# sonniki/image-captioning-with-external-knowledge

Hardware: AMD Instinct MI355X
Metric: decode_steps_per_sec (higher is better)
Workload: dtype f32 (3xbf16 split products, fp32 accumulate); 1 GPU; cfg2: geo variant, per-GPU batch 64 x 20 decode positions, 14x14x2048 features, K=20 knowledge rows, vocab 10000; global_batch=64, graph=True, collective_backend=none, split_allreduce=False, parallelism=dp1 (one flat-bucket all-reduce per step)

## Files before the change

image-captioning-with-external-knowledge_amd/csrc/adam.hip:

```cpp
#include "gemm_common.h"
#include "opt_words.h"

namespace ick {
namespace {

struct AdamHyper {
    float gscale, clip, b1, b2, c1, c2, eps, step, bc2_sqrt, coef, w, wd, f;
    bool coupled;
};

struct AdamEma {
    float* e;
    const float* decay;
    int warmup;
};

struct AdamDecay {
    const float* wd;
    const uint8_t* mask;
    int64_t granules;
    int64_t base;
    int coupled;
};

constexpr int kGranuleShift = 6;

__device__ __forceinline__ bool decay_on(const AdamDecay& dec, int64_t at) {
    const int64_t gr = at >> kGranuleShift;
    return gr < dec.granules && dec.mask[gr] != 0;
}

template <bool kOpt, bool kEma, bool kDecay>
__device__ __forceinline__ bool adam_hyper(AdamHyper& h, float gscale, float clip, float lr, float b1, float b2, float eps,
                                           int step0, const uint32_t* step_ptr, const float* __restrict__ gscale_den,
                                           float* words, const ick_lr_schedule& sched, const AdamEma& ema,
                                           const AdamDecay& dec) {
    if (gscale_den) {
        if (!(gscale_den[0] > 0.f)) return false;
        gscale = gscale / gscale_den[0];
    }
    const float t = (float)(step0 + (step_ptr ? (int)*step_ptr : 0));
    const float bc1 = 1.f - powf(b1, t);
    h.bc2_sqrt = sqrtf(1.f - powf(b2, t));
    h.coef = 1.f;
    if (kOpt) {
        lr = lr_schedule(words[kWordBaseLr], sched, t);
        h.coef = words[kWordCoef];
        if (blockIdx.x == 0 && threadIdx.x == 0) words[kWordLrNow] = lr;
    }
    h.step = lr / bc1;
    h.w = 0.f;
    if (kEma) {
        float d = ema.decay[0];
        if (ema.warmup) d = fminf(d, (1.f + t) / (10.f + t));
        h.w = 1.f - d;
    }
    h.wd = 0.f; h.f = 1.f; h.coupled = false;
    if (kDecay) {
        h.wd = dec.wd[0];
        const float shrink = lr * h.wd;
        h.f = 1.f - shrink;
        h.coupled = dec.coupled != 0;
    }
    h.gscale = gscale; h.clip = clip; h.b1 = b1; h.b2 = b2; h.c1 = 1.f - b1; h.c2 = 1.f - b2; h.eps = eps;
    return true;
}

template <bool kOpt, bool kDecay = false>
__device__ __forceinline__ void adam1(const AdamHyper& h, float& p, float& g, float& m, float& v, bool on = false) {
    float x = g * h.gscale;
    if (kOpt) x = x * h.coef;
    if (h.clip > 0.f) x = fminf(fmaxf(x, -h.clip), h.clip);
    g = x;
    if (kDecay && on) {
        if (h.coupled) {
            const float term = h.wd * p;
            x = x + term;
        } else {
            p = p * h.f;
        }
    }
    m = h.b1 * m + h.c1 * x;
    v = h.b2 * v + h.c2 * x * x;
    p -= h.step * m / (sqrtf(v) / h.bc2_sqrt + h.eps);
}

__device__ __forceinline__ void ema1(const AdamHyper& h, float& e, float p) {
    const float d = p - e;
    e = e + h.w * d;
}

__device__ __forceinline__ void ema4(const AdamHyper& h, float4& e, const float4& p) {
    ema1(h, e.x, p.x);
    ema1(h, e.y, p.y);
    ema1(h, e.z, p.z);
    ema1(h, e.w, p.w);
}

template <bool kOpt, bool kDecay = false>
__device__ __forceinline__ void adam4(const AdamHyper& h, float4& p, float4& g, float4& m, float4& v, bool on = false) {
    adam1<kOpt, kDecay>(h, p.x, g.x, m.x, v.x, on);
    adam1<kOpt, kDecay>(h, p.y, g.y, m.y, v.y, on);
    adam1<kOpt, kDecay>(h, p.z, g.z, m.z, v.z, on);
    adam1<kOpt, kDecay>(h, p.w, g.w, m.w, v.w, on);
}

template <bool kOpt, bool kEma, bool kDecay>
__global__ __launch_bounds__(256) void adam_clamp_kernel(float* __restrict__ p, float* __restrict__ g,
                                                         float* __restrict__ m, float* __restrict__ v, int64_t n,
                                                         float gscale, float clip, float lr, float b1, float b2,
                                                         float eps, int step0, const uint32_t* step_ptr,
                                                         const float* __restrict__ gscale_den, float* words,
                                                         ick_lr_schedule sched, AdamEma ema, AdamDecay dec) {
    const int64_t stride = (int64_t)gridDim.x * 256;
    AdamHyper h;
    if (!adam_hyper<kOpt, kEma, kDecay>(h, gscale, clip, lr, b1, b2, eps, step0, step_ptr, gscale_den, words, sched, ema,
                                         dec))
        return;
    for (int64_t i = (int64_t)blockIdx.x * 256 + threadIdx.x; i < n; i += stride) {
        float gi = g[i], mi = m[i], vi = v[i], pi = p[i], ei = 0.f;
        if (kEma) ei = ema.e[i];
        adam1<kOpt, kDecay>(h, pi, gi, mi, vi, kDecay && decay_on(dec, dec.base + i));
        g[i] = gi; m[i] = mi; v[i] = vi; p[i] = pi;
        if (kEma) { ema1(h, ei, pi); ema.e[i] = ei; }
    }
}

template <bool kOpt, bool kEma, bool kDecay>
__global__ __launch_bounds__(256) void adam_clamp_vec4_kernel(float4* __restrict__ p, float4* __restrict__ g,
                                                              float4* __restrict__ m, float4* __restrict__ v, int64_t n4,
                                                              float gscale, float clip, float lr, float b1, float b2,
                                                              float eps, int step0, const uint32_t* step_ptr,
                                                              const float* __restrict__ gscale_den, float* words,
                                                              ick_lr_schedule sched, AdamEma ema, AdamDecay dec) {
    const int64_t stride = (int64_t)gridDim.x * 256;
    AdamHyper h;
    if (!adam_hyper<kOpt, kEma, kDecay>(h, gscale, clip, lr, b1, b2, eps, step0, step_ptr, gscale_den, words, sched, ema,
                                         dec))
        return;
    float4* __restrict__ e = reinterpret_cast<float4*>(ema.e);
    for (int64_t i = (int64_t)blockIdx.x * 256 + threadIdx.x; i < n4; i += stride) {
        float4 gi = g[i], mi = m[i], vi = v[i], pi = p[i], ei;
        if (kEma) ei = e[i];
        adam4<kOpt, kDecay>(h, pi, gi, mi, vi, kDecay && decay_on(dec, dec.base + 4 * i));
        g[i] = gi; m[i] = mi; v[i] = vi; p[i] = pi;
        if (kEma) { ema4(h, ei, pi); e[i] = ei; }
    }
}

constexpr int kT = 64;
constexpr int kLd = 68;

template <bool kOpt, bool kEma, bool kDecay>
__global__ __launch_bounds__(256) void adam_derive_kernel(float* __restrict__ p, float* __restrict__ g,
                                                          float* __restrict__ m, float* __restrict__ v,
                                                          const ick_adam_item* __restrict__ items,
                                                          const ick_adam_block* __restrict__ blocks, float gscale,
                                                          float clip, float lr, float b1, float b2, float eps, int step0,
                                                          const uint32_t* step_ptr, const float* __restrict__ gscale_den,
                                                          float* words, ick_lr_schedule sched, AdamEma ema, AdamDecay dec) {
    __shared__ __attribute__((aligned(16))) float tile[kT * kLd];
    const ick_adam_block blk = blocks[blockIdx.x];
    AdamHyper h;
    if (!adam_hyper<kOpt, kEma, kDecay>(h, gscale, clip, lr, b1, b2, eps, step0, step_ptr, gscale_den, words, sched, ema,
                                         dec))
        return;
    const int tid = threadIdx.x;

    if (blk.item < 0) {
        float4* p4 = reinterpret_cast<float4*>(p) + blk.off4;
        float4* g4 = reinterpret_cast<float4*>(g) + blk.off4;
        float4* m4 = reinterpret_cast<float4*>(m) + blk.off4;
        float4* v4 = reinterpret_cast<float4*>(v) + blk.off4;
        float4* e4 = reinterpret_cast<float4*>(ema.e) + blk.off4;
        float4 pi[4], gi[4], mi[4], vi[4], ei[4];
        bool on[4];
#pragma unroll
        for (int i = 0; i < 4; ++i) {
            const int j = tid + 256 * i;
            on[i] = false;
            if (j < blk.cnt4) {
                gi[i] = g4[j]; mi[i] = m4[j]; vi[i] = v4[j]; pi[i] = p4[j];
                if (kEma) ei[i] = e4[j];
                if (kDecay) on[i] = decay_on(dec, 4 * ((int64_t)blk.off4 + j));
            }
        }
#pragma unroll
        for (int i = 0; i < 4; ++i) {
            const int j = tid + 256 * i;
            if (j < blk.cnt4) {
                adam4<kOpt, kDecay>(h, pi[i], gi[i], mi[i], vi[i], on[i]);
                g4[j] = gi[i]; m4[j] = mi[i]; v4[j] = vi[i]; p4[j] = pi[i];
                if (kEma) { ema4(h, ei[i], pi[i]); e4[j] = ei[i]; }
                if (blk.copy) reinterpret_cast<float4*>(blk.copy)[j] = pi[i];
            }
        }
        return;
    }

    const ick_adam_item it = items[blk.item];
    const int n0 = blk.tn * kT, k0 = blk.tk * kT;
    const int K = it.K;
    {
        float4 pi[4], gi[4], mi[4], vi[4], ei[4];
        int64_t at[4];
        bool on[4];
#pragma unroll
        for (int i = 0; i < 4; ++i) {
            const int idx = tid + 256 * i;
            const int row = idx >> 4, c4 = idx & 15;
            const int r = n0 + row - it.drow0, k = k0 + 4 * c4;
            at[i] = (r >= 0 && r < it.rows && k < K) ? it.off + (int64_t)r * K + k : -1;
            if (at[i] >= 0) {
                gi[i] = *reinterpret_cast<const float4*>(g + at[i]);
                mi[i] = *reinterpret_cast<const float4*>(m + at[i]);
                vi[i] = *reinterpret_cast<const float4*>(v + at[i]);
                pi[i] = *reinterpret_cast<const float4*>(p + at[i]);
                if (kEma) ei[i] = *reinterpret_cast<const float4*>(ema.e + at[i]);
            }
            on[i] = kDecay && at[i] >= 0 && decay_on(dec, at[i]);
        }
#pragma unroll
        for (int i = 0; i < 4; ++i) {
            const int idx = tid + 256 * i;
            const int row = idx >> 4, c4 = idx & 15;
            float4 out = make_float4(0.f, 0.f, 0.f, 0.f);
            if (at[i] >= 0) {
                adam4<kOpt, kDecay>(h, pi[i], gi[i], mi[i], vi[i], on[i]);
                *reinterpret_cast<float4*>(g + at[i]) = gi[i];
                *reinterpret_cast<float4*>(m + at[i]) = mi[i];
                *reinterpret_cast<float4*>(v + at[i]) = vi[i];
                *reinterpret_cast<float4*>(p + at[i]) = pi[i];
                if (kEma) { ema4(h, ei[i], pi[i]); *reinterpret_cast<float4*>(ema.e + at[i]) = ei[i]; }
                out = pi[i];
                if (it.copy) *reinterpret_cast<float4*>(it.copy + (int64_t)(n0 + row) * it.copy_ld + k0 + 4 * c4) = pi[i];
            }
            *reinterpret_cast<float4*>(tile + row * kLd + 4 * c4) = out;
        }
    }
    __syncthreads();
    const int rlo = it.drow0 - n0, rhi = it.drow0 + it.rows - n0;

    if (it.pack) {
        const int K16 = (K + 15) & ~15;
#pragma unroll
        for (int i = 0; i < 4; ++i) {
            const int u = tid + 256 * i;
            const int j = u >> 6, l = u & 63;
            const int k4 = blk.tk * 16 + j;
// ... 17 lines not shown
    }
    if (it.ps) {
        const int64_t np = (int64_t)((it.Nd + 63) / 64) * 64;
        const int K32 = (K + 31) & ~31;
        char* base = reinterpret_cast<char*>(it.ps);
#pragma unroll
        for (int i = 0; i < 2; ++i) {
            const int u = tid + 256 * i;
            const int row = u & 63, c = u >> 6;
            const int k = k0 + 8 * c;
            if (row >= rlo && row < rhi && k < K32) {
                const float4 a = *reinterpret_cast<const float4*>(tile + row * kLd + 8 * c);
                const float4 b = *reinterpret_cast<const float4*>(tile + row * kLd + 8 * c + 4);
                uint32_t hh[4], mm[4], ll[4];
                split3(a.x, a.y, hh[0], mm[0], ll[0]); split3(a.z, a.w, hh[1], mm[1], ll[1]);
                split3(b.x, b.y, hh[2], mm[2], ll[2]); split3(b.z, b.w, hh[3], mm[3], ll[3]);
                char* dst = base + (((int64_t)(k >> 5) * 3) * np + n0 + row) * 64 + (k & 31) * 2;
                *reinterpret_cast<uint4*>(dst) = uint4{hh[0], hh[1], hh[2], hh[3]};
                *reinterpret_cast<uint4*>(dst + np * 64) = uint4{mm[0], mm[1], mm[2], mm[3]};
                *reinterpret_cast<uint4*>(dst + 2 * np * 64) = uint4{ll[0], ll[1], ll[2], ll[3]};
            }
        }
    }
    if (it.ps_t) {
        const int64_t kp = (int64_t)((K + 63) / 64) * 64;
        char* base = reinterpret_cast<char*>(it.ps_t);
#pragma unroll
        for (int i = 0; i < 2; ++i) {
            const int u = tid + 256 * i;
            const int kk = u & 63, c = u >> 6;
            if (8 * c >= rlo && 8 * c < rhi && k0 + kk < K) {
                float x[8];
#pragma unroll
                for (int e = 0; e < 8; ++e) x[e] = tile[(8 * c + e) * kLd + kk];
                uint32_t hh[4], mm[4], ll[4];
#pragma unroll
                for (int e = 0; e < 4; ++e) split3(x[2 * e], x[2 * e + 1], hh[e], mm[e], ll[e]);
                const int n = n0 + 8 * c;
                char* dst = base + (((int64_t)(n >> 5) * 3) * kp + k0 + kk) * 64 + (n & 31) * 2;
                *reinterpret_cast<uint4*>(dst) = uint4{hh[0], hh[1], hh[2], hh[3]};
                *reinterpret_cast<uint4*>(dst + kp * 64) = uint4{mm[0], mm[1], mm[2], mm[3]};
                *reinterpret_cast<uint4*>(dst + 2 * kp * 64) = uint4{ll[0], ll[1], ll[2], ll[3]};
            }
        }
    }
    if (it.tr) {
#pragma unroll
        for (int i = 0; i < 16; ++i) {
            const int u = tid + 256 * i;
            const int nl = u & 63, kl = u >> 6;
            if (nl >= rlo && nl < rhi && k0 + kl < K) it.tr[(int64_t)(k0 + kl) * it.tr_ld + n0 + nl] = tile[nl * kLd + kl];
        }
    }
}

}
}

using namespace ick;

template <bool kEma, bool kDecay>
static int adam_args(const float* p, const float* g, const float* m, const float* v, int64_t count, int32_t step,
                     const uint32_t* step_ptr, const AdamEma& ema, const AdamDecay& dec, bool& al16) {
    ICK_CHECK_ARG(p && g && m && v && count > 0 && (step >= 1 || step_ptr != nullptr));
    if (kEma) ICK_CHECK_ARG(ema.e != nullptr && ema.decay != nullptr);
    if (kDecay)
        ICK_CHECK_ARG(dec.wd != nullptr && dec.mask != nullptr && dec.granules > 0 &&
                      (dec.coupled == ICK_DECAY_DECOUPLED || dec.coupled == ICK_DECAY_COUPLED));
    al16 = ((reinterpret_cast<uintptr_t>(p) | reinterpret_cast<uintptr_t>(g) | reinterpret_cast<uintptr_t>(m) |
             reinterpret_cast<uintptr_t>(v) | (kEma ? reinterpret_cast<uintptr_t>(ema.e) : 0)) & 15) == 0;
    return ICK_OK;
}

template <bool kOpt, bool kEma, bool kDecay = false>
static int launch_adam(float* p, float* g, float* m, float* v, int64_t n, float gscale, float clip, float lr, float* words,
                       ick_lr_schedule sched, float beta1, float beta2, float eps, int32_t step, const uint32_t* step_ptr,
                       const float* gscale_den, AdamEma ema, void* stream, AdamDecay dec = AdamDecay{}) {
    bool al16;
    if (int rc = adam_args<kEma, kDecay>(p, g, m, v, n, step, step_ptr, ema, dec, al16)) return rc;
    if (kDecay) ICK_CHECK_ARG(dec.granules >= ceil_div(n, (int64_t)1 << kGranuleShift));
    if (kEma && (reinterpret_cast<uintptr_t>(ema.e) & 3)) return ICK_EALIGN;
    int64_t done = 0;
    if (n >= 4096 && al16) {
        const int64_t n4 = n / 4;
        hipLaunchKernelGGL((adam_clamp_vec4_kernel<kOpt, kEma, kDecay>), dim3((int)std::min<int64_t>(ceil_div(n4, 256), 4096)),
                           dim3(256), 0, (hipStream_t)stream, reinterpret_cast<float4*>(p), reinterpret_cast<float4*>(g),
                           reinterpret_cast<float4*>(m), reinterpret_cast<float4*>(v), n4, gscale, clip, lr, beta1, beta2,
                           eps, step, step_ptr, gscale_den, words, sched, ema, dec);
        done = 4 * n4;
        if (done == n) ICK_LAUNCH_RET();
    }
    if (kEma) ema.e += done;
    dec.base = done;
    hipLaunchKernelGGL((adam_clamp_kernel<kOpt, kEma, kDecay>), dim3((int)std::min<int64_t>(ceil_div(n - done, 256), 4096)),
                       dim3(256), 0, (hipStream_t)stream, p + done, g + done, m + done, v + done, n - done, gscale, clip, lr,
                       beta1, beta2, eps, step, step_ptr, gscale_den, words, sched, ema, dec);
    ICK_LAUNCH_RET();
}

template <bool kOpt, bool kEma, bool kDecay = false>
static int launch_adam_derive(float* p, float* g, float* m, float* v, const ick_adam_item* items,
                              const ick_adam_block* blocks, int32_t n_blocks, float gscale, float clip, float lr,
                              float* words, ick_lr_schedule sched, float beta1, float beta2, float eps, int32_t step,
                              const uint32_t* step_ptr, const float* gscale_den, AdamEma ema, void* stream,
                              AdamDecay dec = AdamDecay{}) {
    bool al16;
    if (int rc = adam_args<kEma, kDecay>(p, g, m, v, blocks ? n_blocks : 0, step, step_ptr, ema, dec, al16)) return rc;
    if (!al16) return ICK_EALIGN;
    hipLaunchKernelGGL((adam_derive_kernel<kOpt, kEma, kDecay>), dim3(n_blocks), dim3(256), 0, (hipStream_t)stream, p, g, m, v,
                       items, blocks, gscale, clip, lr, beta1, beta2, eps, step, step_ptr, gscale_den, words, sched, ema,
                       dec);
    ICK_LAUNCH_RET();
}

extern "C" int ick_adam_clamp(float* p, float* g, float* m, float* v, int64_t n, float gscale, float clip, float lr,
                              float beta1, float beta2, float eps, int32_t step, const uint32_t* step_ptr,
                              const float* gscale_den, void* stream) {
    return launch_adam<false, false>(p, g, m, v, n, gscale, clip, lr, nullptr, ick_lr_schedule{}, beta1, beta2, eps, step,
                                     step_ptr, gscale_den, AdamEma{}, stream);
}

extern "C" int ick_adam_opt(float* p, float* g, float* m, float* v, int64_t n, float gscale, float clip, float* words,
                            ick_lr_schedule sched, float beta1, float beta2, float eps, int32_t step,
                            const uint32_t* step_ptr, const float* gscale_den, void* stream) {
    ICK_CHECK_ARG(words != nullptr && lr_schedule_ok(sched));
    return launch_adam<true, false>(p, g, m, v, n, gscale, clip, 0.f, words, sched, beta1, beta2, eps, step, step_ptr,
                                    gscale_den, AdamEma{}, stream);
}

extern "C" int ick_adam_clamp_derive(float* p, float* g, float* m, float* v, const ick_adam_item* items,
                                     const ick_adam_block* blocks, int32_t n_blocks, float gscale, float clip, float lr,
                                     float beta1, float beta2, float eps, int32_t step, const uint32_t* step_ptr,
                                     const float* gscale_den, void* stream) {
    return launch_adam_derive<false, false>(p, g, m, v, items, blocks, n_blocks, gscale, clip, lr, nullptr,
                                            ick_lr_schedule{}, beta1, beta2, eps, step, step_ptr, gscale_den, AdamEma{},
                                            stream);
}

extern "C" int ick_adam_opt_derive(float* p, float* g, float* m, float* v, const ick_adam_item* items,
                                   const ick_adam_block* blocks, int32_t n_blocks, float gscale, float clip, float* words,
                                   ick_lr_schedule sched, float beta1, float beta2, float eps, int32_t step,
                                   const uint32_t* step_ptr, const float* gscale_den, void* stream) {
    ICK_CHECK_ARG(words != nullptr && lr_schedule_ok(sched));
    return launch_adam_derive<true, false>(p, g, m, v, items, blocks, n_blocks, gscale, clip, 0.f, words, sched, beta1,
                                           beta2, eps, step, step_ptr, gscale_den, AdamEma{}, stream);
}

extern "C" int ick_adam_ema(float* p, float* g, float* m, float* v, float* e, int64_t n, float gscale, float clip, float lr,
                            float* words, ick_lr_schedule sched, float beta1, float beta2, float eps, int32_t step,
                            const uint32_t* step_ptr, const float* gscale_den, const float* ema_decay, int32_t ema_warmup,
                            void* stream) {
    const AdamEma ema{e, ema_decay, ema_warmup != 0};
    if (!words)
        return launch_adam<false, true>(p, g, m, v, n, gscale, clip, lr, nullptr, ick_lr_schedule{}, beta1, beta2, eps,
                                        step, step_ptr, gscale_den, ema, stream);
    ICK_CHECK_ARG(lr_schedule_ok(sched));
    return launch_adam<true, true>(p, g, m, v, n, gscale, clip, 0.f, words, sched, beta1, beta2, eps, step, step_ptr,
                                   gscale_den, ema, stream);
}

extern "C" int ick_adam_ema_derive(float* p, float* g, float* m, float* v, float* e, const ick_adam_item* items,
                                   const ick_adam_block* blocks, int32_t n_blocks, float gscale, float clip, float lr,
                                   float* words, ick_lr_schedule sched, float beta1, float beta2, float eps, int32_t step,
                                   const uint32_t* step_ptr, const float* gscale_den, const float* ema_decay,
// ... 16 lines not shown
    return opt();
}

extern "C" int ick_adam_decay(float* p, float* g, float* m, float* v, float* e, int64_t n, float gscale, float clip,
                              float lr, float* words, ick_lr_schedule sched, float beta1, float beta2, float eps,
                              int32_t step, const uint32_t* step_ptr, const float* gscale_den, const float* ema_decay,
                              int32_t ema_warmup, const float* decay, const uint8_t* decay_mask, int64_t n_granules,
                              int32_t decay_form, void* stream) {
    const AdamEma ema{e, ema_decay, ema_warmup != 0};
    const AdamDecay dec{decay, decay_mask, n_granules, 0, decay_form};
    const ick_lr_schedule none{};
    if (!e)
        return with_rate(
            words, sched,
            [&] { return launch_adam<false, false, true>(p, g, m, v, n, gscale, clip, lr, nullptr, none, beta1, beta2, eps,
                                                         step, step_ptr, gscale_den, AdamEma{}, stream, dec); },
            [&] { return launch_adam<true, false, true>(p, g, m, v, n, gscale, clip, 0.f, words, sched, beta1, beta2, eps,
                                                        step, step_ptr, gscale_den, AdamEma{}, stream, dec); });
    return with_rate(
        words, sched,
        [&] { return launch_adam<false, true, true>(p, g, m, v, n, gscale, clip, lr, nullptr, none, beta1, beta2, eps, step,
                                                    step_ptr, gscale_den, ema, stream, dec); },
        [&] { return launch_adam<true, true, true>(p, g, m, v, n, gscale, clip, 0.f, words, sched, beta1, beta2, eps, step,
                                                   step_ptr, gscale_den, ema, stream, dec); });
}

extern "C" int ick_adam_decay_derive(float* p, float* g, float* m, float* v, float* e, const ick_adam_item* items,
                                     const ick_adam_block* blocks, int32_t n_blocks, float gscale, float clip, float lr,
                                     float* words, ick_lr_schedule sched, float beta1, float beta2, float eps, int32_t step,
                                     const uint32_t* step_ptr, const float* gscale_den, const float* ema_decay,
                                     int32_t ema_warmup, const float* decay, const uint8_t* decay_mask,
                                     int64_t n_granules, int32_t decay_form, void* stream) {
    const AdamEma ema{e, ema_decay, ema_warmup != 0};
    const AdamDecay dec{decay, decay_mask, n_granules, 0, decay_form};
    const ick_lr_schedule none{};
    if (!e)
        return with_rate(
            words, sched,
            [&] { return launch_adam_derive<false, false, true>(p, g, m, v, items, blocks, n_blocks, gscale, clip, lr,
                                                                nullptr, none, beta1, beta2, eps, step, step_ptr,
                                                                gscale_den, AdamEma{}, stream, dec); },
            [&] { return launch_adam_derive<true, false, true>(p, g, m, v, items, blocks, n_blocks, gscale, clip, 0.f, words,
                                                               sched, beta1, beta2, eps, step, step_ptr, gscale_den,
                                                               AdamEma{}, stream, dec); });
    return with_rate(
        words, sched,
        [&] { return launch_adam_derive<false, true, true>(p, g, m, v, items, blocks, n_blocks, gscale, clip, lr, nullptr,
                                                           none, beta1, beta2, eps, step, step_ptr, gscale_den, ema, stream,
                                                           dec); },
        [&] { return launch_adam_derive<true, true, true>(p, g, m, v, items, blocks, n_blocks, gscale, clip, 0.f, words,
                                                          sched, beta1, beta2, eps, step, step_ptr, gscale_den, ema, stream,
                                                          dec); });
}
```

image-captioning-with-external-knowledge_amd/csrc/backward.hip:

```cpp
#include "common.h"

namespace ick {
namespace {

template <int NJ>
__global__ __launch_bounds__(256) void layernorm_bwd_kernel(const float* __restrict__ dy, const float* __restrict__ x,
                                                            const float* __restrict__ res,
                                                            const float* __restrict__ gamma,
                                                            const float* __restrict__ mean,
                                                            const float* __restrict__ rstd, float* __restrict__ dz,
                                                            float* __restrict__ dgamma, float* __restrict__ dbeta,
                                                            int64_t rows, int d, int rows_per_block,
                                                            float* __restrict__ dx_drop, DropArg darg,
                                                            float* __restrict__ partials) {
    chain_priority();
    extern __shared__ float sm[];
    const Dropout drop = darg.get();
    const int lane = threadIdx.x & 63, wave = threadIdx.x >> 6;
    float ag[NJ], ab[NJ], gm[NJ];
#pragma unroll
    for (int j = 0; j < NJ; ++j) {
        const int c = lane + 64 * j;
        ag[j] = 0.f; ab[j] = 0.f;
        gm[j] = c < d ? gamma[c] : 0.f;
// ... 150 lines not shown
                                                                float* __restrict__ dtype_emb, int ntypes,
                                                                float* __restrict__ dword, int B, int K, int d) {
    if (!SEQ) chain_priority();
    const ScatterWalk<SEQ> w(B * K);
    for (int row = w.row; row < w.row_end; ++row) {
        const EntityIndex ix = entity_index(variant, ent + (int64_t)row * cols, ntypes, vocab);
        bool mine = w.owns(ix.type);
        if (variant == ICK_NEWS && dword != nullptr) {
#pragma unroll
            for (int q = 0; q < 5; ++q) mine = mine || w.owns(ix.name[q]);
        }
        if (!mine) continue;
        for (int c = w.col; c < d; c += w.col_step) {
            float g = dee[(int64_t)row * d + c];
            if (variant == ICK_NEWS) {
                float s = 0.f;
#pragma unroll
                for (int q = 0; q < 5; ++q) s += word_emb[(int64_t)ix.name[q] * d + c];
                const float avg = s / 5.0f;
                const float enc_g = g * avg;
                if (dword) {
                    const float enc = avg != 0.f ? ee[(int64_t)row * d + c] / avg : 0.f;
                    const float gw = g * enc / 5.0f;
#pragma unroll
                    for (int q = 0; q < 5; ++q) w.add(dword + (int64_t)ix.name[q] * d + c, ix.name[q], gw);
                }
                g = enc_g;
            }
            if (c >= ix.type_off)
                w.add(dtype_emb + (int64_t)ix.type * (d - ix.type_off) + (c - ix.type_off), ix.type, g);
        }
    }
}

template <bool SEQ>
__global__ __launch_bounds__(256) void fact_encode_bwd_kernel(const float* __restrict__ dfe,
                                                              const int64_t* __restrict__ facts, float* __restrict__ dee,
                                                              float* __restrict__ dpred, int num_pred, int B, int K,
                                                              int F, int d) {
    if (!SEQ) chain_priority();
    const ScatterWalk<SEQ> w(B * F);
    for (int row = w.row; row < w.row_end; ++row) {
        const FactPair f = fact_pair(facts, row, K, num_pred);
        const int64_t erow = (int64_t)(row / F) * K + f.subj;
        if (!w.owns(erow) && !w.owns(f.pred)) continue;
        for (int c = w.col; c < d; c += w.col_step) {
            const float g = dfe[(int64_t)row * d + c];
            w.add(dee + erow * d + c, erow, g);
            w.add(dpred + (int64_t)f.pred * d + c, f.pred, g);
        }
    }
}

__global__ __launch_bounds__(256) void pointer_bwd_dh_kernel(const float* __restrict__ ds, int64_t ds_ld, int col0,
                                                             const float* __restrict__ ctx, const float* __restrict__ w,
                                                             const float* __restrict__ ind, float* __restrict__ dh,
                                                             int T, int Kc, int d, const int32_t* __restrict__ rowmap,
                                                             const int32_t* __restrict__ count) {
    chain_priority();
    int b = blockIdx.y, t = blockIdx.x;
    int64_t dsrow = (int64_t)b * T + t;
    if (rowmap != nullptr) {
        if (dsrow >= device_bound((int)gridDim.y * T, count)) return;
        const int lr = rowmap[dsrow];
        b = lr / T;
        t = lr - b * T;
    }
    const float* dsr = ds + dsrow * ds_ld + col0;
    for (int c = threadIdx.x; c < d; c += 256) {
        float acc = 0.f;
        const float* cc = ctx + (int64_t)b * Kc * d + c;
        int k = 0;
        for (; k + 8 <= Kc; k += 8) {
            float v[8], g[8];
#pragma unroll
            for (int q = 0; q < 8; ++q) {
                v[q] = cc[(int64_t)(k + q) * d];
                g[q] = dsr[k + q];
                if (ind) g[q] *= ind[((int64_t)b * T + t) * Kc + k + q];
            }
#pragma unroll
            for (int q = 0; q < 8; ++q) acc = fmaf(g[q], v[q], acc);
        }
        for (; k < Kc; ++k) {
            float g = dsr[k];
            if (ind) g *= ind[((int64_t)b * T + t) * Kc + k];
            acc = fmaf(g, cc[(int64_t)k * d], acc);
        }
        dh[((int64_t)b * T + t) * d + c] += acc * w[c];
    }
}

template <bool SEQ>
__global__ __launch_bounds__(256) void pointer_bwd_dctx_kernel(const float* __restrict__ ds, int64_t ds_ld, int col0,
                                                               const float* __restrict__ h, const float* __restrict__ ctx,
                                                               const float* __restrict__ w, const float* __restrict__ ind,
                                                               float* __restrict__ dctx, float* __restrict__ dw,
                                                               float* __restrict__ dbias, int B, int T, int Kc, int d,
                                                               const int32_t* __restrict__ rowstart) {
    chain_priority();
    extern __shared__ float gs[];
    float* red = gs + T * Kc;
    float* dwp = red + 4;
    const int lane = threadIdx.x & 63, wave = threadIdx.x >> 6;
  for (int b = SEQ ? 0 : blockIdx.x; b < (SEQ ? B : (int)blockIdx.x + 1); ++b) {
    float bsum = 0.f;
    const int64_t row0 = rowstart ? rowstart[b] : (int64_t)b * T;
    const int nrow = rowstart ? min(T, rowstart[b + 1] - rowstart[b]) : T;
    for (int idx = threadIdx.x; idx < T * Kc; idx += 256) {
        const int t = idx / Kc, k = idx - t * Kc;
        float g = t < nrow ? ds[(row0 + t) * ds_ld + col0 + k] : 0.f;
        bsum += g;
        if (ind) g *= ind[((int64_t)b * T + t) * Kc + k];
        gs[idx] = g;
    }
    bsum = block_sum<4>(bsum, red);
    if (threadIdx.x == 0 && blockIdx.y == 0) { if (SEQ) dbias[0] += bsum; else atomicAdd(dbias, bsum); }
    const int c = blockIdx.y * 64 + lane;
    const bool ok = c < d;
    const float* hb = h + (int64_t)b * T * d + (ok ? c : 0);
    const float wc = ok ? w[c] : 0.f;
    float dwl = 0.f;
    for (int k = wave; k < Kc; k += 4) {
        float acc = 0.f;
        for (int t = 0; t < T; ++t) acc = fmaf(gs[t * Kc + k], hb[(int64_t)t * d], acc);
        if (ok) {
            const int64_t o = ((int64_t)b * Kc + k) * d + c;
            dctx[o] += acc * wc;
            dwl = fmaf(acc, ctx[o], dwl);
        }
    }
    dwp[wave * 64 + lane] = dwl;
    __syncthreads();
    if (wave == 0 && ok) {
        const float t = (dwp[lane] + dwp[64 + lane]) + (dwp[128 + lane] + dwp[192 + lane]);
        if (SEQ) dw[c] += t; else atomicAdd(dw + c, t);
    }
    if (SEQ) __syncthreads();
  }
}

template <bool SEQ>
__global__ __launch_bounds__(256) void context_gate_bwd_kernel(const int64_t* __restrict__ captions,
                                                               const int64_t* __restrict__ facts,
                                                               const float* __restrict__ dgate, float* __restrict__ dw,
                                                               float* __restrict__ dbias, int B, int L, int T, int K, int F,
                                                               int V, int num_pred, int d, int mode) {
    extern __shared__ int smi[];
    const int tid = threadIdx.x;
  for (int b = SEQ ? 0 : blockIdx.x; b < (SEQ ? B : (int)blockIdx.x + 1); ++b) {
    const GateTables g = build_gate_tables(smi, captions, facts, b, L, K, F, V, num_pred, mode);
    const int *act = g.act, *pred = g.pred, *rep = g.rep;
    float* suf = reinterpret_cast<float*>(g.end);
    const int c = blockIdx.y * 256 + tid;
    if (c < d) {
        float run = 0.f;
        for (int p = T - 1; p >= 0; --p) {
            run += dgate[((int64_t)b * T + p) * d + c];
            suf[p * 256 + tid] = run;
        }
        if (SEQ) dbias[c] += run; else atomicAdd(dbias + c, run);
        for (int j = 0; j < F; ++j) {
            if (!rep[j] || act[j] >= T) continue;
            float* dst = dw + (int64_t)c * num_pred + pred[j];
            if (SEQ) *dst += suf[act[j] * 256 + tid]; else atomicAdd(dst, suf[act[j] * 256 + tid]);
        }
    }
    if (SEQ) __syncthreads();
  }
}

__global__ void counter_add_kernel(uint32_t* c, uint32_t inc, const float* flag) {
    if (flag == nullptr || flag[0] > 0.f) *c += inc;
}

__global__ __launch_bounds__(256) void scale_kernel(float* __restrict__ x, int64_t n, const float* __restrict__ num,
                                                    const float* __restrict__ den) {
    const float s = num[0] / den[0];
    const int64_t stride = (int64_t)gridDim.x * 256;
    for (int64_t i = (int64_t)blockIdx.x * 256 + threadIdx.x; i < n; i += stride) x[i] *= s;
}

}
}

using namespace ick;

extern "C" int ick_layernorm_bwd_rows_per_block(void) { return 8; }

extern "C" int ick_layernorm_bwd(const float* dy, const float* x, const float* res, const float* gamma,
                                 const float* mean, const float* rstd, float* dz, float* dgamma, float* dbeta,
                                 int64_t rows, int32_t d, float* dx_drop, float drop_p, uint32_t drop_seed,
// ... 29 lines not shown

extern "C" int ick_colsum(const float* a, int64_t M, int32_t N, int64_t ld, float* out, void* stream) {
    ICK_CHECK_ARG(a && out && M > 0 && N > 0 && ld >= N);
    const int rpb = deterministic() ? (int)std::min<int64_t>(M, 1 << 30) : 64;
    ICK_CHECK_ARG(ceil_div(M, rpb) <= 65535);
    hipLaunchKernelGGL(colsum_kernel, dim3(ceil_div(N, 64), ceil_div(M, rpb)), dim3(256), 0, (hipStream_t)stream, a, M,
                       N, ld, out, rpb);
    ICK_LAUNCH_RET();
}

extern "C" int ick_caption_embed_bwd(const float* dx, const int64_t* captions, const int64_t* masks, float* dword,
                                     float* dee, float* dfe, int32_t B, int32_t L, int32_t K, int32_t F, int32_t V,
                                     int32_t d, int32_t pad_token, float scale, float drop_p, uint32_t drop_seed,
                                     uint32_t drop_site, const uint32_t* drop_epoch, void* stream) {
    ICK_CHECK_ARG(dx && captions && masks && dee && B > 0 && L > 0 && K > 0 && d > 0);
    if (deterministic())
        hipLaunchKernelGGL(caption_embed_bwd_kernel<true>, dim3(kDetParts, ceil_div(d, 256)), dim3(256), 0,
                           (hipStream_t)stream, dx, captions, masks, dword, dee, dfe, B, L, K, F, V, d, pad_token, scale,
                           DropArg{drop_p, drop_seed, drop_site, drop_epoch});
    else
        hipLaunchKernelGGL(caption_embed_bwd_kernel<false>, dim3(ceil_div((int64_t)B * L, 4)), dim3(256), 0, (hipStream_t)stream,
                           dx, captions, masks, dword, dee, dfe, B, L, K, F, V, d, pad_token, scale,
                           DropArg{drop_p, drop_seed, drop_site, drop_epoch});
    ICK_LAUNCH_RET();
}

extern "C" int ick_pointer_scores_bwd(const float* ds, int64_t ds_ld, int32_t col0, const float* h, const float* ctx,
                                      const float* w, const float* ind, float* dh, float* dctx, float* dw,
                                      float* dbias, int32_t B, int32_t T, int32_t Kc, int32_t d, void* stream) {
    return ick_pointer_scores_bwd_packed(ds, ds_ld, col0, h, ctx, w, ind, dh, dctx, dw, dbias, B, T, Kc, d, nullptr, nullptr,
                                         stream);
}

extern "C" int ick_pointer_scores_bwd_packed(const float* ds, int64_t ds_ld, int32_t col0, const float* h, const float* ctx,
                                             const float* w, const float* ind, float* dh, float* dctx, float* dw,
                                             float* dbias, int32_t B, int32_t T, int32_t Kc, int32_t d,
                                             const int32_t* rowmap, const int32_t* rowstart, void* stream) {
    ICK_CHECK_ARG(ds && h && ctx && w && dh && dctx && dw && dbias && B > 0 && B <= 65535 && T > 0 && Kc > 0 && d > 0);
    ICK_CHECK_ARG((rowmap == nullptr) == (rowstart == nullptr) && (int64_t)B * T <= INT32_MAX);
    const size_t smem = ((size_t)T * Kc + 4 + 256) * sizeof(float);
    ICK_CHECK_ARG(smem <= 64 * 1024);
    hipStream_t s = (hipStream_t)stream;
    hipLaunchKernelGGL(pointer_bwd_dh_kernel, dim3(T, B), dim3(256), 0, s, ds, ds_ld, col0, ctx, w, ind, dh, T, Kc, d, rowmap,
                       rowstart ? rowstart + B : nullptr);
    if (deterministic())
        hipLaunchKernelGGL(pointer_bwd_dctx_kernel<true>, dim3(1, ceil_div(d, 64)), dim3(256), smem, s, ds, ds_ld, col0, h,
                           ctx, w, ind, dctx, dw, dbias, B, T, Kc, d, rowstart);
    else
        hipLaunchKernelGGL(pointer_bwd_dctx_kernel<false>, dim3(B, ceil_div(d, 64)), dim3(256), smem, s, ds, ds_ld, col0, h,
                           ctx, w, ind, dctx, dw, dbias, B, T, Kc, d, rowstart);
    ICK_LAUNCH_RET();
}

extern "C" int ick_entity_encode_bwd(int32_t variant, const float* dee, const float* entities, int32_t ent_cols,
                                     const float* ee, const float* word_emb, int32_t vocab, float* dtype_emb,
                                     int32_t ntypes, float* dword, int32_t B, int32_t K, int32_t d, void* stream) {
    ICK_CHECK_ARG(dee && entities && dtype_emb && B > 0 && K > 0 && d > 6);
    if (variant == ICK_NEWS) ICK_CHECK_ARG(ee && word_emb && vocab > 0);
    if (deterministic())
        hipLaunchKernelGGL(entity_encode_bwd_kernel<true>, dim3(kDetParts, ceil_div(d, 256)), dim3(256), 0,
                           (hipStream_t)stream, variant, dee, entities, ent_cols, ee, word_emb, vocab, dtype_emb, ntypes,
                           dword, B, K, d);
    else
        hipLaunchKernelGGL(entity_encode_bwd_kernel<false>, dim3(ceil_div((int64_t)B * K, 4)), dim3(256), 0, (hipStream_t)stream,
                           variant, dee, entities, ent_cols, ee, word_emb, vocab, dtype_emb, ntypes, dword, B, K, d);
    ICK_LAUNCH_RET();
}

extern "C" int ick_fact_encode_bwd(const float* dfe, const int64_t* facts, float* dee, float* dpred, int32_t num_pred,
                                   int32_t B, int32_t K, int32_t F, int32_t d, void* stream) {
    ICK_CHECK_ARG(dfe && facts && dee && dpred && B > 0 && K > 0 && F > 0 && d > 0);
    if (deterministic())
        hipLaunchKernelGGL(fact_encode_bwd_kernel<true>, dim3(kDetParts, ceil_div(d, 256)), dim3(256), 0, (hipStream_t)stream,
                           dfe, facts, dee, dpred, num_pred, B, K, F, d);
    else
        hipLaunchKernelGGL(fact_encode_bwd_kernel<false>, dim3(ceil_div((int64_t)B * F, 4)), dim3(256), 0, (hipStream_t)stream,
                           dfe, facts, dee, dpred, num_pred, B, K, F, d);
    ICK_LAUNCH_RET();
}

extern "C" int ick_context_gate_bwd(const int64_t* captions, const int64_t* facts, const float* dgate, float* dw,
                                    float* dbias, int32_t B, int32_t L, int32_t T, int32_t K, int32_t F, int32_t V,
                                    int32_t num_pred, int32_t d, int32_t mode, void* stream) {
    ICK_CHECK_ARG(captions && facts && dgate && dw && dbias && B > 0 && L > 0 && K > 0 && F > 0);
    ICK_CHECK_ARG((mode == 0 && T == L) || (mode == 1 && T == 1));
    const size_t smem = gate_table_ints(K, F) * sizeof(int) + (size_t)T * 256 * sizeof(float);
    ICK_CHECK_ARG(smem <= 64 * 1024);
    if (deterministic())
        hipLaunchKernelGGL(context_gate_bwd_kernel<true>, dim3(1, ceil_div(d, 256)), dim3(256), smem, (hipStream_t)stream,
                           captions, facts, dgate, dw, dbias, B, L, T, K, F, V, num_pred, d, mode);
    else
        hipLaunchKernelGGL(context_gate_bwd_kernel<false>, dim3(B, ceil_div(d, 256)), dim3(256), smem, (hipStream_t)stream,
                           captions, facts, dgate, dw, dbias, B, L, T, K, F, V, num_pred, d, mode);
    ICK_LAUNCH_RET();
}

extern "C" int ick_scale_by_ratio(float* x, int64_t n, const float* num, const float* den, void* stream) {
    ICK_CHECK_ARG(x && num && den && n > 0);
    hipLaunchKernelGGL(scale_kernel, dim3((int)std::min<int64_t>(ceil_div(n, 256), 4096)), dim3(256), 0,
                       (hipStream_t)stream, x, n, num, den);
    ICK_LAUNCH_RET();
}

extern "C" int ick_counter_add(uint32_t* counter, uint32_t inc, void* stream) {
    ICK_CHECK_ARG(counter != nullptr);
    hipLaunchKernelGGL(counter_add_kernel, dim3(1), dim3(1), 0, (hipStream_t)stream, counter, inc, (const float*)nullptr);
// ... 9 lines not shown
```

image-captioning-with-external-knowledge_amd/csrc/score_head.hip:

```cpp
#include "decode_select.h"

namespace ick {
namespace {

constexpr int kMaxPerLane = 16;

template <int NJ>
__global__ __launch_bounds__(256) void pointer_scores_kernel(const float* __restrict__ h, const float* __restrict__ ctx,
                                                             const float* __restrict__ w, const float* __restrict__ bias,
                                                             const float* __restrict__ ind, float* __restrict__ out,
                                                             int T, int Kc, int d, int64_t out_ld, int col0,
                                                             const int32_t* __restrict__ out_gmap,
                                                             const int32_t* __restrict__ rowmap,
                                                             const int32_t* __restrict__ count) {
    chain_priority();
    constexpr int KB = 4;
    const int lane = threadIdx.x & 63, wave = threadIdx.x >> 6;
    int b = blockIdx.y, t = blockIdx.x;
    int64_t orow_id = -1;
    if (rowmap != nullptr) {
        const int m = b * T + t;
        if (m >= device_bound((int)gridDim.y * T, count)) return;
        const int lr = rowmap[m];
        b = lr / T;
// ... 294 lines not shown
        if (tid == 0) row_loss[row] = lse - r[target];
    }
    if (dr) {
        const float wr = kWeighted ? weight[b] : 1.f;
        const float inv = wr / s;
        const float wt = kSmooth ? wr * keep : wr, wu = wr * nsub;
        float4* d4 = reinterpret_cast<float4*>(dr);
        const int tq = (int)(target >> 2), tr = (int)(target & 3);
        for (int i0 = 0; i0 < n4; i0 += 256 * 4) {
            float4 x[4];
#pragma unroll
            for (int j = 0; j < 4; ++j) {
                const int i = i0 + tid + 256 * j;
                x[j] = i < n4 ? r4[i] : make_float4(0.f, 0.f, 0.f, 0.f);
            }
#pragma unroll
            for (int j = 0; j < 4; ++j) {
                const int i = i0 + tid + 256 * j;
                if (i < n4) {
                    float4 gq = make_float4(__expf(x[j].x - m) * inv, __expf(x[j].y - m) * inv, __expf(x[j].z - m) * inv,
                                            __expf(x[j].w - m) * inv);
                    if constexpr (kSmooth) { gq.x += wu; gq.y += wu; gq.z += wu; gq.w += wu; }
                    if (i == tq) {
                        if (tr == 0) gq.x -= wt; else if (tr == 1) gq.y -= wt; else if (tr == 2) gq.z -= wt; else gq.w -= wt;
                    }
                    d4[i] = gq;
                }
            }
        }
        for (int i0 = 4 * n4; i0 < Vx; i0 += 256 * 8) {
            float x[8];
#pragma unroll
            for (int j = 0; j < 8; ++j) {
                const int i = i0 + tid + 256 * j;
                x[j] = i < Vx ? r[i] : 0.f;
            }
#pragma unroll
            for (int j = 0; j < 8; ++j) {
                const int i = i0 + tid + 256 * j;
                if (i < Vx) {
                    if constexpr (kSmooth) dr[i] = (__expf(x[j] - m) * inv + wu) - (i == target ? wt : 0.f);
                    else dr[i] = __expf(x[j] - m) * inv - (i == target ? wr : 0.f);
                }
            }
        }
    }
}

template <bool kWeighted>
__global__ __launch_bounds__(256) void packed_ce_reduce_kernel(const float* __restrict__ row_loss, int n, int L,
                                                               const float* __restrict__ weight,
                                                               float* __restrict__ loss_sum, float* __restrict__ count,
                                                               const int32_t* __restrict__ rowmap,
                                                               const int32_t* __restrict__ nrows) {
    __shared__ float red[4];
    float s = 0.f, c = 0.f;
    n = device_bound(n, nrows);
    for (int i = threadIdx.x; i < n; i += 256) {
        const float v = row_loss[i];
        if (v > -0.5f) { s += kWeighted ? weight[(rowmap ? rowmap[i] : i) / L] * v : v; c += 1.f; }
    }
    s = block_sum<4>(s, red);
    c = block_sum<4>(c, red);
    if (threadIdx.x == 0) { loss_sum[0] = s; count[0] = c; }
}

struct RowScan {
    float m, s;
    float cnt;
    int bi;
};
__device__ __forceinline__ void row_scan_push(RowScan& a, float x, int c, float st, int target) {
    a.s += __expf(x - a.m);
    a.cnt += (x > st || (x == st && c < target)) ? 1.f : 0.f;
}
__device__ __forceinline__ void row_scan_best(float& bv, int& bi, float x, int c) {
    if (x > bv) { bv = x; bi = c; }
}

__global__ __launch_bounds__(256) void row_logprob_rank_kernel(const float* __restrict__ scores, int64_t ld,
                                                               const int64_t* __restrict__ caps,
                                                               const int32_t* __restrict__ rowmap,
                                                               const int32_t* __restrict__ count, int L, int Vx, int pad,
                                                               float* __restrict__ tlp, int32_t* __restrict__ rank,
                                                               int32_t* __restrict__ best) {
    __shared__ float4 red[4];
    const int tid = threadIdx.x, lane = tid & 63, wave = tid >> 6;
    const int64_t row = (int64_t)blockIdx.y * L + blockIdx.x;
    if (row >= device_bound((int)gridDim.y * L, count)) return;
    const int lr = rowmap[row];
    const int b = lr / L, t = lr - b * L;
    if (b >= (int)gridDim.y || t >= L - 1) return;
    const int64_t o = (int64_t)b * (L - 1) + t;
    const int64_t target64 = caps[(int64_t)b * L + t + 1];
    if (target64 == pad || target64 < 0 || target64 >= Vx) {
        if (tid == 0) { tlp[o] = 0.f; rank[o] = -1; best[o] = -1; }
        return;
    }
    const int target = (int)target64;
    const float* r = scores + row * ld;
    const float st = r[target];
    const bool vec = (ld & 3) == 0 && (reinterpret_cast<uintptr_t>(scores) & 15) == 0;
    const int n4 = vec ? (Vx >> 2) : 0;
    const float4* r4 = reinterpret_cast<const float4*>(r);
    RowScan a{-INFINITY, 0.f, 0.f, 0x7fffffff};
    for (int i0 = 0; i0 < n4; i0 += 256 * 4) {
        float4 x[4];
#pragma unroll
        for (int j = 0; j < 4; ++j) {
            const int i = i0 + tid + 256 * j;
            x[j] = i < n4 ? r4[i] : make_float4(-INFINITY, -INFINITY, -INFINITY, -INFINITY);
        }
        float bm = a.m;
        int bi = a.bi;
#pragma unroll
        for (int j = 0; j < 4; ++j) {
            const int c = 4 * (i0 + tid + 256 * j);
// ... 183 lines not shown
}

extern "C" int ick_head_rowmap(const int64_t* lengths, int32_t B, int32_t L, int32_t* decode_len, int32_t* rowstart,
                               int32_t* rowmap, void* stream) {
    using namespace ick;
    ICK_CHECK_ARG(lengths && decode_len && rowstart && rowmap && B > 0 && L > 0 && (int64_t)B * L <= INT32_MAX);
    hipLaunchKernelGGL(head_rowmap_kernel, dim3(1), dim3(256), 0, (hipStream_t)stream, lengths, B, L, decode_len, rowstart,
                       rowmap);
    ICK_LAUNCH_RET();
}

extern "C" int ick_gather_rows(const float* src, int64_t src_rs, const int32_t* rowmap, const int32_t* count, float* dst,
                               int64_t dst_rs, int32_t max_rows, int32_t d, void* stream) {
    using namespace ick;
    ICK_CHECK_ARG(src && rowmap && count && dst && max_rows > 0 && d > 0 && src_rs >= d && dst_rs >= d);
    hipLaunchKernelGGL(gather_rows_kernel, dim3(ceil_div(max_rows, 4)), dim3(256), 0, (hipStream_t)stream, src, src_rs,
                       rowmap, count, dst, dst_rs, max_rows, d);
    ICK_LAUNCH_RET();
}

extern "C" int ick_top2(const float* scores, int64_t ld, int32_t B, int32_t Vx, int32_t* best, int32_t* second,
                        void* stream) {
    using namespace ick;
    ICK_CHECK_ARG(scores && best && second && B > 0 && Vx > 0 && ld >= Vx);
    hipLaunchKernelGGL(top2_kernel, dim3(B), dim3(256), 0, (hipStream_t)stream, scores, ld, Vx, best, second);
    ICK_LAUNCH_RET();
}

extern "C" int ick_greedy_update(const int32_t* best, const int32_t* second, int64_t* output, int32_t* top2_hist,
                                 int32_t* finished, int64_t* next_token, int64_t* next_mask, int32_t B, int32_t step,
                                 int32_t max_len, int32_t V, int32_t K, int32_t has_facts, int32_t end_token,
                                 void* stream) {
    using namespace ick;
    ICK_CHECK_ARG(best && second && output && top2_hist && finished && next_token && next_mask);
    ICK_CHECK_ARG(B > 0 && step >= 0 && step < max_len);
    hipLaunchKernelGGL(greedy_update_kernel, dim3(ceil_div(B, 64)), dim3(64), 0, (hipStream_t)stream, best, second,
                       output, top2_hist, finished, next_token, next_mask, B, step, max_len, V, K, has_facts,
                       end_token);
    ICK_LAUNCH_RET();
}

extern "C" int ick_greedy_select(const float* scores, int64_t ld, int32_t B, int32_t Vx, int64_t* output,
                                 int32_t* top2_hist, int32_t* finished, int64_t* next_token, int64_t* next_mask,
                                 int32_t step, int32_t max_len, int32_t V, int32_t K, int32_t has_facts,
                                 int32_t end_token, void* stream) {
    using namespace ick;
    ICK_CHECK_ARG(scores && output && top2_hist && finished && next_token && next_mask);
    ICK_CHECK_ARG(B > 0 && Vx > 0 && ld >= Vx && step >= 0 && step < max_len);
    hipLaunchKernelGGL(greedy_select_kernel, dim3(B), dim3(256), 0, (hipStream_t)stream, scores, ld, Vx, output,
                       top2_hist, finished, next_token, next_mask, step, max_len, V, K, has_facts, end_token);
    ICK_LAUNCH_RET();
}

extern "C" int ick_packed_ce(const float* scores, int64_t ld, const int64_t* captions_sorted,
                             const int32_t* decode_len, int32_t B, int32_t L, int32_t Vx, int32_t pad_token,
                             float* row_loss, float* loss_sum, float* count, float* dscores, void* stream) {
    using namespace ick;
    ICK_CHECK_ARG(scores && captions_sorted && decode_len && row_loss && loss_sum && count);
    ICK_CHECK_ARG(B > 0 && B <= 65535 && L > 0 && Vx > 0 && ld >= Vx);
    hipStream_t s = (hipStream_t)stream;
    hipLaunchKernelGGL(packed_ce_rows_kernel<false>, dim3(L, B), dim3(256), 0, s, scores, ld, captions_sorted, decode_len,
                       L, Vx, pad_token, row_loss, dscores, nullptr, nullptr, CeEps<false>{});
    hipLaunchKernelGGL(packed_ce_reduce_kernel<false>, dim3(1), dim3(256), 0, s, row_loss, B * L, L, nullptr, loss_sum,
                       count, nullptr, nullptr);
    ICK_LAUNCH_RET();
}

extern "C" int ick_packed_ce_packed(const float* scores, int64_t ld, const int64_t* captions, const int32_t* rowmap,
                                    const int32_t* count, const float* weights, int32_t B, int32_t L, int32_t Vx,
                                    int32_t pad_token, float* row_loss, float* loss_sum, float* count_out, float* dscores,
                                    void* stream) {
    using namespace ick;
    ICK_CHECK_ARG(scores && captions && rowmap && count && row_loss && loss_sum && count_out);
    ICK_CHECK_ARG(B > 0 && B <= 65535 && L > 0 && Vx > 0 && ld >= Vx && (int64_t)B * L <= INT32_MAX);
    hipStream_t s = (hipStream_t)stream;
    if (weights != nullptr) {
        hipLaunchKernelGGL((packed_ce_rows_kernel<true, true>), dim3(L, B), dim3(256), 0, s, scores, ld, captions, count, L,
                           Vx, pad_token, row_loss, dscores, weights, rowmap, CeEps<false>{});
        hipLaunchKernelGGL(packed_ce_reduce_kernel<true>, dim3(1), dim3(256), 0, s, row_loss, B * L, L, weights, loss_sum,
                           count_out, rowmap, count);
    } else {
        hipLaunchKernelGGL((packed_ce_rows_kernel<false, true>), dim3(L, B), dim3(256), 0, s, scores, ld, captions, count, L,
                           Vx, pad_token, row_loss, dscores, nullptr, rowmap, CeEps<false>{});
        hipLaunchKernelGGL(packed_ce_reduce_kernel<false>, dim3(1), dim3(256), 0, s, row_loss, B * L, L, nullptr, loss_sum,
                           count_out, rowmap, count);
    }
    ICK_LAUNCH_RET();
}

extern "C" int ick_packed_ce_smooth(const float* scores, int64_t ld, const int64_t* captions, const int32_t* rowmap,
                                    const int32_t* count, const int32_t* decode_len, const float* weights,
                                    const float* eps, int32_t B, int32_t L, int32_t Vx, int32_t pad_token,
                                    float* row_loss, float* loss_sum, float* count_out, float* dscores, void* stream) {
    using namespace ick;
    ICK_CHECK_ARG(scores && captions && eps && row_loss && loss_sum && count_out);
    ICK_CHECK_ARG((rowmap != nullptr) == (count != nullptr) && (rowmap != nullptr || decode_len != nullptr));
    ICK_CHECK_ARG(B > 0 && B <= 65535 && L > 0 && Vx > 0 && ld >= Vx && (int64_t)B * L <= INT32_MAX);
    hipStream_t s = (hipStream_t)stream;
    const dim3 grid(L, B), block(256);
    const int32_t* dl = rowmap ? count : decode_len;
#define ICK_CE_SMOOTH(W, P)                                                                                            \
    hipLaunchKernelGGL((packed_ce_rows_kernel<W, P, true>), grid, block, 0, s, scores, ld, captions, dl, L, Vx,         \
                       pad_token, row_loss, dscores, weights, rowmap, CeEps<true>{eps})
    if (weights != nullptr) {
        if (rowmap) { ICK_CE_SMOOTH(true, true); } else { ICK_CE_SMOOTH(true, false); }
        hipLaunchKernelGGL(packed_ce_reduce_kernel<true>, dim3(1), block, 0, s, row_loss, B * L, L, weights, loss_sum,
                           count_out, rowmap, count);
    } else {
        if (rowmap) { ICK_CE_SMOOTH(false, true); } else { ICK_CE_SMOOTH(false, false); }
        hipLaunchKernelGGL(packed_ce_reduce_kernel<false>, dim3(1), block, 0, s, row_loss, B * L, L, nullptr, loss_sum,
                           count_out, rowmap, count);
    }
#undef ICK_CE_SMOOTH
    ICK_LAUNCH_RET();
}

extern "C" int ick_row_logprob_rank(const float* scores, int64_t ld, const int64_t* captions, const int32_t* rowmap,
                                    const int32_t* count, int32_t R, int32_t L, int32_t Vx, int32_t pad_token,
                                    float* token_log_prob, int32_t* rank, int32_t* best, void* stream) {
    using namespace ick;
    ICK_CHECK_ARG(scores && captions && rowmap && count && token_log_prob && rank && best);
    ICK_CHECK_ARG(R > 0 && R <= 65535 && L > 1 && Vx > 0 && Vx <= (1 << 24) && ld >= Vx && (int64_t)R * L <= INT32_MAX);
    hipLaunchKernelGGL(row_logprob_rank_kernel, dim3(L, R), dim3(256), 0, (hipStream_t)stream, scores, ld, captions,
                       rowmap, count, L, Vx, pad_token, token_log_prob, rank, best);
    ICK_LAUNCH_RET();
}

extern "C" int ick_caption_score_sums(const int32_t* rowstart, int32_t R, int32_t L, int32_t top_k, float* token_log_prob,
                                      int32_t* rank, int32_t* best, float* log_prob, int32_t* tokens, float* loss_sum,
                                      float* count, float* top1_hits, float* topk_hits, void* stream) {
    using namespace ick;
    ICK_CHECK_ARG(rowstart && token_log_prob && rank && best && log_prob && tokens && loss_sum && count && top1_hits &&
                  topk_hits);
    ICK_CHECK_ARG(R > 0 && L > 1 && top_k >= 1 && (int64_t)R * L <= INT32_MAX);
    hipStream_t s = (hipStream_t)stream;
    hipLaunchKernelGGL(caption_sums_kernel, dim3(ceil_div(R, 4)), dim3(256), 0, s, rowstart, R, L, token_log_prob, rank,
                       best, log_prob, tokens);
    hipLaunchKernelGGL(caption_totals_kernel, dim3(1), dim3(256), 0, s, token_log_prob, rank, (int64_t)R * (L - 1), top_k,
                       loss_sum, count, top1_hits, topk_hits);
    ICK_LAUNCH_RET();
}

extern "C" int ick_packed_ce_weighted(const float* scores, int64_t ld, const int64_t* captions_sorted,
                                      const int32_t* decode_len, const float* weights, int32_t B, int32_t L, int32_t Vx,
                                      int32_t pad_token, float* row_loss, float* loss_sum, float* count, float* dscores,
                                      void* stream) {
    using namespace ick;
    ICK_CHECK_ARG(scores && captions_sorted && decode_len && weights && row_loss && loss_sum && count);
    ICK_CHECK_ARG(B > 0 && B <= 65535 && L > 0 && Vx > 0 && ld >= Vx && (int64_t)B * L <= INT32_MAX);
    hipStream_t s = (hipStream_t)stream;
    hipLaunchKernelGGL(packed_ce_rows_kernel<true>, dim3(L, B), dim3(256), 0, s, scores, ld, captions_sorted, decode_len,
                       L, Vx, pad_token, row_loss, dscores, weights, nullptr, CeEps<false>{});
    hipLaunchKernelGGL(packed_ce_reduce_kernel<true>, dim3(1), dim3(256), 0, s, row_loss, B * L, L, weights, loss_sum,
                       count, nullptr, nullptr);
    ICK_LAUNCH_RET();
}
```

image-captioning-with-external-knowledge_amd/lib.py:

```python
import ctypes as C
import os

_PKG = os.path.dirname(os.path.abspath(__file__))
LIB_PATH = os.path.join(_PKG, "libick_amd.so")
if os.environ.get("ICK_LIB_PATH"):
    LIB_PATH = os.environ["ICK_LIB_PATH"]

ICK_GEO, ICK_KNOWLEDGE, ICK_NEWS = 0, 1, 2
VARIANT_ID = {"geo": ICK_GEO, "knowledge": ICK_KNOWLEDGE, "news": ICK_NEWS}
GEMM_RELU, GEMM_ACCUM, GEMM_ATOMIC, GEMM_COLSUM_ONLY = 1, 2, 4, 16

vp = C.c_void_p
i32 = C.c_int32
i64 = C.c_int64
f32 = C.c_float
u32 = C.c_uint32


class GemmArgs(C.Structure):
    _fields_ = [
        ("A", vp), ("B", vp), ("C", vp), ("bias", vp),
        ("M", i32), ("N", i32), ("K", i32),
        ("a_rs", i64), ("a_ks", i64), ("a_grp", i32), ("a_gs", i64), ("a_gmap", vp),
        ("b_rs", i64), ("b_ks", i64),
# ... 173 lines not shown
    "ick_greedy_select": [vp, i64, i32, i32, vp, vp, vp, vp, vp, i32, i32, i32, i32, i32, i32, vp],
    "ick_packed_ce": [vp, i64, vp, vp, i32, i32, i32, i32, vp, vp, vp, vp, vp],
    "ick_packed_ce_weighted": [vp, i64, vp, vp, vp, i32, i32, i32, i32, vp, vp, vp, vp, vp],
    "ick_samples_to_captions": [vp, i32, i32, i32, i32, i32, i32, i32, i32, vp, vp, vp, vp],
    "ick_cider_d": [vp, i32, i32, vp, i32, i32, i32, vp, vp, i32, f32, f32, i32, i32, i32, vp, i32, i32, vp, i32,
                    vp, vp, vp],
    "ick_decode_supported": [i32, i32, i32, i32, i32],
    "ick_decode_plan": [i32, i32, i32, i32, i32, C.POINTER(i32)],
    "ick_decode_layers": [C.POINTER(DecodeCtx), i32, vp],
    "ick_decode_layers_part": [C.POINTER(DecodeCtx), i32, i32, vp],
    "ick_decode_layers_attn": [C.POINTER(DecodeCtx), vp, i32, i32, vp],
    "ick_decode_init": [C.POINTER(DecodeCtx), i32, i32, vp],
    "ick_decode_select_greedy": [C.POINTER(DecodeCtx), i32, vp],
    "ick_decode_select_beam": [C.POINTER(DecodeCtx), C.POINTER(BeamState), i32, vp],
    "ick_decode_beam_supported": [i32, i32],
    "ick_decode_select_sample": [C.POINTER(DecodeCtx), C.POINTER(SampleState), i32, vp],
    "ick_decode_sample_supported": [i32, i32],
    "ick_decode_select_beam_rules": [C.POINTER(DecodeCtx), C.POINTER(BeamState), C.POINTER(DecodeRules), i32, vp],
    "ick_decode_select_sample_rules": [C.POINTER(DecodeCtx), C.POINTER(SampleState), C.POINTER(DecodeRules), i32, vp],
    "ick_decode_select_beam_diverse": [C.POINTER(DecodeCtx), C.POINTER(BeamState), C.POINTER(DecodeRules),
                                       C.POINTER(DecodeDiversity), i32, vp],
    "ick_decode_select_beam_forced": [C.POINTER(DecodeCtx), C.POINTER(BeamState), C.POINTER(DecodeRules),
                                      C.POINTER(DecodeConstraints), i32, vp],
    "ick_decode_select_beam_biased": [C.POINTER(DecodeCtx), C.POINTER(BeamState), C.POINTER(DecodeRules),
                                      C.POINTER(DecodeBias), i32, vp],
    "ick_decode_select_sample_biased": [C.POINTER(DecodeCtx), C.POINTER(SampleState), C.POINTER(DecodeRules),
                                        C.POINTER(DecodeBias), i32, vp],
    "ick_attention_bwd": [C.POINTER(AttnBwdArgs), vp],
    "ick_layernorm_bwd": [vp, vp, vp, vp, vp, vp, vp, vp, vp, i64, i32, vp, f32, u32, u32, vp, vp, vp],
    "ick_layernorm_bwd_rows_per_block": [],
    "ick_gemm_grouped": [vp, i32, vp],
    "ick_attention_bwd_overwrites": [i32, i32, i32],
    "ick_attention_plan": [i32, i32, i32, i32, i32, C.POINTER(i32)],
    "ick_relu_bwd": [vp, vp, vp, i64, f32, vp],
    "ick_colsum": [vp, i64, i32, i64, vp, vp],
    "ick_caption_embed_bwd": [vp, vp, vp, vp, vp, vp, i32, i32, i32, i32, i32, i32, i32, f32, f32, u32, u32, vp, vp],
    "ick_pointer_scores_bwd": [vp, i64, i32, vp, vp, vp, vp, vp, vp, vp, vp, i32, i32, i32, i32, vp],
    "ick_entity_encode_bwd": [i32, vp, vp, i32, vp, vp, i32, vp, i32, vp, i32, i32, i32, vp],
    "ick_fact_encode_bwd": [vp, vp, vp, vp, i32, i32, i32, i32, i32, vp],
    "ick_context_gate_bwd": [vp, vp, vp, vp, vp, i32, i32, i32, i32, i32, i32, i32, i32, i32, vp],
    "ick_adam_clamp": [vp, vp, vp, vp, i64, f32, f32, f32, f32, f32, f32, i32, vp, vp, vp],
    "ick_adam_clamp_derive": [vp, vp, vp, vp, vp, vp, i32, f32, f32, f32, f32, f32, f32, i32, vp, vp, vp],
    "ick_grad_sqnorm_plan": [i64, C.POINTER(i32)],
    "ick_grad_sqnorm": [vp, i64, f32, vp, vp, i64, vp, vp],
    "ick_adam_opt": [vp, vp, vp, vp, i64, f32, f32, vp, LrSchedule, f32, f32, f32, i32, vp, vp, vp],
    "ick_adam_opt_derive": [vp, vp, vp, vp, vp, vp, i32, f32, f32, vp, LrSchedule, f32, f32, f32, i32, vp, vp, vp],
    "ick_adam_ema": [vp, vp, vp, vp, vp, i64, f32, f32, f32, vp, LrSchedule, f32, f32, f32, i32, vp, vp, vp, i32, vp],
    "ick_adam_ema_derive": [vp, vp, vp, vp, vp, vp, vp, i32, f32, f32, f32, vp, LrSchedule, f32, f32, f32, i32, vp, vp, vp,
                            i32, vp],
    "ick_adam_decay": [vp, vp, vp, vp, vp, i64, f32, f32, f32, vp, LrSchedule, f32, f32, f32, i32, vp, vp, vp, i32, vp, vp,
                       i64, i32, vp],
    "ick_adam_decay_derive": [vp, vp, vp, vp, vp, vp, vp, i32, f32, f32, f32, vp, LrSchedule, f32, f32, f32, i32, vp, vp, vp,
                              i32, vp, vp, i64, i32, vp],
    "ick_conv1_wgrad_plan": [i32, i32, i32, i32, C.POINTER(i32), C.POINTER(i64)],
    "ick_conv1_wgrad": [vp, vp, vp, vp, i32, i32, i32, i32, vp, i64, vp],
    "ick_counter_add": [vp, u32, vp],
    "ick_counter_add_if": [vp, u32, vp, vp],
    "ick_timestamp": [vp, vp],
    "ick_copy_batch": [vp, vp, vp, i32, vp],
    "ick_scale_by_ratio": [vp, i64, vp, vp, vp],
    "ick_head_rowmap": [vp, i32, i32, vp, vp, vp, vp],
    "ick_pointer_scores_packed": [vp, vp, vp, vp, vp, vp, i32, i32, i32, i32, i64, i32, vp, vp, vp],
    "ick_packed_ce_packed": [vp, i64, vp, vp, vp, vp, i32, i32, i32, i32, vp, vp, vp, vp, vp],
    "ick_packed_ce_smooth": [vp, i64, vp, vp, vp, vp, vp, vp, i32, i32, i32, i32, vp, vp, vp, vp, vp],
    "ick_pointer_scores_bwd_packed": [vp, i64, i32, vp, vp, vp, vp, vp, vp, vp, vp, i32, i32, i32, i32, vp, vp, vp],
    "ick_gather_rows": [vp, i64, vp, vp, vp, i64, i32, i32, vp],
    "ick_row_logprob_rank": [vp, i64, vp, vp, vp, i32, i32, i32, i32, vp, vp, vp, vp],
    "ick_caption_score_sums": [vp, i32, i32, i32, vp, vp, vp, vp, vp, vp, vp, vp, vp, vp],
    "ick_sched_sample_mix": [vp, i64, vp, vp, vp, vp, i32, i32, i32, i32, i32, i32, i32, vp, vp, vp, vp, i32, vp, vp, vp,
                             vp],
    "ick_caption_metrics": [vp, i32, i32, vp, i32, i32, i32, i32, i32, i32, vp, i32, i32, C.c_double, i32, vp, i32, vp,
                            vp, vp, vp, vp, vp, vp, vp, vp],
    "ick_caption_metric_sums": [vp, vp, vp, i32, vp, vp, vp, vp],
    "ick_geo_reference_counts": [vp, i32, i32, vp, vp, vp, i32, i32, i32, i32, C.POINTER(i32), i32, i32, i32, vp, i32, vp,
                                 i32, i32, i64, i64, i64, vp, vp, vp, vp],
}

_lib = None
PROFILE = None
_proxy = None


class IckError(RuntimeError):
    pass


def load():
    return _proxy if _proxy is not None else load_raw()


def load_raw():
    global _lib
    if _lib is None:
        if not os.path.exists(LIB_PATH):
            raise IckError(
                "libick_amd.so is missing (%s): build it with `python -c 'import __graft_entry__ as g; g.build()'`"
                " -- there is no fallback path" % LIB_PATH)
        import torch
        lib = C.CDLL(LIB_PATH)
        for name, argtypes in SIGNATURES.items():
            fn = getattr(lib, name)
            fn.argtypes = argtypes
            fn.restype = C.c_int
        _lib = lib
    return _lib


_ERRS = {-1: "ICK_EINVAL (bad shape / null pointer / unsupported size)", -2: "ICK_EALIGN", -3: "ICK_EWORKSPACE"}


def check(rc, what):
    if rc != 0:
        raise IckError("%s failed: %s" % (what, _ERRS.get(rc, "hipError_t %d" % rc)))
```

image-captioning-with-external-knowledge_amd/ops.py:

```python
import contextlib
import ctypes as C
import gc
import math
import os

import torch

from . import lib as L


def _p(t):
    return None if t is None else t.data_ptr()


def _stream():
    return torch.cuda.current_stream().cuda_stream


def _f32c(t, name):
    if t.dtype != torch.float32 or not t.is_cuda:
        raise L.IckError("%s must be a float32 device tensor (got %s on %s)" % (name, t.dtype, t.device))
    return t


# ... 577 lines not shown
def decode_select_beam(ctx, beam_state, pos, rules=None, diversity=None, constraints=None, bias=None):
    if bias is not None:
        if diversity is not None or constraints is not None:
            raise L.IckError("decode_select_beam: a column bias does not compose with beam groups or forced columns")
        name, extra = "ick_decode_select_beam_biased", (_ref(rules), C.byref(bias))
    elif constraints is not None:
        name, extra = "ick_decode_select_beam_forced", (_ref(rules), C.byref(constraints))
    elif diversity is not None:
        name, extra = "ick_decode_select_beam_diverse", (_ref(rules), C.byref(diversity))
    else:
        name, extra = ("ick_decode_select_beam", ()) if rules is None else ("ick_decode_select_beam_rules", (_ref(rules),))
    L.check(getattr(L.load(), name)(C.byref(ctx), C.byref(beam_state), *extra, pos, _stream()), name)


def decode_select_beam_forced(ctx, beam_state, rules, constraints, pos):
    decode_select_beam(ctx, beam_state, pos, rules, constraints=constraints)


def decode_select_sample(ctx, sample_state, pos, rules=None, bias=None):
    if bias is not None:
        name, extra = "ick_decode_select_sample_biased", (_ref(rules), C.byref(bias))
    else:
        name, extra = ("ick_decode_select_sample", ()) if rules is None else \
            ("ick_decode_select_sample_rules", (_ref(rules),))
    L.check(getattr(L.load(), name)(C.byref(ctx), C.byref(sample_state), *extra, pos, _stream()), name)


class HeadRows:

    def __init__(self, lengths, B, Lc):
        dev = lengths.device
        lengths = lengths.reshape(-1)
        if lengths.dtype != torch.int64 or not lengths.is_contiguous():
            lengths = lengths.to(torch.int64).contiguous()
        assert lengths.numel() == B
        self.B, self.L = B, Lc
        self.decode_len = torch.empty(B, device=dev, dtype=torch.int32)
        self.rowstart = torch.empty(B + 1, device=dev, dtype=torch.int32)
        self.rowmap = torch.empty(B * Lc, device=dev, dtype=torch.int32)
        self.count = self.rowstart[B:]
        L.check(L.load().ick_head_rowmap(_p(lengths), B, Lc, _p(self.decode_len), _p(self.rowstart), _p(self.rowmap),
                                         _stream()), "ick_head_rowmap")


def gather_rows(x2, pack):
    rows, d = x2.shape
    assert x2.stride(1) == 1 and rows == pack.rowmap.numel()
    out = torch.empty(rows, d, device=x2.device, dtype=torch.float32)
    L.check(L.load().ick_gather_rows(_p(x2), x2.stride(0), _p(pack.rowmap), _p(pack.count), _p(out), d, rows, d,
                                     _stream()), "ick_gather_rows")
    return out


def packed_ce_rows(scores, captions, pack, pad_token, weights=None, want_grad=False, out_sum=None, out_count=None):
    B, Lc, Vx = scores.shape
    dev = scores.device
    if weights is not None and (weights.shape != (B,) or weights.dtype != torch.float32 or not weights.is_cuda or
                                not weights.is_contiguous()):
        raise L.IckError("packed_ce_rows needs contiguous (B,) float32 weights on the device")
    row_loss = torch.empty(B * Lc, device=dev, dtype=torch.float32)
    loss_sum = out_sum if out_sum is not None else torch.empty(1, device=dev, dtype=torch.float32)
    count = out_count if out_count is not None else torch.empty(1, device=dev, dtype=torch.float32)
    dscores = None
    assert scores.stride(0) == Lc * scores.stride(1) and scores.stride(2) == 1
    if want_grad:
        dscores = torch.empty(B, Lc, scores.stride(1), device=dev, dtype=torch.float32)[:, :, :Vx]
    L.check(L.load().ick_packed_ce_packed(_p(scores), scores.stride(1), _p(captions), _p(pack.rowmap), _p(pack.count),
                                          _p(weights), B, Lc, Vx, pad_token, _p(row_loss), _p(loss_sum), _p(count),
                                          _p(dscores), _stream()), "ick_packed_ce_packed")
    return loss_sum, count, dscores


def row_logprob_rank(scores, captions, pack, pad_token, out=None):
    R, Lc, Vx = scores.shape
    dev = scores.device
    if captions.dtype != torch.int64 or not captions.is_contiguous() or tuple(captions.shape) != (R, Lc):
        raise L.IckError("row_logprob_rank needs contiguous int64 captions (%d, %d)" % (R, Lc))
    assert scores.stride(0) == Lc * scores.stride(1) and scores.stride(2) == 1 and pack.rowmap.numel() == R * Lc
    if out is None:
        out = (torch.empty(R, Lc - 1, device=dev, dtype=torch.float32),
               torch.empty(R, Lc - 1, device=dev, dtype=torch.int32),
               torch.empty(R, Lc - 1, device=dev, dtype=torch.int32))
    tlp, rank, best = out
    assert all(t.shape == (R, Lc - 1) and t.is_contiguous() for t in out)
    assert tlp.dtype == torch.float32 and rank.dtype == torch.int32 and best.dtype == torch.int32
    L.check(L.load().ick_row_logprob_rank(_p(scores), scores.stride(1), _p(captions), _p(pack.rowmap), _p(pack.count), R,
                                          Lc, Vx, pad_token, _p(tlp), _p(rank), _p(best), _stream()),
            "ick_row_logprob_rank")
    return tlp, rank, best


def caption_score_sums(pack, tlp, rank, best, top_k=5, out=None):
    R, T = tlp.shape
    dev = tlp.device
    if out is None:
        out = (torch.empty(R, device=dev, dtype=torch.float32), torch.empty(R, device=dev, dtype=torch.int32),
               torch.empty(4, device=dev, dtype=torch.float32))
    log_prob, tokens, totals = out
    assert log_prob.shape == tokens.shape == (R,) and totals.shape == (4,) and totals.is_contiguous()
    assert log_prob.dtype == totals.dtype == torch.float32 and tokens.dtype == torch.int32
    assert pack.rowstart.numel() == R + 1 and tlp.is_contiguous() and rank.is_contiguous() and best.is_contiguous()
    L.check(L.load().ick_caption_score_sums(_p(pack.rowstart), R, T + 1, int(top_k), _p(tlp), _p(rank), _p(best),
                                            _p(log_prob), _p(tokens), _p(totals[0:1]), _p(totals[1:2]), _p(totals[2:3]),
                                            _p(totals[3:4]), _stream()), "ick_caption_score_sums")
    return log_prob, tokens, totals[0:1], totals[1:2], totals[2:3], totals[3:4]


def packed_ce(scores, captions_sorted, decode_len, pad_token, want_grad=False, out_sum=None, out_count=None):
    B, Lc, Vx = scores.shape
    dev = scores.device
    row_loss = torch.empty(B * Lc, device=dev, dtype=torch.float32)
    loss_sum = out_sum if out_sum is not None else torch.empty(1, device=dev, dtype=torch.float32)
    count = out_count if out_count is not None else torch.empty(1, device=dev, dtype=torch.float32)
    dscores = None
    if want_grad:
        dscores = torch.empty(B, Lc, scores.stride(1), device=dev, dtype=torch.float32)[:, :, :Vx]
        assert scores.stride(0) == Lc * scores.stride(1) and scores.stride(2) == 1
    L.check(L.load().ick_packed_ce(_p(scores), scores.stride(1), _p(captions_sorted), _p(decode_len), B, Lc, Vx,
                                   pad_token, _p(row_loss), _p(loss_sum), _p(count), _p(dscores), _stream()),
            "ick_packed_ce")
    return loss_sum, count, dscores


def packed_ce_weighted(scores, captions_sorted, decode_len, weights, pad_token, want_grad=False, out_sum=None,
                       out_count=None):
    B, Lc, Vx = scores.shape
    dev = scores.device
    if weights.shape != (B,) or weights.dtype != torch.float32 or not weights.is_cuda or not weights.is_contiguous():
        raise L.IckError("packed_ce_weighted needs contiguous (B,) float32 weights on the device")
    row_loss = torch.empty(B * Lc, device=dev, dtype=torch.float32)
    loss_sum = out_sum if out_sum is not None else torch.empty(1, device=dev, dtype=torch.float32)
    count = out_count if out_count is not None else torch.empty(1, device=dev, dtype=torch.float32)
    dscores = None
    if want_grad:
        dscores = torch.empty(B, Lc, scores.stride(1), device=dev, dtype=torch.float32)[:, :, :Vx]
        assert scores.stride(0) == Lc * scores.stride(1) and scores.stride(2) == 1
    L.check(L.load().ick_packed_ce_weighted(_p(scores), scores.stride(1), _p(captions_sorted), _p(decode_len),
                                            _p(weights), B, Lc, Vx, pad_token, _p(row_loss), _p(loss_sum), _p(count),
                                            _p(dscores), _stream()),
            "ick_packed_ce_weighted")
    return loss_sum, count, dscores


def packed_ce_smooth(scores, captions, decode_len_or_pack, pad_token, eps, weights=None, want_grad=False, out_sum=None,
                     out_count=None):
    B, Lc, Vx = scores.shape
    dev = scores.device
    if not isinstance(eps, torch.Tensor) or eps.numel() != 1 or eps.dtype != torch.float32 or not eps.is_cuda:
        raise L.IckError("packed_ce_smooth needs eps as a one-element float32 tensor on the device")
    if weights is not None and (weights.shape != (B,) or weights.dtype != torch.float32 or not weights.is_cuda or
                                not weights.is_contiguous()):
        raise L.IckError("packed_ce_smooth needs contiguous (B,) float32 weights on the device")
    pack = decode_len_or_pack if isinstance(decode_len_or_pack, HeadRows) else None
    row_loss = torch.empty(B * Lc, device=dev, dtype=torch.float32)
    loss_sum = out_sum if out_sum is not None else torch.empty(1, device=dev, dtype=torch.float32)
    count = out_count if out_count is not None else torch.empty(1, device=dev, dtype=torch.float32)
    dscores = None
    if pack is not None or want_grad:
        assert scores.stride(0) == Lc * scores.stride(1) and scores.stride(2) == 1
    if want_grad:
        dscores = torch.empty(B, Lc, scores.stride(1), device=dev, dtype=torch.float32)[:, :, :Vx]
    rowmap, rows, dl = (pack.rowmap, pack.count, None) if pack is not None else (None, None, decode_len_or_pack)
    L.check(L.load().ick_packed_ce_smooth(_p(scores), scores.stride(1), _p(captions), _p(rowmap), _p(rows), _p(dl),
                                          _p(weights), _p(eps), B, Lc, Vx, pad_token, _p(row_loss), _p(loss_sum),
                                          _p(count), _p(dscores), _stream()), "ick_packed_ce_smooth")
    return loss_sum, count, dscores


def samples_to_captions(tokens, V, K, has_facts, start, end, pad, out=None):
    R, T = tokens.shape
    if tokens.dtype != torch.int64 or not tokens.is_cuda or not tokens.is_contiguous():
        raise L.IckError("samples_to_captions needs a contiguous int64 (R, T) device tensor")
    if out is None:
        out = (torch.empty(R, T + 1, device=tokens.device, dtype=torch.int64),
               torch.empty(R, T + 1, device=tokens.device, dtype=torch.int64),
               torch.empty(R, device=tokens.device, dtype=torch.int64))
    caps, masks, lengths = out
    assert caps.shape == masks.shape == (R, T + 1) and lengths.shape == (R,)
    assert caps.is_contiguous() and masks.is_contiguous() and lengths.is_contiguous()
    L.check(L.load().ick_samples_to_captions(_p(tokens), R, T, V, K, int(bool(has_facts)), start, end, pad, _p(caps),
                                             _p(masks), _p(lengths), _stream()),
            "ick_samples_to_captions")
    return caps, masks, lengths


SCHED_SAMPLE_MODES = ("sample", "argmax")


def sched_sample_mix(scores, pack, captions, caption_masks, V, K, F, start_token, pad_token, prob, temperature, seed,
                     step, mode="sample", out=None):
    B, Lc, Vx = scores.shape
    dev = scores.device
    if mode not in SCHED_SAMPLE_MODES:
        raise L.IckError("sched_sample_mix: unknown mode %r (one of %s)" % (mode, ", ".join(SCHED_SAMPLE_MODES)))
    if Vx != V + K + F:
        raise L.IckError("sched_sample_mix: scores have %d columns, V + K + F is %d" % (Vx, V + K + F))
    for name, t in (("captions", captions), ("caption_masks", caption_masks)):
        if t.dtype != torch.int64 or not t.is_cuda or not t.is_contiguous() or tuple(t.shape) != (B, Lc):
            raise L.IckError("sched_sample_mix needs contiguous int64 %s (%d, %d) on the device" % (name, B, Lc))
    for name, t, dt in (("prob", prob, torch.float32), ("temperature", temperature, torch.float32),
                        ("seed", seed, torch.int64), ("step", step, torch.int32)):
        if not isinstance(t, torch.Tensor) or t.numel() != 1 or t.dtype != dt or not t.is_cuda:
            raise L.IckError("sched_sample_mix needs %s as a one-element %s tensor on the device" % (name, dt))
    assert scores.stride(0) == Lc * scores.stride(1) and scores.stride(2) == 1
    assert pack.B == B and pack.L == Lc
    if out is None:
        out = (torch.empty(B, Lc, device=dev, dtype=torch.int64), torch.empty(B, Lc, device=dev, dtype=torch.int64),
               torch.empty(B, Lc, device=dev, dtype=torch.int32))
    caps_in, masks_in, replaced = out
    assert all(tuple(t.shape) == (B, Lc) and t.is_contiguous() for t in out)
    assert caps_in.dtype == masks_in.dtype == torch.int64 and replaced.dtype == torch.int32
    L.check(L.load().ick_sched_sample_mix(_p(scores), scores.stride(1), _p(pack.rowstart), _p(pack.decode_len),
                                          _p(captions), _p(caption_masks), B, Lc, V, K, F, start_token, pad_token,
                                          _p(prob), _p(temperature), _p(seed), _p(step), int(mode == "argmax"),
                                          _p(caps_in), _p(masks_in), _p(replaced), _stream()), "ick_sched_sample_mix")
    return caps_in, masks_in, replaced


# ... 405 lines not shown
        elif db is not None:
            if pack is not None:
                gemm_grouped([colsum_problem(dy, db, k_bound=kb)])
            else:
                colsum(dy, db)

    overlap = SIDE is not None and (dw is not None or db is not None)
    if overlap:
        if wg is not None:
            SIDE.add_problem(wg, dy, x, xt_ps)
            for e in extra:
                SIDE.add_problem(e, dy)
            if group_now:
                SIDE.flush_group()
        else:
            SIDE.submit(param_grads, dy, x)
    if need_dx:
        scatter = {} if pack is None else dict(m_bound=kb, c_grp=1, c_gs=dx.stride(0), c_gmap=pack.rowmap)
        split = max(1, min(16, N // 1024)) if (M * K) <= 1280 * 512 else 1
        if is_deterministic():
            split = 1
        elif accumulate_dx and split == 1 and N >= 512 and (M * K) <= 1280 * 512:
            split = max(1, min(8, (N + 150) // 300))
        if wt_ps is not None and split > 1 and gemm_split_mode() >= 1 and K <= 320:
            split = max(1, min(16, N // 512, 256 // ((M + 63) // 64)))
        if split > 1:
            if dx is None:
                dx = torch.zeros(M, K, device=dy.device, dtype=torch.float32)
            elif not accumulate_dx:
                dx.zero_()
            gemm_raw(dy, w, dx, M, K, N, dy.stride(0), 1, 1, w.stride(0), dx.stride(0), atomic=True, split_k=split,
                     b_ps=wt_ps, **scatter)
        else:
            if dx is None:
                dx = torch.empty(M, K, device=dy.device, dtype=torch.float32)
            gemm_raw(dy, w, dx, M, K, N, dy.stride(0), 1, 1, w.stride(0), dx.stride(0), accumulate=accumulate_dx,
                     gate=gate, gate_scale=gate_scale, **scatter)
            gate = None
    if not overlap:
        param_grads()
    if gate is not None:
        relu_bwd(dx, gate, out=dx, scale=gate_scale)
    return dx


def caption_embed_bwd(dx, captions, masks, dword, dee, dfe, V, pad_token, scale, drop=None):
    B, Lc = captions.shape
    K, d = dee.shape[1], dee.shape[2]
    F = 0 if dfe is None else dfe.shape[1]
    L.check(L.load().ick_caption_embed_bwd(_p(dx), _p(captions), _p(masks), _p(dword), _p(dee), _p(dfe), B, Lc, K, F,
                                           V, d, pad_token, scale, *_dargs(drop), _stream()), "ick_caption_embed_bwd")


def pointer_scores_bwd(dscores, col0, h, ctx, w, ind, dh, dctx, dw, dbias, pack=None):
    B, T, d = h.shape
    Kc = ctx.shape[1]
    if pack is not None:
        L.check(L.load().ick_pointer_scores_bwd_packed(_p(dscores), dscores.stride(-2), col0, _p(h), _p(ctx), _p(w), _p(ind),
                                                       _p(dh), _p(dctx), _p(dw), _p(dbias), B, T, Kc, d, _p(pack.rowmap),
                                                       _p(pack.rowstart), _stream()), "ick_pointer_scores_bwd_packed")
        return
    L.check(L.load().ick_pointer_scores_bwd(_p(dscores), dscores.stride(-2), col0, _p(h), _p(ctx), _p(w), _p(ind),
                                            _p(dh), _p(dctx), _p(dw), _p(dbias), B, T, Kc, d, _stream()),
            "ick_pointer_scores_bwd")


def entity_encode_bwd(variant, dee, entities, ee, dtype_emb, word_emb=None, dword=None):
    B, K, cols = entities.shape
    d = dee.shape[2]
    L.check(L.load().ick_entity_encode_bwd(L.VARIANT_ID[variant], _p(dee), _p(entities), cols, _p(ee), _p(word_emb),
                                           0 if word_emb is None else word_emb.shape[0], _p(dtype_emb),
                                           dtype_emb.shape[0], _p(dword), B, K, d, _stream()),
            "ick_entity_encode_bwd")


def fact_encode_bwd(dfe, facts, dee, dpred):
    B, F, d = dfe.shape
    K = dee.shape[1]
    L.check(L.load().ick_fact_encode_bwd(_p(dfe), _p(facts), _p(dee), _p(dpred), dpred.shape[0], B, K, F, d,
                                         _stream()), "ick_fact_encode_bwd")


def context_gate_bwd(captions, facts, dgate, dw, dbias, K, V, mode=0):
    B, Lc = captions.shape
    F = facts.shape[1]
    T, d = dgate.shape[1], dgate.shape[2]
    L.check(L.load().ick_context_gate_bwd(_p(captions), _p(facts), _p(dgate), _p(dw), _p(dbias), B, Lc, T, K, F, V,
                                          dw.shape[1], d, mode, _stream()), "ick_context_gate_bwd")


def _opt_words(words, who):
    if not isinstance(words, torch.Tensor) or words.dtype != torch.float32 or not words.is_cuda or \
            words.numel() < L.OPT_WORDS or not words.is_contiguous() or words.data_ptr() % 16:
        raise L.IckError("%s needs the optimizer words as a contiguous, 16-byte aligned float32 device tensor of %d "
                         "elements (base lr, max_norm, norm, coef, lr used, sum of squares)" % (who, L.OPT_WORDS))
    return words


def lr_schedule_struct(schedule):
    if isinstance(schedule, L.LrSchedule):
        return schedule
    sch = schedule or {}
    kind = sch.get("kind", "constant")
    if kind not in L.LR_KINDS:
        raise L.IckError("unknown lr schedule kind %r (one of %s)" % (kind, ", ".join(sorted(L.LR_KINDS))))
    return L.LrSchedule(L.LR_KINDS[kind], int(sch.get("warmup_steps", 0)), int(sch.get("total_steps", 0)),
                        float(sch.get("min_lr_ratio", 0.0)))


def grad_sqnorm_plan(n):
    plan = (L.i32 * 3)()
    L.check(L.load().ick_grad_sqnorm_plan(n, plan), "ick_grad_sqnorm_plan")
    return tuple(plan)


def grad_sqnorm(g, words, scratch=None, gscale=1.0, gscale_den=None):
    _opt_words(words, "grad_sqnorm")
    if g.dtype != torch.float32 or not g.is_cuda or not g.is_contiguous():
        raise L.IckError("grad_sqnorm needs a contiguous float32 device bucket")
    if scratch is None:
        scratch = torch.empty(grad_sqnorm_plan(g.numel())[2], device=g.device, dtype=torch.float32)
    L.check(L.load().ick_grad_sqnorm(_p(g), g.numel(), gscale, _p(gscale_den), _p(scratch), scratch.numel(), _p(words),
                                     _stream()), "ick_grad_sqnorm")
    return words


def conv1_wgrad_plan(B, Cc, P, d):
    plan, floats = (L.i32 * 4)(), L.i64()
    L.check(L.load().ick_conv1_wgrad_plan(B, Cc, P, d, plan, C.byref(floats)), "ick_conv1_wgrad_plan")
    return tuple(plan), floats.value


def conv1_wgrad(d_img, feats, dw, db, scratch=None):
    for name, t in (("d_img", d_img), ("feats", feats), ("dw", dw), ("db", db)):
        if not isinstance(t, torch.Tensor) or t.dtype != torch.float32 or not t.is_cuda or not t.is_contiguous():
            raise L.IckError("conv1_wgrad needs %s as a contiguous float32 device tensor" % name)
    if d_img.dim() != 3 or feats.dim() not in (3, 4):
        raise L.IckError("conv1_wgrad takes d_img (B, P, d) and feats (B, C, P) or (B, C, H, W)")
    B, P, d = d_img.shape
    Cc = feats.shape[1]
    if feats.shape[0] != B or feats.numel() != B * Cc * P or dw.numel() != d * Cc or db.numel() != d:
        raise L.IckError("conv1_wgrad: d_img %s, feats %s, dw %s, db %s do not fit together"
                         % (tuple(d_img.shape), tuple(feats.shape), tuple(dw.shape), tuple(db.shape)))
    need = conv1_wgrad_plan(B, Cc, P, d)[1]
    if scratch is None:
        scratch = torch.empty(need, device=d_img.device, dtype=torch.float32)
    elif scratch.dtype != torch.float32 or not scratch.is_cuda or not scratch.is_contiguous() or scratch.numel() < need:
        raise L.IckError("conv1_wgrad needs %d contiguous float32 device floats of scratch" % need)
    L.check(L.load().ick_conv1_wgrad(_p(d_img), _p(feats), _p(dw), _p(db), B, Cc, P, d, _p(scratch), scratch.numel(),
                                     _stream()), "ick_conv1_wgrad")
    return dw, db


_ADAM_ENTRIES = ("ick_adam_clamp", "ick_adam_opt", "ick_adam_clamp_derive", "ick_adam_opt_derive")
_ADAM_EMA_ENTRIES = ("ick_adam_ema", "ick_adam_ema_derive")
_ADAM_DECAY_ENTRIES = ("ick_adam_decay", "ick_adam_decay_derive")
DECAY_DECOUPLED, DECAY_COUPLED = 0, 1


def adam_update(p, g, m, v, step, lr=None, *, words=None, schedule=None, cover=None, clip=5.0, gscale=1.0, beta1=0.9,
                beta2=0.999, eps=1e-8, step_tensor=None, gscale_den=None, ema=None, ema_decay_word=None, ema_warmup=False,
                decay_word=None, decay_mask=None, decoupled=True):
    if (lr is None) == (words is None):
        raise L.IckError("adam_update needs exactly one of lr (a host float) and words (the optimizer words)")
    if words is None and schedule is not None:
        raise L.IckError("adam_update: a schedule shapes the rate in the optimizer words; give words, not lr")
    if ema is None and (ema_decay_word is not None or ema_warmup):
        raise L.IckError("adam_update: ema_decay_word / ema_warmup shape a moving average; give ema= as well")
    if (decay_word is None) != (decay_mask is None):
        raise L.IckError("adam_update: weight decay needs both decay_word (wd) and decay_mask (which granules decay)")
    decay = ()
    if decay_word is not None:
        granules = (p.numel() + 63) // 64
        for what, t, dtype, least in (("decay_word", decay_word, torch.float32, 1),
                                      ("decay_mask", decay_mask, torch.uint8, granules)):
            if not isinstance(t, torch.Tensor) or t.dtype != dtype or not t.is_cuda or not t.is_contiguous() or \
                    t.numel() < least:
                raise L.IckError("adam_update needs %s as a contiguous %s device tensor of at least %d element(s)"
                                 % (what, str(dtype).replace("torch.", ""), least))
        decay = (_p(decay_word), _p(decay_mask), decay_mask.numel(), DECAY_DECOUPLED if decoupled else DECAY_COUPLED)
    if ema is None and not decay:
        name = _ADAM_ENTRIES[(words is not None) + 2 * (cover is not None)]
        rate = (lr,) if words is None else (_p(_opt_words(words, "adam_update")), lr_schedule_struct(schedule))
        avg, tail = (), ()
    else:
        avg, tail = (None,), (None, 0)
        if ema is not None:
            for what, t, least in (("ema", ema, p.numel()), ("ema_decay_word", ema_decay_word, 1)):
                if not isinstance(t, torch.Tensor) or t.dtype != torch.float32 or not t.is_cuda or not t.is_contiguous() or \
                        t.numel() < least:
                    raise L.IckError("adam_update needs %s as a contiguous float32 device tensor of at least %d element(s)"
                                     % (what, least))
            if ema.data_ptr() % (4 if cover is None else 16):
                raise L.IckError("adam_update: ema must lie on %d bytes" % (4 if cover is None else 16))
            avg, tail = (_p(ema),), (_p(ema_decay_word), int(bool(ema_warmup)))
        name = (_ADAM_DECAY_ENTRIES if decay else _ADAM_EMA_ENTRIES)[cover is not None]
        rate = (0.0, _p(_opt_words(words, "adam_update")), lr_schedule_struct(schedule)) if words is not None else \
            (lr, None, L.LrSchedule())
        tail += decay
    if cover is None:
        over = (p.numel(),)
    else:
        L.ADAM_DERIVE_BYTES, L.ADAM_DERIVE_FLOATS = cover.nbytes, p.numel()
        over = (_p(cover.items_dev), _p(cover.blocks_dev), cover.n_blocks)
    L.check(getattr(L.load(), name)(_p(p), _p(g), _p(m), _p(v), *avg, *over, gscale, clip, *rate, beta1, beta2, eps, step,
                                    _p(step_tensor), _p(gscale_den), *tail, _stream()), name)


def counter_add(counter, inc=1):
    L.check(L.load().ick_counter_add(_p(counter), inc, _stream()), "ick_counter_add")


def counter_add_if(counter, inc, flag):
    L.check(L.load().ick_counter_add_if(_p(counter), inc, _p(flag), _stream()), "ick_counter_add_if")


def scale_by_ratio(x, num, den):
    L.check(L.load().ick_scale_by_ratio(_p(x), x.numel(), _p(num), _p(den), _stream()), "ick_scale_by_ratio")
```

image-captioning-with-external-knowledge_amd/profiling.py:

```python
import ctypes as C

import torch

from . import lib as L

PEAK_FP32_MFMA_TFLOPS = 157.3
PEAK_HBM_GBS = 8000.0
PEAK_BF16_MFMA_TFLOPS = 2500.0
PEAK_SPLIT_FP32_EQ_TFLOPS = PEAK_BF16_MFMA_TFLOPS / 6.0
PER_CU_L2_STREAM_GBS = 134.0


def _struct(arg):
    return arg._obj if hasattr(arg, "_obj") else arg


def _gemm_label(a):
    lay = ("A k-major" if (a.a_rs == 1 and a.a_ks != 1) else "A row-major") + ", " + \
          ("B k-major" if (a.b_rs == 1 and a.b_ks != 1) else "B row-major")
    return "%dx%dx%d (%s%s)" % (a.M, a.N, a.K, lay, ", split-K %d" % a.split_k if a.split_k > 1 else "")


TRACE_KEYS = {}

# ... 18 lines not shown
            label = "GEMM " + _gemm_label(a) + tag
            _split_plan(a, label)
            return label, fl, "flop_split" if spl else "flop"
        _split_plan(a, "chain GEMMs (< 2 GFLOP each: projections, FFN, their data gradients)")
        return "chain GEMMs (< 2 GFLOP each: projections, FFN, their data gradients)", fl, "flop"
    if name == "ick_gemm_grouped":
        arr, n = args[0], args[1]
        fl = fl_split = 0.0
        for i in range(n):
            a = arr[i]
            if not (a.flags & L.GEMM_COLSUM_ONLY):
                f = 2.0 * a.M * a.N * a.K
                fl += f
                spl, ps = _split_plan(a)
                if ps:
                    _split_plan(a, "grouped weight-gradient GEMMs")
                if spl:
                    fl_split += f
        return "grouped weight-gradient GEMMs", fl, "flop_mixed", fl_split
    if name == "ick_attention":
        a = _struct(args[0])
        return "attention forward (T=%d)" % a.T if a.T > 1 else "attention decode step", 4.0 * a.B * a.H * a.T * a.S * a.dh, "flop"
    if name == "ick_attention_bwd":
        a = _struct(args[0])
        return "attention backward", 10.0 * a.B * a.H * a.T * a.S * a.dh, "flop"
    if name == "ick_rowchain_fwd":
        a = _struct(args[0])
        fl = 2.0 * a.M * (a.K1 * a.d + (a.d * a.N2 if a.w2p else 0))
        return ("row chain forward (out-projection + add & norm + next Linear)", fl, "flop", 0.0,
                4.0 * (a.K1 * a.d + (a.d * a.N2 if a.w2p else 0)))
    if name == "ick_rowchain_bwd":
        a = _struct(args[0])
        fl = 2.0 * a.M * ((a.K0 * a.d if a.g0 else 0) + (2 * a.d * a.N1 if a.w1p else 0) + a.d * a.d)
        return ("row chain backward (Linear' + norm' [+ FFN' + norm'] + out-projection')", fl, "flop", 0.0,
                4.0 * ((a.K0 * a.d if a.g0 else 0) + (2 * a.d * a.N1 if a.w1p else 0) + a.d * a.d))
    if name == "ick_pack_weights":
        arr, n = args[0], args[1]
        return "packed weight copies", 8.0 * sum(arr[i].N * arr[i].K for i in range(n)), "byte"
    if name == "ick_presplit_weights":
        arr, n = args[0], args[1]
        return "presplit weights", 10.0 * sum(arr[i].N * arr[i].K for i in range(n)), "byte"
    if name == "ick_add_layernorm":
        rows, d = args[5], args[6]
        return "residual + LayerNorm", 4.0 * rows * d * 3, "byte"
    if name == "ick_layernorm_bwd":
        rows, d = args[9], args[10]
        return "LayerNorm backward", 4.0 * rows * d * 5, "byte"
    if name == "ick_packed_ce":
        B, Lc, Vx = args[4], args[5], args[6]
        return "packed cross entropy (+ gradient)", 4.0 * B * Lc * Vx * (2 if args[11] else 1), "byte"
    if name == "ick_packed_ce_weighted":
        B, Lc, Vx = args[5], args[6], args[7]
        return "weighted packed cross entropy (+ gradient)", 4.0 * B * Lc * Vx * (2 if args[12] else 1), "byte"
    if name == "ick_packed_ce_packed":
        B, Lc, Vx = args[6], args[7], args[8]
        return (("weighted " if args[5] else "") + "packed cross entropy (+ gradient)",
                4.0 * B * Lc * Vx * (2 if args[13] else 1), "byte")
    if name == "ick_packed_ce_smooth":
        B, Lc, Vx = args[8], args[9], args[10]
        return (("weighted " if args[6] else "") + "packed cross entropy, label smoothing (+ gradient)",
                4.0 * B * Lc * Vx * (2 if args[15] else 1), "byte")
    if name in ("ick_adam_clamp", "ick_adam_opt"):
        return "clamp + Adam", 4.0 * args[4] * 7, "byte"
    if name in ("ick_adam_clamp_derive", "ick_adam_opt_derive"):
        return "clamp + Adam + re-laid-out weight copies", float(getattr(L, "ADAM_DERIVE_BYTES", 0)), "byte"
    if name == "ick_adam_ema":
        return "clamp + Adam + EMA", 4.0 * args[5] * 9, "byte"
    if name == "ick_adam_ema_derive":
        return ("clamp + Adam + EMA + re-laid-out weight copies",
                float(getattr(L, "ADAM_DERIVE_BYTES", 0)) + 8.0 * getattr(L, "ADAM_DERIVE_FLOATS", 0), "byte")
    if name == "ick_adam_decay":
        streams = 9 if args[4] else 7
        return ("clamp + Adam + weight decay" + (" + EMA" if args[4] else ""),
                4.0 * args[5] * streams + args[5] / 64.0, "byte")
    if name == "ick_adam_decay_derive":
        floats = getattr(L, "ADAM_DERIVE_FLOATS", 0)
        return ("clamp + Adam + weight decay" + (" + EMA" if args[4] else "") + " + re-laid-out weight copies",
                float(getattr(L, "ADAM_DERIVE_BYTES", 0)) + (8.0 * floats if args[4] else 0.0) + floats / 64.0, "byte")
    if name == "ick_grad_sqnorm":
        return "gradient norm (global-norm clip)", 4.0 * args[1], "byte"
    if name == "ick_decode_layers":
        c = _struct(args[0])
        kv = 4.0 * c.R * c.layers * 2 * c.H * c.S * 32
        w = 4.0 * (c.layers * (4 * c.d * c.d + 2 * c.d * c.d + 2 * c.d * c.FF) + c.V * c.d)
        return "fused decode step (3 kernels / layer + head + vocabulary)", kv + w, "byte"
    if name == "ick_decode_layers_part":
        c = _struct(args[0])
        kv = 4.0 * c.R * c.layers * 2 * c.H * c.S * 32
        w = 4.0 * (c.layers * (4 * c.d * c.d + 2 * c.d * c.d + 2 * c.d * c.FF) + c.V * c.d)
        first = 4.0 * 4 * c.d * c.d
        return ("fused decode step (3 kernels / layer + head + vocabulary)", first if args[2] == 1 else kv + w - first, "byte")
    if name == "ick_decode_select_greedy":
        return "greedy selection + next-token embedding", None, None
    return name[4:].replace("_", " "), None, None


class _Profiled:
    def __init__(self, lib):
        self._lib = lib

    def __getattr__(self, name):
        fn = getattr(self._lib, name)
        argtypes = L.SIGNATURES.get(name)
        if L.PROFILE is None or not argtypes or argtypes[-1] is not L.vp:
            return fn

        def timed(*args):
            label, work, unit, *rest = classify(name, args)
            e0, e1 = torch.cuda.Event(enable_timing=True), torch.cuda.Event(enable_timing=True)
            e0.record()
            rc = fn(*args)
            e1.record()
            L.PROFILE.append((label, work, unit, e0, e1, rest[0] if rest else 0.0, rest[1] if len(rest) > 1 else 0.0))
            return rc
        return timed


def start():
    L.PROFILE = []
    L._proxy = _Profiled(L.load_raw())


def stop():
    rec, L.PROFILE = L.PROFILE, None
    L._proxy = None
    return rec


def summarise(records, steps):
    torch.cuda.synchronize()
    rows = {}
    for label, work, unit, e0, e1, work_split, cu_bytes in records:
        r = rows.setdefault(label, {"name": label, "launches": 0, "us": 0.0, "work": 0.0, "unit": unit, "work_split": 0.0,
                                    "cu_bytes": 0.0})
        r["launches"] += 1
        r["cu_bytes"] += cu_bytes
        r["us"] += e0.elapsed_time(e1) * 1e3
        if work is not None:
            r["work"] += work
            r["work_split"] += work_split
    out = []
    for r in rows.values():
        n = r["launches"]
        row = {"name": r["name"], "launches_per_step": n / steps, "avg_us": r["us"] / n, "us_per_step": r["us"] / steps}
        if r["unit"] in ("flop", "flop_split", "flop_mixed") and r["us"] > 0 and r["work"] > 0:
            ach = r["work"] / (r["us"] * 1e-6) / 1e12
# ... 25 lines not shown
```

image-captioning-with-external-knowledge_amd/training.py:

```python
import collections
import contextlib
import functools
import math
import os
import weakref

import torch

from . import dp, ops
from .bucket import ParamBucket
from .decoder import DropSites
from .lib import IckError
from .weights import DerivedWeights, first_stage, vocab_planes_wanted


class Tape:

    def __init__(self):
        self.enc_layers = {}
        self.dec_layers = []
        self.misc = {}


def _p(x):
# ... 445 lines not shown

    def late(self):
        if self.side is not None and getattr(self, "joined", False):
            self.retired = self.side
            self.side = ops.SideStream()
        self._run(True)


def _backward_phases(dec, tape, dscores, grads, want_image_grad=False, image_grad_sink=None):
    m = tape.misc
    V = dec.vocab_size
    h, ee, fe = m["h"], m["ee"], m["fe"]
    dims = _dims(dec, h)
    B, L, M, d, H, _, dev = dims
    grads = dict(grads)
    for prm in unique_parameters(dec):
        if id(prm) not in grads and prm is not dec.word_embedding.weight:
            grads[id(prm)] = torch.zeros_like(prm)
    P, K, Fn, S = m["P"], m["K"], m["Fn"], m["S"]
    Vx = dscores.shape[2]
    dsc2 = dscores.view(M, Vx)
    pre = m.get("prezero") or {}

    def zeroed(name, like):
        t = pre.get(name)
        return t if t is not None and t.shape == like.shape else torch.zeros_like(like)

    dee = zeroed("dee", ee)
    dfe = zeroed("dfe", fe) if fe is not None else None
    hv = m["hv"] if dec.has_facts else h
    dhv0 = pre.get("dhv")
    pack = m.get("pack")
    valid = pack if os.environ.get("ICK_NO_VALID_ROW_WGRAD", "0") in ("", "0") and not ops.is_deterministic() else None
    hv_t_ps = _rows_t_presplit(hv.view(M, d), pack) if _g(grads, dec.fc_vocab.weight) is not None else None
    if dhv0 is not None and (dhv0.shape != (M, d) or (pack is None and ops.is_deterministic())):
        dhv0 = None
    if dhv0 is None and pack is not None:
        dhv0 = torch.zeros(M, d, device=dev, dtype=torch.float32)
    dhv = _lin_bwd(grads, dsc2[:, :V], hv.view(M, d), dec.fc_vocab.weight, dec.fc_vocab.bias, dx=dhv0,
                   acc=dhv0 is not None, group_now=True, wt_ps=m.get("vocab_t_ps"), xt_ps=hv_t_ps, pack=pack).view(B, L, d)
    if dec.has_facts:
        dh = ops.mul(dhv, m["gate"])
        dgate = ops.mul(dhv, h)
        gw, gb = _g(grads, dec.fc_predicate.weight), _g(grads, dec.fc_predicate.bias)
        if gw is not None:
            ops.context_gate_bwd(m["captions"], m["facts"], dgate, gw, gb, K, V, mode=0)
    else:
        dh = dhv

    def gbuf(param):
        return _g(grads, param)

    ops.pointer_scores_bwd(dscores, V, h, ee, _p(dec.fc_entity.weight), None, dh, dee, gbuf(dec.fc_entity.weight),
                           gbuf(dec.fc_entity.bias), pack=pack)
    if dec.has_facts:
        ops.pointer_scores_bwd(dscores, V + K, h, fe, _p(dec.fc_fact.weight), m["eib"], dh, dfe,
                               gbuf(dec.fc_fact.weight), gbuf(dec.fc_fact.bias), pack=pack)
    layers = list(dec.transformer_decoder.layers)
    nseg = 2 * len(layers)
    dkv_rows = ops.attention_bwd_buffer((B, S, nseg * d), L, S, d // H, dev)
    ops.stamp("bwd: head done")
    pkb = m.get("pkb")
    mem_t_ps = _memory_t_presplit(m, B, S, d)
    mem2 = m["mem"].view(B * S, d)
    dx, state = dh, (dh.view(M, d), None, None)
    for li in reversed(range(len(layers))):
        if pkb is not None:
            state = _decoder_layer_bwd_chain(li, layers[li], tape.dec_layers[li], state, dkv_rows, m["kv"], S, grads,
                                             pkb, mem2, mem_t_ps, valid, dims)
            dx = state[0]
        else:
            dx = _decoder_layer_bwd(li, layers[li], tape.dec_layers[li], dx, dkv_rows, m["kv"], S, grads, mem2,
                                    mem_t_ps, valid, dims)
        ops.stamp("bwd: decoder layer %d done" % li)
    yield
    nctx = K + Fn
    dkv_ctx = dkv_rows[:, P:]
    if pkb is None:
        ksplit = max(1, min(8, (nseg * d) // 450)) if B * nctx * d <= 1280 * 512 else 1
        if ops.is_deterministic():
            ksplit = 1
        dctx = (torch.zeros if ksplit > 1 else torch.empty)(B, nctx, d, device=dev, dtype=torch.float32)
        ops.gemm_raw(dkv_ctx, m["wkv"], dctx, B * nctx, d, nseg * d, nseg * d, 1, 1, d, d, a_grp=nctx,
                     a_gs=S * nseg * d, atomic=ksplit > 1, split_k=ksplit)
    if want_image_grad:
        d_img = torch.empty(B, P, d, device=dev, dtype=torch.float32)

        def image_grad():
            ops.gemm_raw(dkv_rows, m["wkv"], d_img, B * P, d, nseg * d, nseg * d, 1, 1, d, d, a_grp=P, a_gs=S * nseg * d)
            if image_grad_sink is not None:
                image_grad_sink(d_img)

        if image_grad_sink is not None and ops.SIDE is not None and not os.environ.get("ICK_CONV1_BWD_MAIN"):
            ops.SIDE.submit(image_grad, dkv_rows, m["wkv"], d_img)
        else:
            image_grad()
        m["d_img"] = d_img
    ops.stamp("bwd: context gradient ready")

    def context_encoder_bwd(stack, name, tag, rows):
        if pkb is not None:
            return _context_encoder_bwd_chain(dec, stack, tape.enc_layers[name], grads, pkb, tag, dkv_ctx[:, rows],
                                              pkb[("kv", "T")])
        return _context_encoder_bwd(dec, stack, tape.enc_layers[name], dctx[:, rows].contiguous(), grads)

    dee_enc = context_encoder_bwd(dec.transformer_encoder_entities, "entities", "e", slice(0, K))
    ops.stamp("bwd: entity context encoder done")
    dee += dee_enc
    if dec.has_facts:
        dfe += context_encoder_bwd(dec.transformer_encoder_facts, "facts", "f", slice(K, None))
# ... 182 lines not shown
        self.flat_e = self.enc_e = self._ema_word = None
        self._ema_swapped = False
        self.train_conv1 = bool(train_conv1)
        self.encoder_lr = float(encoder_lr)
        if self.train_conv1 and encoder is None:
            raise IckError("train_conv1=True needs encoder=: the step cannot reach Encoder.conv1 without it")
        self.max_grad_norm = check_max_grad_norm(max_grad_norm)
        self.lr_schedule = check_lr_schedule(lr_schedule)
        self._words = self._norm_scratch = None
        self.label_smoothing = self._check_smoothing(label_smoothing)
        self._eps_word = None
        self.lazy = bool(lazy_update)
        self.packed_head = os.environ.get("ICK_NO_PACKED_HEAD", "0") in ("", "0")
        self._pending = False
        self._gb = None
        if deterministic is None:
            deterministic = ops.is_deterministic()
        else:
            ops.set_deterministic(bool(deterministic))
        self.deterministic = bool(deterministic)
        self.enc = encoder
        self.seed = seed
        self.lr, self.clip, self.betas, self.eps = lr, (0.0 if grad_clip is None else grad_clip), betas, eps
        self.pg = process_group
        self.use_graph = use_graph
        self.step_count = 0
        params = [p for p in unique_parameters(decoder) if p.requires_grad]
        early_ids = {id(p) for p in early_parameters(decoder)}
        params = [p for p in params if id(p) in early_ids] + [p for p in params if id(p) not in early_ids]
        dev = params[0].device
        if self.train_conv1 and encoder.conv1.weight.device != dev:
            raise IckError("train_conv1=True: the encoder must be on the decoder's device (%s)" % dev)
        self._dec_bucket = db = ParamBucket(params, IckError)
        self._buckets = [db]
        self.params, self.n = params, db.n
        self.n_early = db.offsets[sum(id(p) in early_ids for p in params)]
        self.flat_p, self.flat_m, self.flat_v = db.p, db.m, db.v
        self.ne = 0
        if self.train_conv1:
            c1 = encoder.conv1
            self._enc_bucket = eb = ParamBucket([c1.weight, c1.bias], IckError)
            self._buckets.append(eb)
            self.enc_params, self.ne = eb.params, eb.n
            self.enc_p, self.enc_m, self.enc_v = eb.p, eb.m, eb.v
            encoder.invalidate_caches()
        self._t = self.n + self.ne
        self.flat_g = torch.zeros(self._t + 2, device=dev, dtype=torch.float32)
        self.grads = db.grad_views(self.flat_g[:self.n])
        if self.train_conv1:
            self.enc_g = self.flat_g[self.n:self._t]
            eg = eb.grad_views(self.enc_g)
            self._c1_gw, self._c1_gb = eg[id(c1.weight)].view(c1.weight.shape[0], -1), eg[id(c1.bias)]
        self.counter = torch.zeros(1, device=dev, dtype=torch.int32)
        self.one = torch.ones(1, device=dev, dtype=torch.float32)
        if self.max_grad_norm is not None or self.lr_schedule is not None:
            self._make_words()
        if self.label_smoothing != 0.0:
            self._eps_word = torch.full((1,), self.label_smoothing, device=dev, dtype=torch.float32)
        if self.ema_decay is not None:
            self._ema_word = torch.full((1,), self.ema_decay, device=dev, dtype=torch.float32)
        if self.ss is not None:
            sd = (self.seed if self.ss["seed"] is None else self.ss["seed"]) & (2 ** 64 - 1)
            self._ss_words = (torch.full((1,), self.ss["prob"], device=dev, dtype=torch.float32),
                              torch.full((1,), self.ss["temperature"], device=dev, dtype=torch.float32),
                              torch.tensor([sd - 2 ** 64 if sd >= 2 ** 63 else sd], device=dev, dtype=torch.int64))
        if self.weight_decay is not None:
            names = {}
            for name, p in decoder.named_parameters():
                names.setdefault(id(p), name)
            self._decayed = [(names[id(p)], p) for p in params if self._decay_filter(names[id(p)], p)]
            self._wd_word = torch.full((1,), self.weight_decay, device=dev, dtype=torch.float32)
            self._wd_mask = db.decay_mask(p for _, p in self._decayed)
        if self.encoder_weight_decay is not None:
            self._enc_wd_word = torch.full((1,), self.encoder_weight_decay, device=dev, dtype=torch.float32)
            self._enc_wd_mask = eb.decay_mask([encoder.conv1.weight])
        self._graphs = {}
        self.derived = None
        self._derived_tried = False
        for b in self._buckets:
            dp.broadcast_bucket(b.p, self.pg)
            if self.ema_decay is not None:
                b.start_average()
        self.flat_e = self._dec_bucket.e
        if self.train_conv1:
            self.enc_e = self._enc_bucket.e
        env = os.environ.get("ICK_SPLIT_ALLREDUCE", "0")
        self.allreduce_probe_ms = None
        if dp.world_size(self.pg) > 1 and (env == "auto" or os.environ.get("ICK_ALLREDUCE_PROBE") == "1"):
            self.allreduce_probe_ms = dp.time_all_reduce(self.flat_g, self.pg)
        if env == "auto":
            self.split = self.allreduce_probe_ms is not None and self.allreduce_probe_ms > 0.26
        else:
            self.split = env not in ("", "0")

    def _overlap(self, off_switch):
        if self.deterministic:
            return False
        return bool((self.use_graph or os.environ.get("ICK_GROUP_SAME_STREAM")) and not os.environ.get(off_switch))

    def _enc_kwargs(self, enc_in):
        if enc_in.dim() == 4:
            c1 = self.enc.conv1
            return dict(enc_tok=None, feats=enc_in, conv1=(c1.weight.detach(), c1.bias.detach(), self.enc.conv1_presplit()))
        return dict(enc_tok=enc_in)

    @staticmethod
# ... 2 lines not shown
        if not 0.0 <= eps < 1.0:
            raise IckError("label_smoothing must lie in [0, 1), got %r" % (eps,))
        return eps

    def set_label_smoothing(self, eps):
        eps = self._check_smoothing(eps)
        if eps != 0.0:
            if self._eps_word is None:
                self._eps_word = torch.empty(1, device=self.flat_p.device, dtype=torch.float32)
            self._eps_word.fill_(eps)
        self.label_smoothing = eps

    def _make_words(self):
        dev = self.flat_p.device
        if self._words is None:
            w = [0.0] * 8
            w[0], w[1], w[3] = float(self.lr), self.max_grad_norm or 0.0, 1.0
            self._words = torch.tensor(w, device=dev, dtype=torch.float32)
            self._sched = ops.lr_schedule_struct(self.lr_schedule)
        if self.max_grad_norm is not None and self._norm_scratch is None:
            self._norm_scratch = torch.empty(ops.grad_sqnorm_plan(self.n)[2], device=dev, dtype=torch.float32)

    def _word(self, i, what):
        if self._words is None:
            raise IckError("%s needs a TrainStep built with max_grad_norm= or lr_schedule=" % what)
        return self._words[i:i + 1]

    @property
    def grad_norm(self):
        return self._word(2, "grad_norm")

    @property
    def clip_coef(self):
        return self._word(3, "clip_coef")

    @property
    def lr_now(self):
        return self._word(4, "lr_now")

    def set_max_grad_norm(self, m):
        m = check_max_grad_norm(m)
        self.flush()
        if (m is None) != (self.max_grad_norm is None):
            self._graphs.clear()
        self.max_grad_norm = m
        if m is None and self._words is None:
            return
        self._make_words()
        self._words[1:2].fill_(m or 0.0)
        if m is None:
            self._words[3:4].fill_(1.0)

    def _loss(self, scores, captions, decode_len, weights, pack=None):
        tail = dict(want_grad=True, out_sum=self.flat_g[self._t:self._t + 1], out_count=self.flat_g[self._t + 1:])
        pad = self.dec.word_map["<pad>"]
        if self.label_smoothing != 0.0:
            return ops.packed_ce_smooth(scores, captions, pack if pack is not None else decode_len, pad, self._eps_word,
                                        weights=weights, **tail)
        if pack is not None:
            return ops.packed_ce_rows(scores, captions, pack, pad, weights=weights, **tail)
        if weights is None:
            return ops.packed_ce(scores, captions, decode_len, pad, **tail)
        return ops.packed_ce_weighted(scores, captions, decode_len, weights, pad, **tail)

    def _side_tail(self, box, captions, entities, facts, lengths):
        def tail():
            self.flat_g.zero_()
            if self.packed_head:
                box["pack"] = ops.HeadRows(lengths, captions.shape[0], captions.shape[1])
                box["decode_len"] = box["pack"].decode_len
            else:
                box["decode_len"] = (lengths.reshape(-1) - 1).to(torch.int32)
            box["prezero"] = _prezeroed(self.dec, captions, entities, facts)

        return tail

    def _forward_and_loss(self, captions, caption_masks, entities, facts, enc_in, gmap, lengths, weights=None):
        box = {}
        lazy = self._lazy_active(enc_in)
        fed, fed_masks = captions, caption_masks
        if self.ss is not None:
            if self._ss_inline:
                self._first_pass(captions, caption_masks, entities, facts, enc_in, gmap, lengths)
            fed, fed_masks = self._ss_bufs[tuple(captions.shape)][:2]
        scores, tape = forward_with_tape(self.dec, fed, fed_masks, entities, facts, gmap=gmap,
                                         seed=self.seed * 2654435761 & 0xFFFFFFFF, epoch=self.counter, fresh_pack=True,
                                         overlap=self._overlap("ICK_NO_FWD_OVERLAP"),
                                         side_tail=self._side_tail(box, captions, entities, facts, lengths),
                                         derived=self.derived, pre_side=self._deferred_update if lazy else None,
                                         pre_main=self._adam_conv1 if self.train_conv1 and lazy else None,
                                         head_rows=lambda: box.get("pack"), **self._enc_kwargs(enc_in))
        tape.misc["prezero"] = box.get("prezero")
        ops.stamp("fwd: scores done")
        ce = self._loss(scores, captions, box["decode_len"], weights, box.get("pack"))
        ops.stamp("CE done")
        return (self.dec, tape, ce[2], self.grads), dict(self._conv1_bwd_kwargs(enc_in),
                                                         overlap=self._overlap("ICK_NO_BWD_OVERLAP"))

    def _first_pass(self, captions, caption_masks, entities, facts, enc_in, gmap, lengths, weights=None):
        dec = self.dec
        B, Lc = captions.shape
        V, K = dec.vocab_size, entities.shape[1]
        Fn = facts.shape[1] if dec.has_facts else 0
        wm = dec.word_map
        wi = dec.weight_images()
        groups = ["kv"] + (["chain"] if dec.chain_supported() else []) + (["pred_wt"] if dec.has_facts else [])
        if ops.gemm_split_mode() != 0:
# ... 36 lines not shown

    def sampled_inputs(self):
        self._need_sampling("sampled_inputs")
        if self._ss_out is None:
            raise IckError("sampled_inputs: no step has run yet")
        return self._ss_out

    def _part_a(self, *inputs):
        ops.stamp("A: start")
        args, kwargs = self._forward_and_loss(*inputs)
        backward_from_tape(*args, **kwargs)
        ops.stamp("A: end (after join)")

    def _lazy_active(self, enc_in):
        return bool(self.lazy and self.ss is None and self.use_graph and self.derived is not None and not self.split
                    and not self.deterministic
                    and enc_in is not None and enc_in.dim() == 4 and self._overlap("ICK_NO_FWD_OVERLAP"))

    def _conv1_bwd_kwargs(self, enc_in):
        if not self.train_conv1:
            return {}

        def sink(d_img):
            ops.stamp("conv1 weight gradient starts")
            ops.conv1_wgrad(d_img, enc_in, self._c1_gw, self._c1_gb)
            ops.stamp("conv1 weight gradient done")

        return dict(want_image_grad=True, image_grad_sink=sink)

    def _ema_kwargs(self, e):
        if self.ema_decay is None:
            return {}
        return dict(ema=e, ema_decay_word=self._ema_word, ema_warmup=self.ema_warmup)

    def _decay_kwargs(self, word, mask):
        if word is None:
            return {}
        return dict(decay_word=word, decay_mask=mask, decoupled=self.decoupled_weight_decay)

    def _adam_conv1(self):
        ops.adam_update(self.enc_p, self.enc_g, self.enc_m, self.enc_v, 1, lr=self.encoder_lr, clip=self.clip, gscale=1.0,
                        beta1=self.betas[0], beta2=self.betas[1], eps=self.eps, step_tensor=self.counter,
                        gscale_den=self.flat_g[self._t + 1:], **self._ema_kwargs(self.enc_e),
                        **self._decay_kwargs(self._enc_wd_word, self._enc_wd_mask))
        self._conv1_resplit()

    def _conv1_resplit(self):
        ps = self.enc.conv1_presplit()
        if ps is not None:
            w = self.enc.conv1.weight.detach()
            ops.presplit_weights([(w.view(w.shape[0], -1), ps)])

    def _deferred_update(self):
        self._adam()
        ops.counter_add_if(self.counter, 1, self.flat_g[self._t + 1:])

    def flush(self):
        if not self._pending:
            return
        if self._gb is not None:
            self._gb.replay()
        else:
            self._part_b()
        self.flat_g[self._t + 1:].zero_()
        self._pending = False
        self.dec.invalidate_caches()
        if self.derived is not None:
            self.derived.mark_current()

    def _adam(self):
        den = self.flat_g[self._t + 1:]
        if self._words is not None and self.max_grad_norm is not None:
            ops.grad_sqnorm(self.flat_g[:self.n], self._words, self._norm_scratch, gscale=1.0, gscale_den=den)
        rate = dict(lr=self.lr) if self._words is None else dict(words=self._words, schedule=self._sched)
        ops.adam_update(self.flat_p, self.flat_g, self.flat_m, self.flat_v, 1, cover=self.derived,
                        clip=self.clip, gscale=1.0, beta1=self.betas[0], beta2=self.betas[1], eps=self.eps,
                        step_tensor=self.counter, gscale_den=den, **rate, **self._ema_kwargs(self.flat_e),
                        **self._decay_kwargs(self._wd_word, self._wd_mask))

    def _part_a1(self, *inputs):
        args, kwargs = self._forward_and_loss(*inputs)
        self._bp = BackwardPass(*args, **kwargs)
        self._bp.early(join=True)

    def _part_a2(self):
        self._bp.late()

    def _part_b(self):
        ops.stamp("B: start")
        self._adam()
        if self.train_conv1:
            self._adam_conv1()
        ops.counter_add(self.counter, 1)
        ops.stamp("B: end")

    @staticmethod
    def _warm_static(fn, inputs):
        static = [None if t is None else t.contiguous().clone() for t in inputs]
        side = torch.cuda.Stream()
        side.wait_stream(torch.cuda.current_stream())
        with torch.cuda.stream(side):
            fn(*static)
        torch.cuda.current_stream().wait_stream(side)
        return static

    @staticmethod
    def _after(first, fn):
        return fn if first is None else lambda *s: (first(*s), fn(*s))

    def _capture(self, fn, inputs, first=None):
        static = self._warm_static(self._after(first, fn), inputs)
        g = torch.cuda.CUDAGraph()
        with ops.capture(g):
            fn(*static)
        return g, static

    def _capture_split(self, inputs, first=None):
        static = self._warm_static(self._after(first, lambda *s: (self._part_a1(*s), self._part_a2())), inputs)
        g1, g2 = torch.cuda.CUDAGraph(), torch.cuda.CUDAGraph()
        with ops.capture(g1):
            self._part_a1(*static)
        with ops.capture(g2):
            self._part_a2()
        return g1, static, g2

    def _adam_order(self):
        mine = {id(p) for p in self.params}
        return [p for p in unique_parameters(self.dec) if id(p) in mine]

    def _slot(self, flat, p):
        return self._dec_bucket.slot(flat, p)
# ... 307 lines not shown
                        first(*static)
                    if not self._graphs:
                        self._ss_first.clear()
                    self._ss_first[key] = g0
                gb, _ = self._capture(self._part_b, [])
                self._gb = gb
                self._graphs[key] = (ga, static, gb, ga2)
                self._last_static = static
            except RuntimeError as e:
                import warnings
                warnings.warn("ick_amd TrainStep: hipGraph capture failed (%s); continuing without graphs" % e)
                torch.cuda.synchronize()
                self.use_graph = False
            for t, sv in zip(state, snap):
                t.copy_(sv)
            if self.derived is not None:
                self.derived.stale = True
                self.derived.ensure_current()
            if self.train_conv1:
                self._conv1_resplit()
            self.flat_g[self._t + 1:].zero_()
        if self.use_graph:
            ga, static, gb, ga2 = self._graphs[key]
            if self._lazy_active(enc_in) and not self._pending:
                self.flat_g[self._t + 1:].zero_()
            from .decoder import copy_inputs
            copy_inputs(static, inputs)
            part_a, part_a2, part_b = ga.replay, None if ga2 is None else ga2.replay, gb.replay
            first = self._ss_first[key].replay if self.ss is not None and not self._ss_inline else None
        else:
            part_a = functools.partial(self._part_a1 if self.split else self._part_a, *inputs)
            part_a2, part_b = self._part_a2 if self.split else None, self._part_b
            first = functools.partial(self._first_pass, *inputs) if self.ss is not None and not self._ss_inline else None
        if first is not None:
            first()
        part_a()
        if part_a2 is None:
            dp.allreduce_bucket(self.flat_g, self.pg)
        else:
            w1 = dp.allreduce_bucket(self.flat_g[:self.n_early], self.pg, async_op=True)
            part_a2()
            w2 = dp.allreduce_bucket(self.flat_g[self.n_early:], self.pg, async_op=True)
            for w in (w1, w2):
                if w is not None:
                    w.wait()
        if self._lazy_active(enc_in):
            self._pending = True
        else:
            part_b()
        self.step_count += 1
        dec.invalidate_caches()
        if self.derived is not None:
            self.derived.mark_current()
        return self.flat_g[self._t:self._t + 1] / self.flat_g[self._t + 1:]
```

include/ick_amd.h:

```cpp
#ifndef ICK_AMD_H
#define ICK_AMD_H

#include <stdint.h>

#ifdef __cplusplus
extern "C" {
#endif

#define ICK_OK 0
#define ICK_EINVAL (-1)
#define ICK_EALIGN (-2)
#define ICK_EWORKSPACE (-3)

#define ICK_MAX_LAYERS 8

int ick_version(void);
int ick_set_deterministic(int on);
int ick_get_deterministic(void);
int ick_device_info(int* num_cu, int* wave_size, char* arch_name, int arch_name_len);

typedef struct {
    const float* A; const float* B; float* C; const float* bias;
    int32_t M, N, K;
    int64_t a_rs, a_ks; int32_t a_grp; int64_t a_gs; const int32_t* a_gmap;
// ... 323 lines not shown
    float* pack_t;
    float* copy;
    void* ps;
    void* ps_t;
    float* tr;
    int64_t copy_ld, tr_ld;
} ick_adam_item;
typedef struct ick_adam_block {
    int32_t item, tn, tk, cnt4;
    int64_t off4;
    float* copy;
} ick_adam_block;
int ick_adam_clamp_derive(float* p, float* g, float* m, float* v, const ick_adam_item* items,
                          const ick_adam_block* blocks, int32_t n_blocks, float gscale, float clip, float lr,
                          float beta1, float beta2, float eps, int32_t step, const uint32_t* step_ptr,
                          const float* gscale_den, void* stream);

#define ICK_OPT_WORDS 8
enum { ICK_LR_CONSTANT = 0, ICK_LR_INVERSE_SQRT = 1, ICK_LR_COSINE = 2, ICK_LR_LINEAR = 3 };
typedef struct ick_lr_schedule {
    int32_t kind, warmup, total;
    float min_ratio;
} ick_lr_schedule;
int ick_grad_sqnorm_plan(int64_t n, int32_t* plan);
int ick_grad_sqnorm(const float* g, int64_t n, float gscale, const float* gscale_den, float* scratch,
                    int64_t scratch_floats, float* words, void* stream);
int ick_adam_opt(float* p, float* g, float* m, float* v, int64_t n, float gscale, float clip, float* words,
                 ick_lr_schedule sched, float beta1, float beta2, float eps, int32_t step, const uint32_t* step_ptr,
                 const float* gscale_den, void* stream);
int ick_adam_opt_derive(float* p, float* g, float* m, float* v, const ick_adam_item* items, const ick_adam_block* blocks,
                        int32_t n_blocks, float gscale, float clip, float* words, ick_lr_schedule sched, float beta1,
                        float beta2, float eps, int32_t step, const uint32_t* step_ptr, const float* gscale_den,
                        void* stream);
int ick_adam_ema(float* p, float* g, float* m, float* v, float* e, int64_t n, float gscale, float clip, float lr,
                 float* words, ick_lr_schedule sched, float beta1, float beta2, float eps, int32_t step,
                 const uint32_t* step_ptr, const float* gscale_den, const float* ema_decay, int32_t ema_warmup,
                 void* stream);
int ick_adam_ema_derive(float* p, float* g, float* m, float* v, float* e, const ick_adam_item* items,
                        const ick_adam_block* blocks, int32_t n_blocks, float gscale, float clip, float lr, float* words,
                        ick_lr_schedule sched, float beta1, float beta2, float eps, int32_t step, const uint32_t* step_ptr,
                        const float* gscale_den, const float* ema_decay, int32_t ema_warmup, void* stream);
#define ICK_DECAY_DECOUPLED 0
#define ICK_DECAY_COUPLED 1
int ick_adam_decay(float* p, float* g, float* m, float* v, float* e, int64_t n, float gscale, float clip, float lr,
                   float* words, ick_lr_schedule sched, float beta1, float beta2, float eps, int32_t step,
                   const uint32_t* step_ptr, const float* gscale_den, const float* ema_decay, int32_t ema_warmup,
                   const float* decay, const uint8_t* decay_mask, int64_t n_granules, int32_t decay_form, void* stream);
int ick_adam_decay_derive(float* p, float* g, float* m, float* v, float* e, const ick_adam_item* items,
                          const ick_adam_block* blocks, int32_t n_blocks, float gscale, float clip, float lr, float* words,
                          ick_lr_schedule sched, float beta1, float beta2, float eps, int32_t step,
                          const uint32_t* step_ptr, const float* gscale_den, const float* ema_decay, int32_t ema_warmup,
                          const float* decay, const uint8_t* decay_mask, int64_t n_granules, int32_t decay_form,
                          void* stream);
int ick_conv1_wgrad_plan(int32_t B, int32_t C, int32_t P, int32_t d, int32_t* plan, int64_t* scratch_floats);
int ick_conv1_wgrad(const float* d_img, const float* feats, float* dw, float* db, int32_t B, int32_t C, int32_t P,
                    int32_t d, float* scratch, int64_t scratch_floats, void* stream);
int ick_counter_add(uint32_t* counter, uint32_t inc, void* stream);
int ick_counter_add_if(uint32_t* counter, uint32_t inc, const float* flag, void* stream);
int ick_copy_batch(const void* const* src, void* const* dst, const long long* bytes, int n, void* stream);
int ick_timestamp(unsigned long long* out, void* stream);
int ick_scale_by_ratio(float* x, int64_t n, const float* num, const float* den, void* stream);

int ick_head_rowmap(const int64_t* lengths, int32_t B, int32_t L, int32_t* decode_len, int32_t* rowstart,
                    int32_t* rowmap, void* stream);
int ick_pointer_scores_packed(const float* h, const float* ctx, const float* w, const float* bias, const float* ind,
                              float* out, int32_t B, int32_t T, int32_t Kc, int32_t d, int64_t out_ld, int32_t col0,
                              const int32_t* rowmap, const int32_t* count, void* stream);
int ick_packed_ce_packed(const float* scores, int64_t ld, const int64_t* captions, const int32_t* rowmap,
                         const int32_t* count, const float* weights, int32_t B, int32_t L, int32_t Vx, int32_t pad_token,
                         float* row_loss, float* loss_sum, float* count_out, float* dscores, void* stream);
int ick_packed_ce_smooth(const float* scores, int64_t ld, const int64_t* captions, const int32_t* rowmap,
                         const int32_t* count, const int32_t* decode_len, const float* weights, const float* eps,
                         int32_t B, int32_t L, int32_t Vx, int32_t pad_token, float* row_loss, float* loss_sum,
                         float* count_out, float* dscores, void* stream);
int ick_pointer_scores_bwd_packed(const float* ds, int64_t ds_ld, int32_t col0, const float* h, const float* ctx,
                                  const float* w, const float* ind, float* dh, float* dctx, float* dw, float* dbias,
                                  int32_t B, int32_t T, int32_t Kc, int32_t d, const int32_t* rowmap,
                                  const int32_t* rowstart, void* stream);
int ick_gather_rows(const float* src, int64_t src_rs, const int32_t* rowmap, const int32_t* count, float* dst,
                    int64_t dst_rs, int32_t max_rows, int32_t d, void* stream);

int ick_row_logprob_rank(const float* scores, int64_t ld, const int64_t* captions, const int32_t* rowmap,
                         const int32_t* count, int32_t R, int32_t L, int32_t Vx, int32_t pad_token, float* token_log_prob,
                         int32_t* rank, int32_t* best, void* stream);
int ick_caption_score_sums(const int32_t* rowstart, int32_t R, int32_t L, int32_t top_k, float* token_log_prob,
                           int32_t* rank, int32_t* best, float* log_prob, int32_t* tokens, float* loss_sum, float* count,
                           float* top1_hits, float* topk_hits, void* stream);

int ick_sched_sample_mix(const float* scores, int64_t ld, const int32_t* rowstart, const int32_t* decode_len,
                         const int64_t* captions, const int64_t* caption_masks, int32_t B, int32_t L, int32_t V,
                         int32_t K, int32_t F, int32_t start_token, int32_t pad_token, const float* prob,
                         const float* temperature, const int64_t* seed, const uint32_t* step, int32_t argmax,
                         int64_t* captions_in, int64_t* masks_in, int32_t* replaced, void* stream);

#define ICK_GEO_TERMS 8
#define ICK_GEO_NAME_CHARS 50
#define ICK_GEO_MAX_T 128
#define ICK_GEO_MAX_K 4095
#define ICK_GEO_MAX_BINS 64
#define ICK_GEO_MAX_TYPES 4096
int ick_geo_reference_counts(const int64_t* tokens, int32_t N, int32_t T, const int32_t* image_index,
                             const float* entities, const int64_t* entity_names, int32_t B, int32_t K, int32_t C,
                             int32_t V, const int32_t* trigger_ids, int32_t of_id, int32_t the_id, int32_t a_id,
                             const double* bins_distance, int32_t n_distance, const double* bins_azimuth,
                             int32_t n_azimuth, int32_t n_types, int64_t hist_ld, int64_t seed, int64_t row_offset,
                             int32_t* marks, int32_t* generated, int32_t* random, void* stream);

#ifdef __cplusplus
}
#endif
#endif
```

Before: 822,700 decode-steps/s.

## Fold step-counter bump into Adam, fuse pointer bwd kernels, compute loss mean on device

```diff
diff --git a/image-captioning-with-external-knowledge_amd/csrc/adam.hip b/image-captioning-with-external-knowledge_amd/csrc/adam.hip
--- a/image-captioning-with-external-knowledge_amd/csrc/adam.hip
+++ b/image-captioning-with-external-knowledge_amd/csrc/adam.hip
@@ -22,6 +22,21 @@
     int64_t base;
     int coupled;
 };
+
+struct AdamBump {
+    uint32_t* counter;
+    uint32_t inc;
+    uint32_t* ticket;
+};
+__device__ __forceinline__ void adam_bump(const AdamBump& b) {
+    if (b.ticket == nullptr) return;
+    __syncthreads();
+    if (threadIdx.x == 0 &&
+        __hip_atomic_fetch_add(b.ticket, 1u, __ATOMIC_RELAXED, __HIP_MEMORY_SCOPE_AGENT) == gridDim.x - 1u) {
+        *b.counter += b.inc;
+        __hip_atomic_store(b.ticket, 0u, __ATOMIC_RELAXED, __HIP_MEMORY_SCOPE_AGENT);
+    }
+}
 
 constexpr int kGranuleShift = 6;
 
@@ -111,7 +126,7 @@
                                                          float gscale, float clip, float lr, float b1, float b2,
                                                          float eps, int step0, const uint32_t* step_ptr,
                                                          const float* __restrict__ gscale_den, float* words,
-                                                         ick_lr_schedule sched, AdamEma ema, AdamDecay dec) {
+                                                         ick_lr_schedule sched, AdamEma ema, AdamDecay dec, AdamBump bump) {
     const int64_t stride = (int64_t)gridDim.x * 256;
     AdamHyper h;
     if (!adam_hyper<kOpt, kEma, kDecay>(h, gscale, clip, lr, b1, b2, eps, step0, step_ptr, gscale_den, words, sched, ema,
@@ -124,6 +139,7 @@
         g[i] = gi; m[i] = mi; v[i] = vi; p[i] = pi;
         if (kEma) { ema1(h, ei, pi); ema.e[i] = ei; }
     }
+    adam_bump(bump);
 }
 
 template <bool kOpt, bool kEma, bool kDecay>
@@ -132,7 +148,7 @@
                                                               float gscale, float clip, float lr, float b1, float b2,
                                                               float eps, int step0, const uint32_t* step_ptr,
                                                               const float* __restrict__ gscale_den, float* words,
-                                                              ick_lr_schedule sched, AdamEma ema, AdamDecay dec) {
+                                                              ick_lr_schedule sched, AdamEma ema, AdamDecay dec, AdamBump bump) {
     const int64_t stride = (int64_t)gridDim.x * 256;
     AdamHyper h;
     if (!adam_hyper<kOpt, kEma, kDecay>(h, gscale, clip, lr, b1, b2, eps, step0, step_ptr, gscale_den, words, sched, ema,
@@ -146,6 +162,7 @@
         g[i] = gi; m[i] = mi; v[i] = vi; p[i] = pi;
         if (kEma) { ema4(h, ei, pi); e[i] = ei; }
     }
+    adam_bump(bump);
 }
 
 constexpr int kT = 64;
@@ -158,7 +175,8 @@
                                                           const ick_adam_block* __restrict__ blocks, float gscale,
                                                           float clip, float lr, float b1, float b2, float eps, int step0,
                                                           const uint32_t* step_ptr, const float* __restrict__ gscale_den,
-                                                          float* words, ick_lr_schedule sched, AdamEma ema, AdamDecay dec) {
+                                                          float* words, ick_lr_schedule sched, AdamEma ema, AdamDecay dec,
+                                                          AdamBump bump) {
     __shared__ __attribute__((aligned(16))) float tile[kT * kLd];
     const ick_adam_block blk = blocks[blockIdx.x];
     AdamHyper h;
@@ -195,6 +213,7 @@
                 if (blk.copy) reinterpret_cast<float4*>(blk.copy)[j] = pi[i];
             }
         }
+        adam_bump(bump);
         return;
     }
 
@@ -318,6 +337,7 @@
             if (nl >= rlo && nl < rhi && k0 + kl < K) it.tr[(int64_t)(k0 + kl) * it.tr_ld + n0 + nl] = tile[nl * kLd + kl];
         }
     }
+    adam_bump(bump);
 }
 
 }
@@ -341,18 +361,22 @@
 template <bool kOpt, bool kEma, bool kDecay = false>
 static int launch_adam(float* p, float* g, float* m, float* v, int64_t n, float gscale, float clip, float lr, float* words,
                        ick_lr_schedule sched, float beta1, float beta2, float eps, int32_t step, const uint32_t* step_ptr,
-                       const float* gscale_den, AdamEma ema, void* stream, AdamDecay dec = AdamDecay{}) {
+                       const float* gscale_den, AdamEma ema, void* stream, AdamDecay dec = AdamDecay{},
+                       AdamBump bump = AdamBump{}) {
     bool al16;
     if (int rc = adam_args<kEma, kDecay>(p, g, m, v, n, step, step_ptr, ema, dec, al16)) return rc;
+    if (bump.ticket) ICK_CHECK_ARG(step_ptr != nullptr);
+    bump.counter = const_cast<uint32_t*>(step_ptr);
     if (kDecay) ICK_CHECK_ARG(dec.granules >= ceil_div(n, (int64_t)1 << kGranuleShift));
     if (kEma && (reinterpret_cast<uintptr_t>(ema.e) & 3)) return ICK_EALIGN;
     int64_t done = 0;
     if (n >= 4096 && al16) {
         const int64_t n4 = n / 4;
+        const AdamBump here = n % 4 == 0 ? bump : AdamBump{};
         hipLaunchKernelGGL((adam_clamp_vec4_kernel<kOpt, kEma, kDecay>), dim3((int)std::min<int64_t>(ceil_div(n4, 256), 4096)),
                            dim3(256), 0, (hipStream_t)stream, reinterpret_cast<float4*>(p), reinterpret_cast<float4*>(g),
                            reinterpret_cast<float4*>(m), reinterpret_cast<float4*>(v), n4, gscale, clip, lr, beta1, beta2,
-                           eps, step, step_ptr, gscale_den, words, sched, ema, dec);
+                           eps, step, step_ptr, gscale_den, words, sched, ema, dec, here);
         done = 4 * n4;
         if (done == n) ICK_LAUNCH_RET();
     }
@@ -360,7 +384,7 @@
     dec.base = done;
     hipLaunchKernelGGL((adam_clamp_kernel<kOpt, kEma, kDecay>), dim3((int)std::min<int64_t>(ceil_div(n - done, 256), 4096)),
                        dim3(256), 0, (hipStream_t)stream, p + done, g + done, m + done, v + done, n - done, gscale, clip, lr,
-                       beta1, beta2, eps, step, step_ptr, gscale_den, words, sched, ema, dec);
+                       beta1, beta2, eps, step, step_ptr, gscale_den, words, sched, ema, dec, bump);
     ICK_LAUNCH_RET();
 }
 
@@ -369,13 +393,15 @@
                               const ick_adam_block* blocks, int32_t n_blocks, float gscale, float clip, float lr,
                               float* words, ick_lr_schedule sched, float beta1, float beta2, float eps, int32_t step,
                               const uint32_t* step_ptr, const float* gscale_den, AdamEma ema, void* stream,
-                              AdamDecay dec = AdamDecay{}) {
+                              AdamDecay dec = AdamDecay{}, AdamBump bump = AdamBump{}) {
     bool al16;
     if (int rc = adam_args<kEma, kDecay>(p, g, m, v, blocks ? n_blocks : 0, step, step_ptr, ema, dec, al16)) return rc;
     if (!al16) return ICK_EALIGN;
+    if (bump.ticket) ICK_CHECK_ARG(step_ptr != nullptr);
+    bump.counter = const_cast<uint32_t*>(step_ptr);
     hipLaunchKernelGGL((adam_derive_kernel<kOpt, kEma, kDecay>), dim3(n_blocks), dim3(256), 0, (hipStream_t)stream, p, g, m, v,
                        items, blocks, gscale, clip, lr, beta1, beta2, eps, step, step_ptr, gscale_den, words, sched, ema,
-                       dec);
+                       dec, bump);
     ICK_LAUNCH_RET();
 }
 
@@ -498,3 +524,61 @@
                                                           sched, beta1, beta2, eps, step, step_ptr, gscale_den, ema, stream,
                                                           dec); });
 }
+
+template <bool kDerive, typename... Over>
+static int adam_step(float* p, float* g, float* m, float* v, float* e, float gscale, float clip, float lr, float* words,
+                     ick_lr_schedule sched, float beta1, float beta2, float eps, int32_t step, uint32_t* step_ptr,
+                     const float* gscale_den, const float* ema_decay, int32_t ema_warmup, const float* decay,
+                     const uint8_t* decay_mask, int64_t n_granules, int32_t decay_form, uint32_t bump_inc,
+                     uint32_t* ticket, void* stream, Over... over) {
+    const AdamEma ema = e ? AdamEma{e, ema_decay, ema_warmup != 0} : AdamEma{};
+    const AdamDecay dec{decay, decay_mask, n_granules, 0, decay_form};
+    const AdamBump bump{nullptr, bump_inc, ticket};
+    if (words) ICK_CHECK_ARG(lr_schedule_ok(sched));
+    if (!words) sched = ick_lr_schedule{};
+    auto go = [&](auto opt, auto avg, auto wd) {
+        constexpr bool kOpt = decltype(opt)::value, kEma = decltype(avg)::value, kDecay = decltype(wd)::value;
+        const float rate = kOpt ? 0.f : lr;
+        if constexpr (kDerive)
+            return launch_adam_derive<kOpt, kEma, kDecay>(p, g, m, v, over..., gscale, clip, rate, words, sched, beta1, beta2,
+                                                          eps, step, step_ptr, gscale_den, ema, stream,
+                                                          kDecay ? dec : AdamDecay{}, bump);
+        else
+            return launch_adam<kOpt, kEma, kDecay>(p, g, m, v, over..., gscale, clip, rate, words, sched, beta1, beta2, eps,
+                                                   step, step_ptr, gscale_den, ema, stream, kDecay ? dec : AdamDecay{},
+                                                   bump);
+    };
+    using T = std::true_type;
+    using F = std::false_type;
+    const int which = (words ? 1 : 0) | (e ? 2 : 0) | (decay ? 4 : 0);
+    switch (which) {
+        case 0: return go(F{}, F{}, F{});
+        case 1: return go(T{}, F{}, F{});
+        case 2: return go(F{}, T{}, F{});
+        case 3: return go(T{}, T{}, F{});
+        case 4: return go(F{}, F{}, T{});
+        case 5: return go(T{}, F{}, T{});
+        case 6: return go(F{}, T{}, T{});
+        default: return go(T{}, T{}, T{});
+    }
+}
+
+extern "C" int ick_adam_step(float* p, float* g, float* m, float* v, float* e, int64_t n, float gscale, float clip, float lr,
+                             float* words, ick_lr_schedule sched, float beta1, float beta2, float eps, int32_t step,
+                             uint32_t* step_ptr, const float* gscale_den, const float* ema_decay, int32_t ema_warmup,
+                             const float* decay, const uint8_t* decay_mask, int64_t n_granules, int32_t decay_form,
+                             uint32_t bump_inc, uint32_t* ticket, void* stream) {
+    return adam_step<false>(p, g, m, v, e, gscale, clip, lr, words, sched, beta1, beta2, eps, step, step_ptr, gscale_den,
+                            ema_decay, ema_warmup, decay, decay_mask, n_granules, decay_form, bump_inc, ticket, stream, n);
+}
+
+extern "C" int ick_adam_step_derive(float* p, float* g, float* m, float* v, float* e, const ick_adam_item* items,
+                                    const ick_adam_block* blocks, int32_t n_blocks, float gscale, float clip, float lr,
+                                    float* words, ick_lr_schedule sched, float beta1, float beta2, float eps, int32_t step,
+                                    uint32_t* step_ptr, const float* gscale_den, const float* ema_decay,
+                                    int32_t ema_warmup, const float* decay, const uint8_t* decay_mask, int64_t n_granules,
+                                    int32_t decay_form, uint32_t bump_inc, uint32_t* ticket, void* stream) {
+    return adam_step<true>(p, g, m, v, e, gscale, clip, lr, words, sched, beta1, beta2, eps, step, step_ptr, gscale_den,
+                           ema_decay, ema_warmup, decay, decay_mask, n_granules, decay_form, bump_inc, ticket, stream,
+                           items, blocks, n_blocks);
+}
diff --git a/image-captioning-with-external-knowledge_amd/csrc/backward.hip b/image-captioning-with-external-knowledge_amd/csrc/backward.hip
--- a/image-captioning-with-external-knowledge_amd/csrc/backward.hip
+++ b/image-captioning-with-external-knowledge_amd/csrc/backward.hip
@@ -226,16 +226,15 @@
     }
 }
 
-__global__ __launch_bounds__(256) void pointer_bwd_dh_kernel(const float* __restrict__ ds, int64_t ds_ld, int col0,
-                                                             const float* __restrict__ ctx, const float* __restrict__ w,
-                                                             const float* __restrict__ ind, float* __restrict__ dh,
-                                                             int T, int Kc, int d, const int32_t* __restrict__ rowmap,
-                                                             const int32_t* __restrict__ count) {
-    chain_priority();
-    int b = blockIdx.y, t = blockIdx.x;
+__device__ __forceinline__ void pointer_bwd_dh_role(int bx, int by, int B, const float* __restrict__ ds, int64_t ds_ld,
+                                                    int col0, const float* __restrict__ ctx, const float* __restrict__ w,
+                                                    const float* __restrict__ ind, float* __restrict__ dh, int T, int Kc,
+                                                    int d, const int32_t* __restrict__ rowmap,
+                                                    const int32_t* __restrict__ count) {
+    int b = by, t = bx;
     int64_t dsrow = (int64_t)b * T + t;
     if (rowmap != nullptr) {
-        if (dsrow >= device_bound((int)gridDim.y * T, count)) return;
+        if (dsrow >= device_bound(B * T, count)) return;
         const int lr = rowmap[dsrow];
         b = lr / T;
         t = lr - b * T;
@@ -265,19 +264,26 @@
     }
 }
 
-template <bool SEQ>
-__global__ __launch_bounds__(256) void pointer_bwd_dctx_kernel(const float* __restrict__ ds, int64_t ds_ld, int col0,
-                                                               const float* __restrict__ h, const float* __restrict__ ctx,
-                                                               const float* __restrict__ w, const float* __restrict__ ind,
-                                                               float* __restrict__ dctx, float* __restrict__ dw,
-                                                               float* __restrict__ dbias, int B, int T, int Kc, int d,
-                                                               const int32_t* __restrict__ rowstart) {
+__global__ __launch_bounds__(256) void pointer_bwd_dh_kernel(const float* __restrict__ ds, int64_t ds_ld, int col0,
+                                                             const float* __restrict__ ctx, const float* __restrict__ w,
+                                                             const float* __restrict__ ind, float* __restrict__ dh,
+                                                             int T, int Kc, int d, const int32_t* __restrict__ rowmap,
+                                                             const int32_t* __restrict__ count) {
     chain_priority();
-    extern __shared__ float gs[];
+    pointer_bwd_dh_role(blockIdx.x, blockIdx.y, gridDim.y, ds, ds_ld, col0, ctx, w, ind, dh, T, Kc, d, rowmap, count);
+}
+
+template <bool SEQ, bool kBatch>
+__device__ __forceinline__ void pointer_bwd_dctx_role(int bx, int by, float* gs, const float* __restrict__ ds,
+                                                      int64_t ds_ld, int col0, const float* __restrict__ h,
+                                                      const float* __restrict__ ctx, const float* __restrict__ w,
+                                                      const float* __restrict__ ind, float* __restrict__ dctx,
+                                                      float* __restrict__ dw, float* __restrict__ dbias, int B, int T,
+                                                      int Kc, int d, const int32_t* __restrict__ rowstart) {
     float* red = gs + T * Kc;
     float* dwp = red + 4;
     const int lane = threadIdx.x & 63, wave = threadIdx.x >> 6;
-  for (int b = SEQ ? 0 : blockIdx.x; b < (SEQ ? B : (int)blockIdx.x + 1); ++b) {
+  for (int b = SEQ ? 0 : bx; b < (SEQ ? B : bx + 1); ++b) {
     float bsum = 0.f;
     const int64_t row0 = rowstart ? rowstart[b] : (int64_t)b * T;
     const int nrow = rowstart ? min(T, rowstart[b + 1] - rowstart[b]) : T;
@@ -289,15 +295,27 @@
         gs[idx] = g;
     }
     bsum = block_sum<4>(bsum, red);
-    if (threadIdx.x == 0 && blockIdx.y == 0) { if (SEQ) dbias[0] += bsum; else atomicAdd(dbias, bsum); }
-    const int c = blockIdx.y * 64 + lane;
+    if (threadIdx.x == 0 && by == 0) { if (SEQ) dbias[0] += bsum; else atomicAdd(dbias, bsum); }
+    const int c = by * 64 + lane;
     const bool ok = c < d;
     const float* hb = h + (int64_t)b * T * d + (ok ? c : 0);
     const float wc = ok ? w[c] : 0.f;
     float dwl = 0.f;
     for (int k = wave; k < Kc; k += 4) {
         float acc = 0.f;
-        for (int t = 0; t < T; ++t) acc = fmaf(gs[t * Kc + k], hb[(int64_t)t * d], acc);
+        if (kBatch) {
+            int t = 0;
+            for (; t + 8 <= T; t += 8) {
+                float hv[8];
+#pragma unroll
+                for (int q = 0; q < 8; ++q) hv[q] = hb[(int64_t)(t + q) * d];
+#pragma unroll
+                for (int q = 0; q < 8; ++q) acc = fmaf(gs[(t + q) * Kc + k], hv[q], acc);
+            }
+            for (; t < T; ++t) acc = fmaf(gs[t * Kc + k], hb[(int64_t)t * d], acc);
+        } else {
+            for (int t = 0; t < T; ++t) acc = fmaf(gs[t * Kc + k], hb[(int64_t)t * d], acc);
+        }
         if (ok) {
             const int64_t o = ((int64_t)b * Kc + k) * d + c;
             dctx[o] += acc * wc;
@@ -312,6 +330,41 @@
     }
     if (SEQ) __syncthreads();
   }
+}
+
+template <bool SEQ>
+__global__ __launch_bounds__(256) void pointer_bwd_dctx_kernel(const float* __restrict__ ds, int64_t ds_ld, int col0,
+                                                               const float* __restrict__ h, const float* __restrict__ ctx,
+                                                               const float* __restrict__ w, const float* __restrict__ ind,
+                                                               float* __restrict__ dctx, float* __restrict__ dw,
+                                                               float* __restrict__ dbias, int B, int T, int Kc, int d,
+                                                               const int32_t* __restrict__ rowstart) {
+    chain_priority();
+    extern __shared__ float gs[];
+    pointer_bwd_dctx_role<SEQ, false>(blockIdx.x, blockIdx.y, gs, ds, ds_ld, col0, h, ctx, w, ind, dctx, dw, dbias, B, T, Kc,
+                                      d, rowstart);
+}
+
+template <bool SEQ>
+__global__ __launch_bounds__(256) void pointer_bwd_fused_kernel(const float* __restrict__ ds, int64_t ds_ld, int col0,
+                                                                const float* __restrict__ h, const float* __restrict__ ctx,
+                                                                const float* __restrict__ w, const float* __restrict__ ind,
+                                                                float* __restrict__ dh, float* __restrict__ dctx,
+                                                                float* __restrict__ dw, float* __restrict__ dbias, int B,
+                                                                int T, int Kc, int d, const int32_t* __restrict__ rowmap,
+                                                                const int32_t* __restrict__ rowstart, int ctx_x,
+                                                                int n_ctx) {
+    chain_priority();
+    extern __shared__ float gs[];
+    const int id = blockIdx.x;
+    if (id < n_ctx) {
+        pointer_bwd_dctx_role<SEQ, true>(id % ctx_x, id / ctx_x, gs, ds, ds_ld, col0, h, ctx, w, ind, dctx, dw, dbias, B, T,
+                                         Kc, d, rowstart);
+    } else {
+        const int r = id - n_ctx;
+        pointer_bwd_dh_role(r % T, r / T, B, ds, ds_ld, col0, ctx, w, ind, dh, T, Kc, d, rowmap,
+                            rowstart ? rowstart + B : nullptr);
+    }
 }
 
 template <bool SEQ>
@@ -447,6 +500,36 @@
     ICK_LAUNCH_RET();
 }
 
+extern "C" int ick_pointer_scores_bwd_fused_packed(const float* ds, int64_t ds_ld, int32_t col0, const float* h,
+                                                   const float* ctx, const float* w, const float* ind, float* dh,
+                                                   float* dctx, float* dw, float* dbias, int32_t B, int32_t T, int32_t Kc,
+                                                   int32_t d, const int32_t* rowmap, const int32_t* rowstart,
+                                                   void* stream) {
+    ICK_CHECK_ARG(ds && h && ctx && w && dh && dctx && dw && dbias && B > 0 && B <= 65535 && T > 0 && Kc > 0 && d > 0);
+    ICK_CHECK_ARG((rowmap == nullptr) == (rowstart == nullptr) && (int64_t)B * T <= INT32_MAX);
+    const size_t smem = ((size_t)T * Kc + 4 + 256) * sizeof(float);
+    ICK_CHECK_ARG(smem <= 64 * 1024);
+    const int ctx_x = deterministic() ? 1 : B;
+    const int64_t n_ctx = (int64_t)ctx_x * ceil_div(d, 64);
+    ICK_CHECK_ARG(n_ctx + (int64_t)B * T <= INT32_MAX);
+    const dim3 grid((unsigned)(n_ctx + (int64_t)B * T));
+    hipStream_t s = (hipStream_t)stream;
+    if (deterministic())
+        hipLaunchKernelGGL(pointer_bwd_fused_kernel<true>, grid, dim3(256), smem, s, ds, ds_ld, col0, h, ctx, w, ind, dh,
+                           dctx, dw, dbias, B, T, Kc, d, rowmap, rowstart, ctx_x, (int)n_ctx);
+    else
+        hipLaunchKernelGGL(pointer_bwd_fused_kernel<false>, grid, dim3(256), smem, s, ds, ds_ld, col0, h, ctx, w, ind, dh,
+                           dctx, dw, dbias, B, T, Kc, d, rowmap, rowstart, ctx_x, (int)n_ctx);
+    ICK_LAUNCH_RET();
+}
+
+extern "C" int ick_pointer_scores_bwd_fused(const float* ds, int64_t ds_ld, int32_t col0, const float* h, const float* ctx,
+                                            const float* w, const float* ind, float* dh, float* dctx, float* dw,
+                                            float* dbias, int32_t B, int32_t T, int32_t Kc, int32_t d, void* stream) {
+    return ick_pointer_scores_bwd_fused_packed(ds, ds_ld, col0, h, ctx, w, ind, dh, dctx, dw, dbias, B, T, Kc, d, nullptr,
+                                               nullptr, stream);
+}
+
 extern "C" int ick_entity_encode_bwd(int32_t variant, const float* dee, const float* entities, int32_t ent_cols,
                                      const float* ee, const float* word_emb, int32_t vocab, float* dtype_emb,
                                      int32_t ntypes, float* dword, int32_t B, int32_t K, int32_t d, void* stream) {
diff --git a/image-captioning-with-external-knowledge_amd/csrc/score_head.hip b/image-captioning-with-external-knowledge_amd/csrc/score_head.hip
--- a/image-captioning-with-external-knowledge_amd/csrc/score_head.hip
+++ b/image-captioning-with-external-knowledge_amd/csrc/score_head.hip
@@ -370,7 +370,8 @@
                                                                const float* __restrict__ weight,
                                                                float* __restrict__ loss_sum, float* __restrict__ count,
                                                                const int32_t* __restrict__ rowmap,
-                                                               const int32_t* __restrict__ nrows) {
+                                                               const int32_t* __restrict__ nrows,
+                                                               float* __restrict__ mean) {
     __shared__ float red[4];
     float s = 0.f, c = 0.f;
     n = device_bound(n, nrows);
@@ -380,7 +381,11 @@
     }
     s = block_sum<4>(s, red);
     c = block_sum<4>(c, red);
-    if (threadIdx.x == 0) { loss_sum[0] = s; count[0] = c; }
+    if (threadIdx.x == 0) {
+        loss_sum[0] = s;
+        count[0] = c;
+        if (mean) mean[0] = c > 0.f ? s / c : 0.f;
+    }
 }
 
 struct RowScan {
@@ -670,9 +675,9 @@
     ICK_LAUNCH_RET();
 }
 
-extern "C" int ick_packed_ce(const float* scores, int64_t ld, const int64_t* captions_sorted,
+static int packed_ce_impl(const float* scores, int64_t ld, const int64_t* captions_sorted,
                              const int32_t* decode_len, int32_t B, int32_t L, int32_t Vx, int32_t pad_token,
-                             float* row_loss, float* loss_sum, float* count, float* dscores, void* stream) {
+                             float* row_loss, float* loss_sum, float* count, float* dscores, float* mean, void* stream) {
     using namespace ick;
     ICK_CHECK_ARG(scores && captions_sorted && decode_len && row_loss && loss_sum && count);
     ICK_CHECK_ARG(B > 0 && B <= 65535 && L > 0 && Vx > 0 && ld >= Vx);
@@ -680,14 +685,14 @@
     hipLaunchKernelGGL(packed_ce_rows_kernel<false>, dim3(L, B), dim3(256), 0, s, scores, ld, captions_sorted, decode_len,
                        L, Vx, pad_token, row_loss, dscores, nullptr, nullptr, CeEps<false>{});
     hipLaunchKernelGGL(packed_ce_reduce_kernel<false>, dim3(1), dim3(256), 0, s, row_loss, B * L, L, nullptr, loss_sum,
-                       count, nullptr, nullptr);
-    ICK_LAUNCH_RET();
-}
-
-extern "C" int ick_packed_ce_packed(const float* scores, int64_t ld, const int64_t* captions, const int32_t* rowmap,
+                       count, nullptr, nullptr, mean);
+    ICK_LAUNCH_RET();
+}
+
+static int packed_ce_packed_impl(const float* scores, int64_t ld, const int64_t* captions, const int32_t* rowmap,
                                     const int32_t* count, const float* weights, int32_t B, int32_t L, int32_t Vx,
                                     int32_t pad_token, float* row_loss, float* loss_sum, float* count_out, float* dscores,
-                                    void* stream) {
+                                    float* mean, void* stream) {
     using namespace ick;
     ICK_CHECK_ARG(scores && captions && rowmap && count && row_loss && loss_sum && count_out);
     ICK_CHECK_ARG(B > 0 && B <= 65535 && L > 0 && Vx > 0 && ld >= Vx && (int64_t)B * L <= INT32_MAX);
@@ -696,20 +701,21 @@
         hipLaunchKernelGGL((packed_ce_rows_kernel<true, true>), dim3(L, B), dim3(256), 0, s, scores, ld, captions, count, L,
                            Vx, pad_token, row_loss, dscores, weights, rowmap, CeEps<false>{});
         hipLaunchKernelGGL(packed_ce_reduce_kernel<true>, dim3(1), dim3(256), 0, s, row_loss, B * L, L, weights, loss_sum,
-                           count_out, rowmap, count);
+                           count_out, rowmap, count, mean);
     } else {
         hipLaunchKernelGGL((packed_ce_rows_kernel<false, true>), dim3(L, B), dim3(256), 0, s, scores, ld, captions, count, L,
                            Vx, pad_token, row_loss, dscores, nullptr, rowmap, CeEps<false>{});
         hipLaunchKernelGGL(packed_ce_reduce_kernel<false>, dim3(1), dim3(256), 0, s, row_loss, B * L, L, nullptr, loss_sum,
-                           count_out, rowmap, count);
-    }
-    ICK_LAUNCH_RET();
-}
-
-extern "C" int ick_packed_ce_smooth(const float* scores, int64_t ld, const int64_t* captions, const int32_t* rowmap,
+                           count_out, rowmap, count, mean);
+    }
+    ICK_LAUNCH_RET();
+}
+
+static int packed_ce_smooth_impl(const float* scores, int64_t ld, const int64_t* captions, const int32_t* rowmap,
                                     const int32_t* count, const int32_t* decode_len, const float* weights,
                                     const float* eps, int32_t B, int32_t L, int32_t Vx, int32_t pad_token,
-                                    float* row_loss, float* loss_sum, float* count_out, float* dscores, void* stream) {
+                                    float* row_loss, float* loss_sum, float* count_out, float* dscores, float* mean,
+                                    void* stream) {
     using namespace ick;
     ICK_CHECK_ARG(scores && captions && eps && row_loss && loss_sum && count_out);
     ICK_CHECK_ARG((rowmap != nullptr) == (count != nullptr) && (rowmap != nullptr || decode_len != nullptr));
@@ -723,11 +729,11 @@
     if (weights != nullptr) {
         if (rowmap) { ICK_CE_SMOOTH(true, true); } else { ICK_CE_SMOOTH(true, false); }
         hipLaunchKernelGGL(packed_ce_reduce_kernel<true>, dim3(1), block, 0, s, row_loss, B * L, L, weights, loss_sum,
-                           count_out, rowmap, count);
+                           count_out, rowmap, count, mean);
     } else {
         if (rowmap) { ICK_CE_SMOOTH(false, true); } else { ICK_CE_SMOOTH(false, false); }
         hipLaunchKernelGGL(packed_ce_reduce_kernel<false>, dim3(1), block, 0, s, row_loss, B * L, L, nullptr, loss_sum,
-                           count_out, rowmap, count);
+                           count_out, rowmap, count, mean);
     }
 #undef ICK_CE_SMOOTH
     ICK_LAUNCH_RET();
@@ -759,10 +765,10 @@
     ICK_LAUNCH_RET();
 }
 
-extern "C" int ick_packed_ce_weighted(const float* scores, int64_t ld, const int64_t* captions_sorted,
+static int packed_ce_weighted_impl(const float* scores, int64_t ld, const int64_t* captions_sorted,
                                       const int32_t* decode_len, const float* weights, int32_t B, int32_t L, int32_t Vx,
                                       int32_t pad_token, float* row_loss, float* loss_sum, float* count, float* dscores,
-                                      void* stream) {
+                                      float* mean, void* stream) {
     using namespace ick;
     ICK_CHECK_ARG(scores && captions_sorted && decode_len && weights && row_loss && loss_sum && count);
     ICK_CHECK_ARG(B > 0 && B <= 65535 && L > 0 && Vx > 0 && ld >= Vx && (int64_t)B * L <= INT32_MAX);
@@ -770,6 +776,68 @@
     hipLaunchKernelGGL(packed_ce_rows_kernel<true>, dim3(L, B), dim3(256), 0, s, scores, ld, captions_sorted, decode_len,
                        L, Vx, pad_token, row_loss, dscores, weights, nullptr, CeEps<false>{});
     hipLaunchKernelGGL(packed_ce_reduce_kernel<true>, dim3(1), dim3(256), 0, s, row_loss, B * L, L, weights, loss_sum,
-                       count, nullptr, nullptr);
-    ICK_LAUNCH_RET();
-}
+                       count, nullptr, nullptr, mean);
+    ICK_LAUNCH_RET();
+}
+
+extern "C" int ick_packed_ce(const float* scores, int64_t ld, const int64_t* captions_sorted, const int32_t* decode_len,
+                             int32_t B, int32_t L, int32_t Vx, int32_t pad_token, float* row_loss, float* loss_sum,
+                             float* count, float* dscores, void* stream) {
+    return packed_ce_impl(scores, ld, captions_sorted, decode_len, B, L, Vx, pad_token, row_loss, loss_sum, count, dscores,
+                          nullptr, stream);
+}
+
+extern "C" int ick_packed_ce_weighted(const float* scores, int64_t ld, const int64_t* captions_sorted,
+                                      const int32_t* decode_len, const float* weights, int32_t B, int32_t L, int32_t Vx,
+                                      int32_t pad_token, float* row_loss, float* loss_sum, float* count, float* dscores,
+                                      void* stream) {
+    return packed_ce_weighted_impl(scores, ld, captions_sorted, decode_len, weights, B, L, Vx, pad_token, row_loss, loss_sum,
+                                   count, dscores, nullptr, stream);
+}
+
+extern "C" int ick_packed_ce_packed(const float* scores, int64_t ld, const int64_t* captions, const int32_t* rowmap,
+                                    const int32_t* count, const float* weights, int32_t B, int32_t L, int32_t Vx,
+                                    int32_t pad_token, float* row_loss, float* loss_sum, float* count_out, float* dscores,
+                                    void* stream) {
+    return packed_ce_packed_impl(scores, ld, captions, rowmap, count, weights, B, L, Vx, pad_token, row_loss, loss_sum,
+                                 count_out, dscores, nullptr, stream);
+}
+
+extern "C" int ick_packed_ce_smooth(const float* scores, int64_t ld, const int64_t* captions, const int32_t* rowmap,
+                                    const int32_t* count, const int32_t* decode_len, const float* weights,
+                                    const float* eps, int32_t B, int32_t L, int32_t Vx, int32_t pad_token,
+                                    float* row_loss, float* loss_sum, float* count_out, float* dscores, void* stream) {
+    return packed_ce_smooth_impl(scores, ld, captions, rowmap, count, decode_len, weights, eps, B, L, Vx, pad_token, row_loss,
+                                 loss_sum, count_out, dscores, nullptr, stream);
+}
+
+extern "C" int ick_packed_ce_weighted_mean(const float* scores, int64_t ld, const int64_t* captions_sorted,
+                                           const int32_t* decode_len, const float* weights, int32_t B, int32_t L,
+                                           int32_t Vx, int32_t pad_token, float* row_loss, float* loss_sum, float* count,
+                                           float* dscores, float* mean, void* stream) {
+    ICK_CHECK_ARG(mean != nullptr);
+    if (weights == nullptr)
+        return packed_ce_impl(scores, ld, captions_sorted, decode_len, B, L, Vx, pad_token, row_loss, loss_sum, count,
+                              dscores, mean, stream);
+    return packed_ce_weighted_impl(scores, ld, captions_sorted, decode_len, weights, B, L, Vx, pad_token, row_loss, loss_sum,
+                                   count, dscores, mean, stream);
+}
+
+extern "C" int ick_packed_ce_packed_mean(const float* scores, int64_t ld, const int64_t* captions, const int32_t* rowmap,
+                                         const int32_t* count, const float* weights, int32_t B, int32_t L, int32_t Vx,
+                                         int32_t pad_token, float* row_loss, float* loss_sum, float* count_out,
+                                         float* dscores, float* mean, void* stream) {
+    ICK_CHECK_ARG(mean != nullptr);
+    return packed_ce_packed_impl(scores, ld, captions, rowmap, count, weights, B, L, Vx, pad_token, row_loss, loss_sum,
+                                 count_out, dscores, mean, stream);
+}
+
+extern "C" int ick_packed_ce_smooth_mean(const float* scores, int64_t ld, const int64_t* captions, const int32_t* rowmap,
+                                         const int32_t* count, const int32_t* decode_len, const float* weights,
+                                         const float* eps, int32_t B, int32_t L, int32_t Vx, int32_t pad_token,
+                                         float* row_loss, float* loss_sum, float* count_out, float* dscores, float* mean,
+                                         void* stream) {
+    ICK_CHECK_ARG(mean != nullptr);
+    return packed_ce_smooth_impl(scores, ld, captions, rowmap, count, decode_len, weights, eps, B, L, Vx, pad_token, row_loss,
+                                 loss_sum, count_out, dscores, mean, stream);
+}
diff --git a/image-captioning-with-external-knowledge_amd/lib.py b/image-captioning-with-external-knowledge_amd/lib.py
--- a/image-captioning-with-external-knowledge_amd/lib.py
+++ b/image-captioning-with-external-knowledge_amd/lib.py
@@ -249,6 +249,10 @@
                        i64, i32, vp],
     "ick_adam_decay_derive": [vp, vp, vp, vp, vp, vp, vp, i32, f32, f32, f32, vp, LrSchedule, f32, f32, f32, i32, vp, vp, vp,
                               i32, vp, vp, i64, i32, vp],
+    "ick_adam_step": [vp, vp, vp, vp, vp, i64, f32, f32, f32, vp, LrSchedule, f32, f32, f32, i32, vp, vp, vp, i32, vp, vp,
+                      i64, i32, u32, vp, vp],
+    "ick_adam_step_derive": [vp, vp, vp, vp, vp, vp, vp, i32, f32, f32, f32, vp, LrSchedule, f32, f32, f32, i32, vp, vp, vp,
+                             i32, vp, vp, i64, i32, u32, vp, vp],
     "ick_conv1_wgrad_plan": [i32, i32, i32, i32, C.POINTER(i32), C.POINTER(i64)],
     "ick_conv1_wgrad": [vp, vp, vp, vp, i32, i32, i32, i32, vp, i64, vp],
     "ick_counter_add": [vp, u32, vp],
@@ -262,6 +266,11 @@
     "ick_packed_ce_smooth": [vp, i64, vp, vp, vp, vp, vp, vp, i32, i32, i32, i32, vp, vp, vp, vp, vp],
     "ick_pointer_scores_bwd_packed": [vp, i64, i32, vp, vp, vp, vp, vp, vp, vp, vp, i32, i32, i32, i32, vp, vp, vp],
     "ick_gather_rows": [vp, i64, vp, vp, vp, i64, i32, i32, vp],
+    "ick_packed_ce_weighted_mean": [vp, i64, vp, vp, vp, i32, i32, i32, i32, vp, vp, vp, vp, vp, vp],
+    "ick_packed_ce_packed_mean": [vp, i64, vp, vp, vp, vp, i32, i32, i32, i32, vp, vp, vp, vp, vp, vp],
+    "ick_packed_ce_smooth_mean": [vp, i64, vp, vp, vp, vp, vp, vp, i32, i32, i32, i32, vp, vp, vp, vp, vp, vp],
+    "ick_pointer_scores_bwd_fused": [vp, i64, i32, vp, vp, vp, vp, vp, vp, vp, vp, i32, i32, i32, i32, vp],
+    "ick_pointer_scores_bwd_fused_packed": [vp, i64, i32, vp, vp, vp, vp, vp, vp, vp, vp, i32, i32, i32, i32, vp, vp, vp],
     "ick_row_logprob_rank": [vp, i64, vp, vp, vp, i32, i32, i32, i32, vp, vp, vp, vp],
     "ick_caption_score_sums": [vp, i32, i32, i32, vp, vp, vp, vp, vp, vp, vp, vp, vp, vp],
     "ick_sched_sample_mix": [vp, i64, vp, vp, vp, vp, i32, i32, i32, i32, i32, i32, i32, vp, vp, vp, vp, i32, vp, vp, vp,
diff --git a/image-captioning-with-external-knowledge_amd/ops.py b/image-captioning-with-external-knowledge_amd/ops.py
--- a/image-captioning-with-external-knowledge_amd/ops.py
+++ b/image-captioning-with-external-knowledge_amd/ops.py
@@ -653,7 +653,8 @@
     return out
 
 
-def packed_ce_rows(scores, captions, pack, pad_token, weights=None, want_grad=False, out_sum=None, out_count=None):
+def packed_ce_rows(scores, captions, pack, pad_token, weights=None, want_grad=False, out_sum=None, out_count=None,
+                   mean=None):
     B, Lc, Vx = scores.shape
     dev = scores.device
     if weights is not None and (weights.shape != (B,) or weights.dtype != torch.float32 or not weights.is_cuda or
@@ -666,10 +667,19 @@
     assert scores.stride(0) == Lc * scores.stride(1) and scores.stride(2) == 1
     if want_grad:
         dscores = torch.empty(B, Lc, scores.stride(1), device=dev, dtype=torch.float32)[:, :, :Vx]
-    L.check(L.load().ick_packed_ce_packed(_p(scores), scores.stride(1), _p(captions), _p(pack.rowmap), _p(pack.count),
-                                          _p(weights), B, Lc, Vx, pad_token, _p(row_loss), _p(loss_sum), _p(count),
-                                          _p(dscores), _stream()), "ick_packed_ce_packed")
+    name, tail = _ce_mean("ick_packed_ce_packed", mean)
+    L.check(getattr(L.load(), name)(_p(scores), scores.stride(1), _p(captions), _p(pack.rowmap), _p(pack.count),
+                                    _p(weights), B, Lc, Vx, pad_token, _p(row_loss), _p(loss_sum), _p(count), _p(dscores),
+                                    *tail, _stream()), name)
     return loss_sum, count, dscores
+
+
+def _ce_mean(name, mean):
+    if mean is None:
+        return name, ()
+    if mean.numel() != 1 or mean.dtype != torch.float32 or not mean.is_cuda:
+        raise L.IckError("the loss's mean must be one float32 on the device")
+    return name + "_mean", (_p(mean),)
 
 
 def row_logprob_rank(scores, captions, pack, pad_token, out=None):
@@ -707,7 +717,7 @@
     return log_prob, tokens, totals[0:1], totals[1:2], totals[2:3], totals[3:4]
 
 
-def packed_ce(scores, captions_sorted, decode_len, pad_token, want_grad=False, out_sum=None, out_count=None):
+def packed_ce(scores, captions_sorted, decode_len, pad_token, want_grad=False, out_sum=None, out_count=None, mean=None):
     B, Lc, Vx = scores.shape
     dev = scores.device
     row_loss = torch.empty(B * Lc, device=dev, dtype=torch.float32)
@@ -717,6 +727,12 @@
     if want_grad:
         dscores = torch.empty(B, Lc, scores.stride(1), device=dev, dtype=torch.float32)[:, :, :Vx]
         assert scores.stride(0) == Lc * scores.stride(1) and scores.stride(2) == 1
+    if mean is not None:
+        name, tail = _ce_mean("ick_packed_ce_weighted", mean)
+        L.check(getattr(L.load(), name)(_p(scores), scores.stride(1), _p(captions_sorted), _p(decode_len), None, B, Lc, Vx,
+                                        pad_token, _p(row_loss), _p(loss_sum), _p(count), _p(dscores), *tail, _stream()),
+                name)
+        return loss_sum, count, dscores
     L.check(L.load().ick_packed_ce(_p(scores), scores.stride(1), _p(captions_sorted), _p(decode_len), B, Lc, Vx,
                                    pad_token, _p(row_loss), _p(loss_sum), _p(count), _p(dscores), _stream()),
             "ick_packed_ce")
@@ -724,7 +740,7 @@
 
 
 def packed_ce_weighted(scores, captions_sorted, decode_len, weights, pad_token, want_grad=False, out_sum=None,
-                       out_count=None):
+                       out_count=None, mean=None):
     B, Lc, Vx = scores.shape
     dev = scores.device
     if weights.shape != (B,) or weights.dtype != torch.float32 or not weights.is_cuda or not weights.is_contiguous():
@@ -736,15 +752,15 @@
     if want_grad:
         dscores = torch.empty(B, Lc, scores.stride(1), device=dev, dtype=torch.float32)[:, :, :Vx]
         assert scores.stride(0) == Lc * scores.stride(1) and scores.stride(2) == 1
-    L.check(L.load().ick_packed_ce_weighted(_p(scores), scores.stride(1), _p(captions_sorted), _p(decode_len),
-                                            _p(weights), B, Lc, Vx, pad_token, _p(row_loss), _p(loss_sum), _p(count),
-                                            _p(dscores), _stream()),
-            "ick_packed_ce_weighted")
+    name, tail = _ce_mean("ick_packed_ce_weighted", mean)
+    L.check(getattr(L.load(), name)(_p(scores), scores.stride(1), _p(captions_sorted), _p(decode_len), _p(weights), B, Lc,
+                                    Vx, pad_token, _p(row_loss), _p(loss_sum), _p(count), _p(dscores), *tail, _stream()),
+            name)
     return loss_sum, count, dscores
 
 
 def packed_ce_smooth(scores, captions, decode_len_or_pack, pad_token, eps, weights=None, want_grad=False, out_sum=None,
-                     out_count=None):
+                     out_count=None, mean=None):
     B, Lc, Vx = scores.shape
     dev = scores.device
     if not isinstance(eps, torch.Tensor) or eps.numel() != 1 or eps.dtype != torch.float32 or not eps.is_cuda:
@@ -762,9 +778,10 @@
     if want_grad:
         dscores = torch.empty(B, Lc, scores.stride(1), device=dev, dtype=torch.float32)[:, :, :Vx]
     rowmap, rows, dl = (pack.rowmap, pack.count, None) if pack is not None else (None, None, decode_len_or_pack)
-    L.check(L.load().ick_packed_ce_smooth(_p(scores), scores.stride(1), _p(captions), _p(rowmap), _p(rows), _p(dl),
-                                          _p(weights), _p(eps), B, Lc, Vx, pad_token, _p(row_loss), _p(loss_sum),
-                                          _p(count), _p(dscores), _stream()), "ick_packed_ce_smooth")
+    name, tail = _ce_mean("ick_packed_ce_smooth", mean)
+    L.check(getattr(L.load(), name)(_p(scores), scores.stride(1), _p(captions), _p(rowmap), _p(rows), _p(dl), _p(weights),
+                                    _p(eps), B, Lc, Vx, pad_token, _p(row_loss), _p(loss_sum), _p(count), _p(dscores),
+                                    *tail, _stream()), name)
     return loss_sum, count, dscores
 
 
@@ -1276,17 +1293,15 @@
                                            V, d, pad_token, scale, *_dargs(drop), _stream()), "ick_caption_embed_bwd")
 
 
-def pointer_scores_bwd(dscores, col0, h, ctx, w, ind, dh, dctx, dw, dbias, pack=None):
+def pointer_scores_bwd(dscores, col0, h, ctx, w, ind, dh, dctx, dw, dbias, pack=None, fused=False):
     B, T, d = h.shape
     Kc = ctx.shape[1]
+    name = "ick_pointer_scores_bwd_fused" if fused else "ick_pointer_scores_bwd"
+    tail = ()
     if pack is not None:
-        L.check(L.load().ick_pointer_scores_bwd_packed(_p(dscores), dscores.stride(-2), col0, _p(h), _p(ctx), _p(w), _p(ind),
-                                                       _p(dh), _p(dctx), _p(dw), _p(dbias), B, T, Kc, d, _p(pack.rowmap),
-                                                       _p(pack.rowstart), _stream()), "ick_pointer_scores_bwd_packed")
-        return
-    L.check(L.load().ick_pointer_scores_bwd(_p(dscores), dscores.stride(-2), col0, _p(h), _p(ctx), _p(w), _p(ind),
-                                            _p(dh), _p(dctx), _p(dw), _p(dbias), B, T, Kc, d, _stream()),
-            "ick_pointer_scores_bwd")
+        name, tail = name + "_packed", (_p(pack.rowmap), _p(pack.rowstart))
+    L.check(getattr(L.load(), name)(_p(dscores), dscores.stride(-2), col0, _p(h), _p(ctx), _p(w), _p(ind), _p(dh),
+                                    _p(dctx), _p(dw), _p(dbias), B, T, Kc, d, *tail, _stream()), name)
 
 
 def entity_encode_bwd(variant, dee, entities, ee, dtype_emb, word_emb=None, dword=None):
@@ -1384,7 +1399,7 @@
 
 def adam_update(p, g, m, v, step, lr=None, *, words=None, schedule=None, cover=None, clip=5.0, gscale=1.0, beta1=0.9,
                 beta2=0.999, eps=1e-8, step_tensor=None, gscale_den=None, ema=None, ema_decay_word=None, ema_warmup=False,
-                decay_word=None, decay_mask=None, decoupled=True):
+                decay_word=None, decay_mask=None, decoupled=True, bump=None):
     if (lr is None) == (words is None):
         raise L.IckError("adam_update needs exactly one of lr (a host float) and words (the optimizer words)")
     if words is None and schedule is not None:
@@ -1403,6 +1418,27 @@
                 raise L.IckError("adam_update needs %s as a contiguous %s device tensor of at least %d element(s)"
                                  % (what, str(dtype).replace("torch.", ""), least))
         decay = (_p(decay_word), _p(decay_mask), decay_mask.numel(), DECAY_DECOUPLED if decoupled else DECAY_COUPLED)
+    if bump is not None:
+        inc, ticket = bump
+        if step_tensor is None or ticket.numel() != 1 or ticket.dtype != torch.int32 or not ticket.is_cuda:
+            raise L.IckError("adam_update: bump needs step_tensor and a one-element int32 device ticket")
+        if ema is not None:
+            for what, t, least in (("ema", ema, p.numel()), ("ema_decay_word", ema_decay_word, 1)):
+                if not isinstance(t, torch.Tensor) or t.dtype != torch.float32 or not t.is_cuda or not t.is_contiguous() or \
+                        t.numel() < least:
+                    raise L.IckError("adam_update needs %s as a contiguous float32 device tensor of at least %d element(s)"
+                                     % (what, least))
+        if cover is None:
+            name, over = "ick_adam_step", (p.numel(),)
+        else:
+            L.ADAM_DERIVE_BYTES, L.ADAM_DERIVE_FLOATS = cover.nbytes, p.numel()
+            name, over = "ick_adam_step_derive", (_p(cover.items_dev), _p(cover.blocks_dev), cover.n_blocks)
+        rate = (0.0, _p(_opt_words(words, "adam_update")), lr_schedule_struct(schedule)) if words is not None else \
+            (lr, None, L.LrSchedule())
+        L.check(getattr(L.load(), name)(_p(p), _p(g), _p(m), _p(v), _p(ema), *over, gscale, clip, *rate, beta1, beta2, eps,
+                                        step, _p(step_tensor), _p(gscale_den), _p(ema_decay_word), int(bool(ema_warmup)),
+                                        *(decay or (None, None, 0, 0)), int(inc), _p(ticket), _stream()), name)
+        return
     if ema is None and not decay:
         name = _ADAM_ENTRIES[(words is not None) + 2 * (cover is not None)]
         rate = (lr,) if words is None else (_p(_opt_words(words, "adam_update")), lr_schedule_struct(schedule))
@@ -1431,6 +1467,10 @@
                                     _p(step_tensor), _p(gscale_den), *tail, _stream()), name)
 
 
+def adam_ticket(device):
+    return torch.zeros(1, device=device, dtype=torch.int32)
+
+
 def counter_add(counter, inc=1):
     L.check(L.load().ick_counter_add(_p(counter), inc, _stream()), "ick_counter_add")
 
diff --git a/image-captioning-with-external-knowledge_amd/profiling.py b/image-captioning-with-external-knowledge_amd/profiling.py
--- a/image-captioning-with-external-knowledge_amd/profiling.py
+++ b/image-captioning-with-external-knowledge_amd/profiling.py
@@ -94,11 +94,15 @@
     if name == "ick_packed_ce_weighted":
         B, Lc, Vx = args[5], args[6], args[7]
         return "weighted packed cross entropy (+ gradient)", 4.0 * B * Lc * Vx * (2 if args[12] else 1), "byte"
-    if name == "ick_packed_ce_packed":
+    if name == "ick_packed_ce_weighted_mean":
+        B, Lc, Vx = args[5], args[6], args[7]
+        return (("weighted " if args[4] else "") + "packed cross entropy (+ gradient)",
+                4.0 * B * Lc * Vx * (2 if args[12] else 1), "byte")
+    if name in ("ick_packed_ce_packed", "ick_packed_ce_packed_mean"):
         B, Lc, Vx = args[6], args[7], args[8]
         return (("weighted " if args[5] else "") + "packed cross entropy (+ gradient)",
                 4.0 * B * Lc * Vx * (2 if args[13] else 1), "byte")
-    if name == "ick_packed_ce_smooth":
+    if name in ("ick_packed_ce_smooth", "ick_packed_ce_smooth_mean"):
         B, Lc, Vx = args[8], args[9], args[10]
         return (("weighted " if args[6] else "") + "packed cross entropy, label smoothing (+ gradient)",
                 4.0 * B * Lc * Vx * (2 if args[15] else 1), "byte")
@@ -119,6 +123,15 @@
         floats = getattr(L, "ADAM_DERIVE_FLOATS", 0)
         return ("clamp + Adam + weight decay" + (" + EMA" if args[4] else "") + " + re-laid-out weight copies",
                 float(getattr(L, "ADAM_DERIVE_BYTES", 0)) + (8.0 * floats if args[4] else 0.0) + floats / 64.0, "byte")
+    if name in ("ick_adam_step", "ick_adam_step_derive"):
+        e, decay = args[4], args[19 if name == "ick_adam_step" else 21]
+        label = "clamp + Adam" + (" + weight decay" if decay else "") + (" + EMA" if e else "")
+        if name == "ick_adam_step":
+            return label, 4.0 * args[5] * (9 if e else 7) + (args[5] / 64.0 if decay else 0.0), "byte"
+        floats = getattr(L, "ADAM_DERIVE_FLOATS", 0)
+        return (label + " + re-laid-out weight copies",
+                float(getattr(L, "ADAM_DERIVE_BYTES", 0)) + (8.0 * floats if e else 0.0) + (floats / 64.0 if decay else 0.0),
+                "byte")
     if name == "ick_grad_sqnorm":
         return "gradient norm (global-norm clip)", 4.0 * args[1], "byte"
     if name == "ick_decode_layers":
@@ -134,6 +147,8 @@
         return ("fused decode step (3 kernels / layer + head + vocabulary)", first if args[2] == 1 else kv + w - first, "byte")
     if name == "ick_decode_select_greedy":
         return "greedy selection + next-token embedding", None, None
+    if name in ("ick_pointer_scores_bwd_fused", "ick_pointer_scores_bwd_fused_packed"):
+        return "pointer scores bwd" + (" packed" if name.endswith("_packed") else ""), None, None
     return name[4:].replace("_", " "), None, None
 
 
diff --git a/image-captioning-with-external-knowledge_amd/training.py b/image-captioning-with-external-knowledge_amd/training.py
--- a/image-captioning-with-external-knowledge_amd/training.py
+++ b/image-captioning-with-external-knowledge_amd/training.py
@@ -521,10 +521,10 @@
         return _g(grads, param)
 
     ops.pointer_scores_bwd(dscores, V, h, ee, _p(dec.fc_entity.weight), None, dh, dee, gbuf(dec.fc_entity.weight),
-                           gbuf(dec.fc_entity.bias), pack=pack)
+                           gbuf(dec.fc_entity.bias), pack=pack, fused=True)
     if dec.has_facts:
         ops.pointer_scores_bwd(dscores, V + K, h, fe, _p(dec.fc_fact.weight), m["eib"], dh, dfe,
-                               gbuf(dec.fc_fact.weight), gbuf(dec.fc_fact.bias), pack=pack)
+                               gbuf(dec.fc_fact.weight), gbuf(dec.fc_fact.bias), pack=pack, fused=True)
     layers = list(dec.transformer_decoder.layers)
     nseg = 2 * len(layers)
     dkv_rows = ops.attention_bwd_buffer((B, S, nseg * d), L, S, d // H, dev)
@@ -813,6 +813,8 @@
             eg = eb.grad_views(self.enc_g)
             self._c1_gw, self._c1_gb = eg[id(c1.weight)].view(c1.weight.shape[0], -1), eg[id(c1.bias)]
         self.counter = torch.zeros(1, device=dev, dtype=torch.int32)
+        self._mean = torch.zeros(1, device=dev, dtype=torch.float32)
+        self._adam_ticket = ops.adam_ticket(dev)
         self.one = torch.ones(1, device=dev, dtype=torch.float32)
         if self.max_grad_norm is not None or self.lr_schedule is not None:
             self._make_words()
@@ -921,7 +923,8 @@
             self._words[3:4].fill_(1.0)
 
     def _loss(self, scores, captions, decode_len, weights, pack=None):
-        tail = dict(want_grad=True, out_sum=self.flat_g[self._t:self._t + 1], out_count=self.flat_g[self._t + 1:])
+        tail = dict(want_grad=True, out_sum=self.flat_g[self._t:self._t + 1], out_count=self.flat_g[self._t + 1:],
+                    mean=self._mean)
         pad = self.dec.word_map["<pad>"]
         if self.label_smoothing != 0.0:
             return ops.packed_ce_smooth(scores, captions, pack if pack is not None else decode_len, pad, self._eps_word,
@@ -1064,8 +1067,7 @@
             ops.presplit_weights([(w.view(w.shape[0], -1), ps)])
 
     def _deferred_update(self):
-        self._adam()
-        ops.counter_add_if(self.counter, 1, self.flat_g[self._t + 1:])
+        self._adam(bump=(1, self._adam_ticket))
 
     def flush(self):
         if not self._pending:
@@ -1080,7 +1082,7 @@
         if self.derived is not None:
             self.derived.mark_current()
 
-    def _adam(self):
+    def _adam(self, bump=None):
         den = self.flat_g[self._t + 1:]
         if self._words is not None and self.max_grad_norm is not None:
             ops.grad_sqnorm(self.flat_g[:self.n], self._words, self._norm_scratch, gscale=1.0, gscale_den=den)
@@ -1088,7 +1090,7 @@
         ops.adam_update(self.flat_p, self.flat_g, self.flat_m, self.flat_v, 1, cover=self.derived,
                         clip=self.clip, gscale=1.0, beta1=self.betas[0], beta2=self.betas[1], eps=self.eps,
                         step_tensor=self.counter, gscale_den=den, **rate, **self._ema_kwargs(self.flat_e),
-                        **self._decay_kwargs(self._wd_word, self._wd_mask))
+                        **self._decay_kwargs(self._wd_word, self._wd_mask), bump=bump)
 
     def _part_a1(self, *inputs):
         args, kwargs = self._forward_and_loss(*inputs)
@@ -1502,4 +1504,6 @@
         dec.invalidate_caches()
         if self.derived is not None:
             self.derived.mark_current()
+        if dp.world_size(self.pg) == 1:
+            return self._mean
         return self.flat_g[self._t:self._t + 1] / self.flat_g[self._t + 1:]
diff --git a/include/ick_amd.h b/include/ick_amd.h
--- a/include/ick_amd.h
+++ b/include/ick_amd.h
@@ -399,6 +399,17 @@
                           const uint32_t* step_ptr, const float* gscale_den, const float* ema_decay, int32_t ema_warmup,
                           const float* decay, const uint8_t* decay_mask, int64_t n_granules, int32_t decay_form,
                           void* stream);
+int ick_adam_step(float* p, float* g, float* m, float* v, float* e, int64_t n, float gscale, float clip, float lr,
+                  float* words, ick_lr_schedule sched, float beta1, float beta2, float eps, int32_t step,
+                  uint32_t* step_ptr, const float* gscale_den, const float* ema_decay, int32_t ema_warmup,
+                  const float* decay, const uint8_t* decay_mask, int64_t n_granules, int32_t decay_form,
+                  uint32_t bump_inc, uint32_t* ticket, void* stream);
+int ick_adam_step_derive(float* p, float* g, float* m, float* v, float* e, const ick_adam_item* items,
+                         const ick_adam_block* blocks, int32_t n_blocks, float gscale, float clip, float lr, float* words,
+                         ick_lr_schedule sched, float beta1, float beta2, float eps, int32_t step, uint32_t* step_ptr,
+                         const float* gscale_den, const float* ema_decay, int32_t ema_warmup, const float* decay,
+                         const uint8_t* decay_mask, int64_t n_granules, int32_t decay_form, uint32_t bump_inc,
+                         uint32_t* ticket, void* stream);
 int ick_conv1_wgrad_plan(int32_t B, int32_t C, int32_t P, int32_t d, int32_t* plan, int64_t* scratch_floats);
 int ick_conv1_wgrad(const float* d_img, const float* feats, float* dw, float* db, int32_t B, int32_t C, int32_t P,
                     int32_t d, float* scratch, int64_t scratch_floats, void* stream);
@@ -427,6 +438,26 @@
 int ick_gather_rows(const float* src, int64_t src_rs, const int32_t* rowmap, const int32_t* count, float* dst,
                     int64_t dst_rs, int32_t max_rows, int32_t d, void* stream);
 
+int ick_packed_ce_weighted_mean(const float* scores, int64_t ld, const int64_t* captions, const int32_t* decode_len,
+                                const float* weights, int32_t B, int32_t L, int32_t Vx, int32_t pad_token,
+                                float* row_loss, float* loss_sum, float* count_out, float* dscores, float* mean,
+                                void* stream);
+int ick_packed_ce_packed_mean(const float* scores, int64_t ld, const int64_t* captions, const int32_t* rowmap,
+                              const int32_t* count, const float* weights, int32_t B, int32_t L, int32_t Vx,
+                              int32_t pad_token, float* row_loss, float* loss_sum, float* count_out, float* dscores,
+                              float* mean, void* stream);
+int ick_packed_ce_smooth_mean(const float* scores, int64_t ld, const int64_t* captions, const int32_t* rowmap,
+                              const int32_t* count, const int32_t* decode_len, const float* weights, const float* eps,
+                              int32_t B, int32_t L, int32_t Vx, int32_t pad_token, float* row_loss, float* loss_sum,
+                              float* count_out, float* dscores, float* mean, void* stream);
+int ick_pointer_scores_bwd_fused(const float* ds, int64_t ds_ld, int32_t col0, const float* h, const float* ctx,
+                                 const float* w, const float* ind, float* dh, float* dctx, float* dw, float* dbias,
+                                 int32_t B, int32_t T, int32_t Kc, int32_t d, void* stream);
+int ick_pointer_scores_bwd_fused_packed(const float* ds, int64_t ds_ld, int32_t col0, const float* h, const float* ctx,
+                                        const float* w, const float* ind, float* dh, float* dctx, float* dw,
+                                        float* dbias, int32_t B, int32_t T, int32_t Kc, int32_t d, const int32_t* rowmap,
+                                        const int32_t* rowstart, void* stream);
+
 int ick_row_logprob_rank(const float* scores, int64_t ld, const int64_t* captions, const int32_t* rowmap,
                          const int32_t* count, int32_t R, int32_t L, int32_t Vx, int32_t pad_token, float* token_log_prob,
                          int32_t* rank, int32_t* best, void* stream);
```

Measured after the change: 836,400 decode-steps/s (median of 6 runs). +1.7%, better.
